# rafifmalikdzaki/Multitask-Bonetumor-yolo

Hardware: AMD Instinct MI355X
Metric: images/sec at 640x640 multitask fwd (det+seg+cls) + decode/NMS/masks (higher is better)
Workload: dtype bf16; 1 GPU; configs[1]: batch-16/GPU 640x640 multitask inference (ConvNeXt-T + C2f-BiFPN + Detect/Segment/cls) + decode + per-image NMS(top-100) + mask assembly; random-init weights; batch_per_gpu=16, img=640, parallelism=dp1 (batch sharded, no data-path collective)

## Files before the change

include/mtbt_hip.h:

```cpp
#ifndef MTBT_HIP_H
#define MTBT_HIP_H

#include <stdint.h>

#ifdef __cplusplus
extern "C" {
#endif

#define MTBT_OK 0
#define MTBT_EINVAL (-1)
#define MTBT_EALIGN (-2)
#define MTBT_ELAUNCH (-3)
#define MTBT_EWORKSPACE (-4)

#define MTBT_F32 0
#define MTBT_BF16 1
#define MTBT_F16 2

#define MTBT_ACT_NONE 0
#define MTBT_ACT_SILU 1
#define MTBT_ACT_ELU 2
#define MTBT_ACT_GELU 3
#define MTBT_ACT_DSILU 5
#define MTBT_ACT_DELU 6
#define MTBT_ACT_DGELU 7
#define MTBT_ACT_GELU_POLY 4
#define MTBT_ACT_DGELU_POLY 8

#define MTBT_OUT_NHWC 0
#define MTBT_OUT_CONVT2X2 1

#define MTBT_ABI_VERSION 5
int mtbt_abi_version(void);
int mtbt_sizeof_args(int which);
const char* mtbt_target_arch(void);

typedef struct mtbt_conv_args {
  const void* x;
  const void* w;
  void* y;
  const float* scale;
  const float* shift;
  const void* res;
  int64_t x_batch_stride, y_batch_stride, res_batch_stride;
  int32_t x_pixel_stride, y_pixel_stride, res_pixel_stride;
  int32_t N, H, W, C;
  int32_t K;
  int32_t R, S;
  int32_t stride, pad;
  int32_t Ho, Wo;
  int32_t dtype;
  int32_t out_dtype;
  int32_t act;
  int32_t out_mode;
  int32_t tile_hint;
  void* y2;
  int32_t policy;
  int32_t debug;
  float* colsum;
  const float* colsum_shift;
  int32_t colsum_sq;
  int32_t colsum_accumulate;
  void* colsum_ws;
  int64_t colsum_ws_bytes;
} mtbt_conv_args;

int mtbt_conv2d_nhwc(const mtbt_conv_args* a, void* stream);
int64_t mtbt_conv_colsum_workspace_bytes(int64_t pixels , int K, int with_squares);
int mtbt_conv_colsum_layout(const mtbt_conv_args* a, int64_t* rows, int32_t* pitch);
int mtbt_conv_kernel_choice(const mtbt_conv_args* a, int32_t* choice);

int mtbt_conv2d_nhwc_batch(const mtbt_conv_args* calls, int n, void* stream);
int mtbt_conv_batch_kernel_choice(const mtbt_conv_args* calls, int n, int32_t* choice);

int mtbt_stem_conv4x4_ln(const float* x, const float* w, const float* bias, const float* ln_w,
                         const float* ln_b, float ln_eps, void* y, int N, int H, int W, int Cout,
                         int out_dtype, void* stream);

int mtbt_dwconv_nhwc(const void* x, const void* w, const float* bias, const float* ln_w,
                     const float* ln_b, float ln_eps, const float* scale, const float* shift, int act,
                     void* y, int N, int H, int W, int C, int ksize, int dtype, void* stream);
int mtbt_dwconv3x3_mult_nhwc(const void* x, const void* w, const float* scale, const float* shift, int act, void* y,
                             int N, int H, int W, int C, int M, int dtype, void* stream);
int mtbt_dwconv_kernel_choice(int N, int H, int W, int C, int ksize, int ln, int act, int dtype, int32_t* choice);
int mtbt_dwconv3x3_mult_kernel_choice(int N, int H, int W, int C, int M, int act, int dtype, int32_t* choice);

int mtbt_layernorm_nhwc(const void* x, const float* w, const float* b, float eps, void* y,
                        int64_t pixels, int C, int dtype, void* stream);

typedef struct mtbt_fuse_args {
  const void* x[3];
  float wgt[3];
  int32_t resample[3];
  int32_t n_in;
  void* y;
  int32_t N, H, W, C;
  int32_t dtype;
  int32_t add_weight_bug;
  const float* wgt_dev;
} mtbt_fuse_args;

int mtbt_bifpn_fuse(const mtbt_fuse_args* a, void* stream);

typedef struct mtbt_node_args {
  mtbt_fuse_args fuse;
  const void* w;
  const float* shift;
  void* y;
  int32_t y_pixel_stride;
  int32_t K;
  int32_t act;
} mtbt_node_args;
int mtbt_bifpn_node_nhwc(const mtbt_node_args* a, void* stream);

typedef struct mtbt_pw_chain_args {
  const void* x;
  const void* w1;
  const float* scale1;
  const float* shift1;
  const void* w2;
  const float* scale2;
  const float* shift2;
  void* y;
  int64_t pixels;
  int32_t y_pixel_stride;
  int32_t C;
  int32_t M;
  int32_t K;
  int32_t dtype;
  int32_t out_dtype;
  int32_t act1;
  int32_t act2;
} mtbt_pw_chain_args;
int mtbt_pw_chain_nhwc(const mtbt_pw_chain_args* a, void* stream);
int mtbt_pw_chain_supported(const mtbt_pw_chain_args* a);
int mtbt_sizeof_pw_chain_args(void);

int64_t mtbt_bn_train_workspace_bytes(int64_t pixels, int C);
int mtbt_bn_train_nhwc(const void* x, void* y, const float* gamma, const float* beta, float* running_mean,
                       float* running_var, float momentum, float eps, int act, int64_t pixels, int C, int dtype,
                       void* workspace, int64_t workspace_bytes, void* stream);

int mtbt_gap_fc(const void* x, const float* w, const float* b, float* y, int N, int HW, int C,
                int nout, int dtype, void* stream);

typedef struct mtbt_decode_args {
  const float* map[3];
  int32_t h[3], w[3];
  int32_t map_pixel_stride[3];
  float stride[3];
  int32_t n_levels, N, nc, reg_max;
  int32_t xywh;
  float* boxes;
  float* scores;
  float* best_score;
  int32_t* best_label;
  float* preds_cat;
  int32_t cat_stride;
} mtbt_decode_args;

int mtbt_decode_boxes(const mtbt_decode_args* a, void* stream);

int64_t mtbt_nms_workspace_bytes(int N, int A);
int mtbt_nms_batched(const float* boxes, const float* best_score, const int32_t* best_label, int N, int A,
                     float conf_th, float iou_th, float clamp_max, int top_k, int64_t* keep_idx,
                     int32_t* keep_anchor, float* out_boxes, float* out_scores, int64_t* out_labels,
                     int32_t* counts, int32_t* n_cand, void* workspace, int64_t workspace_bytes,
                     void* stream);

typedef struct mtbt_mask_args {
  const float* protos;
  const float* coeff;
  int64_t coeff_batch_stride, coeff_k_stride, coeff_c_stride;
  const int32_t* gather_idx;
  const int32_t* counts;
  float bias;
  int32_t N, K, nm, hp, wp, Hout, Wout;
  float* logits;
  uint8_t* masks;
} mtbt_mask_args;

int mtbt_mask_assemble(const mtbt_mask_args* a, void* stream);

typedef struct mtbt_frame {
  int32_t height, width;
  float step;
  float scale;
  int32_t pitch;
  int32_t reserved;
  int64_t offset;
} mtbt_frame;

typedef struct mtbt_frame_mask_args {
  const float* protos;
  const float* coeff;
  int64_t coeff_batch_stride, coeff_k_stride, coeff_c_stride;
  const int32_t* gather_idx;
  const int32_t* counts;
  const float* boxes;
  float* boxes_frame;
  uint8_t* out;
  int64_t out_bytes;
  int32_t N, K, nm, hp, wp;
  int32_t crop;
} mtbt_frame_mask_args;

int mtbt_masks_to_frames(const mtbt_frame_mask_args* a, const mtbt_frame* frames, int n_frames, void* stream);
int mtbt_sizeof_frame_args(int which);

#define MTBT_FUSE_MAX_SOURCES 8
#define MTBT_FUSE_MAX_CANDIDATES 4096
typedef struct mtbt_box_fuse_args {
  const float* boxes[MTBT_FUSE_MAX_SOURCES];
  const float* scores[MTBT_FUSE_MAX_SOURCES];
  const int64_t* labels[MTBT_FUSE_MAX_SOURCES];
  const int32_t* counts[MTBT_FUSE_MAX_SOURCES];
  const int32_t* anchors[MTBT_FUSE_MAX_SOURCES];
  int32_t orient[MTBT_FUSE_MAX_SOURCES];
  float weight[MTBT_FUSE_MAX_SOURCES];
  int32_t n_sources, N, K, top_k;
  float img_size, iou_thr, skip_thr;
  int32_t reserved;
  float* out_boxes;
  float* out_scores;
  int64_t* out_labels;
  int32_t* out_counts;
  int32_t* n_clusters;
  int32_t* n_members;
  int32_t* lead_source;
  int32_t* lead_slot;
  int32_t* lead_anchor;
  void* workspace;
  int64_t workspace_bytes;
} mtbt_box_fuse_args;

int64_t mtbt_fuse_workspace_bytes(int n_sources, int N, int K);
int mtbt_fuse_detections(const mtbt_box_fuse_args* a, void* stream);
int mtbt_sizeof_box_fuse_args(void);
int mtbt_fuse_detections_members(const mtbt_box_fuse_args* a, int32_t* member_slot, void* stream);

typedef struct mtbt_vote_mask_args {
  const float* protos[MTBT_FUSE_MAX_SOURCES];
  const float* mc[MTBT_FUSE_MAX_SOURCES];
  int64_t mc_batch_stride[MTBT_FUSE_MAX_SOURCES], mc_k_stride[MTBT_FUSE_MAX_SOURCES], mc_c_stride[MTBT_FUSE_MAX_SOURCES];
  const int32_t* anchors[MTBT_FUSE_MAX_SOURCES];
  const float* scores[MTBT_FUSE_MAX_SOURCES];
  float weight[MTBT_FUSE_MAX_SOURCES];
  int32_t orient[MTBT_FUSE_MAX_SOURCES];
  const int32_t* member_slot;
  const int32_t* counts;
  const float* boxes;
  float* boxes_frame;
  float* W;
  float* Ss;
  uint8_t* out;
  int64_t out_bytes;
  int32_t n_sources, N, K, top_k, nm, hp, wp, crop;
} mtbt_vote_mask_args;

int mtbt_vote_masks(const mtbt_vote_mask_args* a, const mtbt_frame* frames, int n_frames, void* stream);
int mtbt_sizeof_vote_mask_args(void);

#define MTBT_TILE_MAX_PER_IMAGE 64
#define MTBT_MERGE_IOU 0
#define MTBT_MERGE_IOS 1
typedef struct mtbt_tile {
  int32_t image;
  int32_t pox, poy;
  int32_t wx0, wy0, wx1, wy1;
  int32_t height, width;
  int32_t reserved;
  float step, scale;
  float fox, foy;
} mtbt_tile;

typedef struct mtbt_tile_merge_args {
  const float* boxes;
  const float* scores;
  const int64_t* labels;
  const int32_t* counts;
  const int32_t* anchors;
  const mtbt_tile* tiles;
  const mtbt_tile* tiles_dev;
  const int32_t* first;
  int32_t N, n_tiles, K, top_k;
  int32_t metric, class_agnostic;
  float thr, skip_thr;
  float* out_boxes;
  float* out_scores;
  int64_t* out_labels;
// ... 442 lines not shown
```

multitask_bonetumor_yolo_amd/_lib.py:

```python
import ctypes as C
import os

_HERE = os.path.dirname(os.path.abspath(__file__))
LIB_PATH = os.path.join(_HERE, "csrc", "libmtbt_hip.so")

ABI_VERSION = 5
F32, BF16, F16 = 0, 1, 2
ACT_NONE, ACT_SILU, ACT_ELU, ACT_GELU, ACT_GELU_POLY, ACT_DSILU, ACT_DELU, ACT_DGELU, ACT_DGELU_POLY = 0, 1, 2, 3, 4, 5, 6, 7, 8
OUT_NHWC, OUT_CONVT2X2 = 0, 1
RES_ID, RES_UP_BILINEAR, RES_DOWN_MEAN, RES_UP_NEAREST, RES_MAXPOOL = 0, 1, 2, 3, 4
CONFUSION_MAX_NC = 64

ERRORS = {-1: "MTBT_EINVAL (bad argument / unsupported shape)", -2: "MTBT_EALIGN (misaligned pointer or stride)",
          -3: "MTBT_ELAUNCH (kernel launch failed)", -4: "MTBT_EWORKSPACE (workspace too small)"}


class ConvArgs(C.Structure):
    _fields_ = [
        ("x", C.c_void_p), ("w", C.c_void_p), ("y", C.c_void_p), ("scale", C.c_void_p), ("shift", C.c_void_p),
        ("res", C.c_void_p),
        ("x_batch_stride", C.c_int64), ("y_batch_stride", C.c_int64), ("res_batch_stride", C.c_int64),
        ("x_pixel_stride", C.c_int32), ("y_pixel_stride", C.c_int32), ("res_pixel_stride", C.c_int32),
        ("N", C.c_int32), ("H", C.c_int32), ("W", C.c_int32), ("C", C.c_int32), ("K", C.c_int32),
        ("R", C.c_int32), ("S", C.c_int32), ("stride", C.c_int32), ("pad", C.c_int32),
        ("Ho", C.c_int32), ("Wo", C.c_int32), ("dtype", C.c_int32), ("out_dtype", C.c_int32),
        ("act", C.c_int32), ("out_mode", C.c_int32), ("tile_hint", C.c_int32), ("y2", C.c_void_p),
        ("policy", C.c_int32), ("debug", C.c_int32),
        ("colsum", C.c_void_p), ("colsum_shift", C.c_void_p), ("colsum_sq", C.c_int32), ("colsum_accumulate", C.c_int32),
        ("colsum_ws", C.c_void_p), ("colsum_ws_bytes", C.c_int64),
    ]


class FuseArgs(C.Structure):
    _fields_ = [
        ("x", C.c_void_p * 3), ("wgt", C.c_float * 3), ("resample", C.c_int32 * 3), ("n_in", C.c_int32),
        ("y", C.c_void_p), ("N", C.c_int32), ("H", C.c_int32), ("W", C.c_int32), ("C", C.c_int32),
        ("dtype", C.c_int32), ("add_weight_bug", C.c_int32), ("wgt_dev", C.c_void_p),
    ]


class NodeArgs(C.Structure):
    _fields_ = [("fuse", FuseArgs), ("w", C.c_void_p), ("shift", C.c_void_p), ("y", C.c_void_p), ("y_pixel_stride", C.c_int32), ("K", C.c_int32),
                ("act", C.c_int32)]


class PwChainArgs(C.Structure):
    _fields_ = [("x", C.c_void_p), ("w1", C.c_void_p), ("scale1", C.c_void_p), ("shift1", C.c_void_p), ("w2", C.c_void_p), ("scale2", C.c_void_p),
                ("shift2", C.c_void_p), ("y", C.c_void_p), ("pixels", C.c_int64), ("y_pixel_stride", C.c_int32), ("C", C.c_int32), ("M", C.c_int32),
                ("K", C.c_int32), ("dtype", C.c_int32), ("out_dtype", C.c_int32), ("act1", C.c_int32), ("act2", C.c_int32)]


class UpconvArgs(C.Structure):
    _fields_ = [("x", C.c_void_p), ("w", C.c_void_p), ("y", C.c_void_p), ("shift", C.c_void_p),
                ("x_batch_stride", C.c_int64), ("y_batch_stride", C.c_int64), ("x_pixel_stride", C.c_int32), ("y_pixel_stride", C.c_int32),
                ("N", C.c_int32), ("H", C.c_int32), ("W", C.c_int32), ("C", C.c_int32), ("K", C.c_int32), ("dtype", C.c_int32), ("act", C.c_int32)]


class DecodeArgs(C.Structure):
    _fields_ = [
        ("map", C.c_void_p * 3), ("h", C.c_int32 * 3), ("w", C.c_int32 * 3), ("map_pixel_stride", C.c_int32 * 3),
        ("stride", C.c_float * 3), ("n_levels", C.c_int32), ("N", C.c_int32), ("nc", C.c_int32),
        ("reg_max", C.c_int32), ("xywh", C.c_int32),
        ("boxes", C.c_void_p), ("scores", C.c_void_p), ("best_score", C.c_void_p), ("best_label", C.c_void_p),
        ("preds_cat", C.c_void_p), ("cat_stride", C.c_int32),
    ]


class MaskArgs(C.Structure):
    _fields_ = [
        ("protos", C.c_void_p), ("coeff", C.c_void_p),
        ("coeff_batch_stride", C.c_int64), ("coeff_k_stride", C.c_int64), ("coeff_c_stride", C.c_int64),
        ("gather_idx", C.c_void_p), ("counts", C.c_void_p), ("bias", C.c_float),
        ("N", C.c_int32), ("K", C.c_int32), ("nm", C.c_int32), ("hp", C.c_int32), ("wp", C.c_int32),
        ("Hout", C.c_int32), ("Wout", C.c_int32), ("logits", C.c_void_p), ("masks", C.c_void_p),
    ]


class LossArgs(C.Structure):
    _fields_ = [
        ("map", C.c_void_p * 3), ("h", C.c_int32 * 3), ("w", C.c_int32 * 3), ("map_pixel_stride", C.c_int32 * 3),
        ("n_levels", C.c_int32), ("N", C.c_int32), ("nc", C.c_int32), ("reg_max", C.c_int32), ("img_size", C.c_float),
        ("gt_xyxy", C.c_void_p), ("gt_cls", C.c_void_p), ("gt_off", C.c_void_p),
        ("iou_thresh", C.c_float), ("label_smoothing", C.c_float), ("training", C.c_int32),
        ("seg_logits", C.c_void_p), ("seg_targets", C.c_void_p), ("seg_bias", C.c_void_p), ("seg_n", C.c_int64),
        ("img_logits", C.c_void_p), ("img_gt", C.c_void_p), ("n_img_classes", C.c_int32),
        ("w_seg", C.c_float), ("w_box", C.c_float), ("w_dfl", C.c_float), ("w_cls", C.c_float), ("w_img", C.c_float),
        ("workspace", C.c_void_p), ("workspace_bytes", C.c_int64), ("out", C.c_void_p),
    ]


class BoxEvalArgs(C.Structure):
    _fields_ = [("boxes", C.c_void_p), ("scores", C.c_void_p), ("labels", C.c_void_p), ("counts", C.c_void_p), ("gt", C.c_void_p),
                ("rank", C.c_void_p), ("match", C.c_void_p), ("ignore", C.c_void_p), ("gt_area", C.c_void_p), ("status", C.c_void_p),
                ("iou_thresholds", C.c_double * 32), ("B", C.c_int32), ("K", C.c_int32), ("M", C.c_int32), ("T", C.c_int32),
                ("max_det", C.c_int32), ("gt_format", C.c_int32), ("img_size", C.c_float)]


class PrepDesc(C.Structure):
    _fields_ = [("src", C.c_void_p), ("dst", C.c_void_p), ("scale0", C.c_void_p), ("scale1", C.c_void_p),
                ("sstride", C.c_int64 * 4), ("dim", C.c_int32 * 4), ("flip", C.c_int32 * 4),
                ("scale0_dim", C.c_int32), ("scale1_dim", C.c_int32), ("dst_dtype", C.c_int32), ("src_dim3", C.c_int32)]


class RawImage(C.Structure):
    _fields_ = [("bgr", C.c_void_p), ("mask", C.c_void_p), ("height", C.c_int32), ("width", C.c_int32),
                ("row_stride", C.c_int64), ("mask_row_stride", C.c_int64)]


class Frame(C.Structure):
    _fields_ = [("height", C.c_int32), ("width", C.c_int32), ("step", C.c_float), ("scale", C.c_float), ("pitch", C.c_int32),
                ("reserved", C.c_int32), ("offset", C.c_int64)]


class FrameMaskArgs(C.Structure):
    _fields_ = [("protos", C.c_void_p), ("coeff", C.c_void_p),
                ("coeff_batch_stride", C.c_int64), ("coeff_k_stride", C.c_int64), ("coeff_c_stride", C.c_int64),
                ("gather_idx", C.c_void_p), ("counts", C.c_void_p), ("boxes", C.c_void_p), ("boxes_frame", C.c_void_p),
                ("out", C.c_void_p), ("out_bytes", C.c_int64),
                ("N", C.c_int32), ("K", C.c_int32), ("nm", C.c_int32), ("hp", C.c_int32), ("wp", C.c_int32), ("crop", C.c_int32)]


class PackMasksArgs(C.Structure):
    _fields_ = [("src", C.c_void_p), ("plane_of", C.c_void_p), ("boxes", C.c_void_p), ("out", C.c_void_p),
                ("plane_stride", C.c_int64), ("row_stride", C.c_int64),
                ("n_src", C.c_int32), ("n_out", C.c_int32), ("H", C.c_int32), ("W", C.c_int32), ("pitch", C.c_int32), ("dtype", C.c_int32)]


class MaskImage(C.Structure):
    _fields_ = [("det", C.c_void_p), ("gt_base", C.c_void_p), ("H", C.c_int32), ("W", C.c_int32), ("pitch", C.c_int32),
                ("g0", C.c_int32), ("gt_planes", C.c_int32), ("reserved", C.c_int32)]


class MaskPairArgs(C.Structure):
    _fields_ = [("counts", C.c_void_p), ("gt_image", C.c_void_p), ("inter", C.c_void_p), ("det_area", C.c_void_p), ("gt_area", C.c_void_p),
                ("B", C.c_int32), ("K", C.c_int32), ("M", C.c_int32), ("reserved", C.c_int32)]


class MaskEvalArgs(C.Structure):
    _fields_ = [("inter", C.c_void_p), ("det_area", C.c_void_p), ("gt_px", C.c_void_p), ("scores", C.c_void_p), ("labels", C.c_void_p),
                ("counts", C.c_void_p), ("gt_image", C.c_void_p), ("gt_label", C.c_void_p),
                ("rank", C.c_void_p), ("match", C.c_void_p), ("ignore", C.c_void_p), ("gt_area", C.c_void_p), ("status", C.c_void_p),
                ("iou_thresholds", C.c_double * 32), ("B", C.c_int32), ("K", C.c_int32), ("M", C.c_int32), ("T", C.c_int32),
                ("max_det", C.c_int32), ("reserved", C.c_int32)]


class MaskLossArgs(C.Structure):
    _fields_ = [("map", C.c_void_p * 3), ("h", C.c_int32 * 3), ("w", C.c_int32 * 3), ("map_pixel_stride", C.c_int32 * 3),
                ("n_levels", C.c_int32), ("N", C.c_int32), ("reg_max", C.c_int32), ("img_size", C.c_float), ("iou_thresh", C.c_float),
                ("n_gt", C.c_int32), ("gt_xyxy", C.c_void_p), ("gt_off", C.c_void_p), ("mc", C.c_void_p),
                ("mc_batch_stride", C.c_int64), ("mc_anchor_stride", C.c_int64), ("mc_channel_stride", C.c_int64),
                ("protos", C.c_void_p), ("gt_masks", C.c_void_p), ("hp", C.c_int32), ("wp", C.c_int32), ("nm", C.c_int32), ("weight", C.c_float),
                ("d_mc", C.c_void_p), ("d_protos", C.c_void_p), ("accumulate_dmc", C.c_int32), ("dprotos_dtype", C.c_int32),
                ("accumulate_dprotos", C.c_int32), ("reserved", C.c_int32), ("workspace", C.c_void_p), ("workspace_bytes", C.c_int64),
                ("out", C.c_void_p)]


class TalLossArgs(C.Structure):
    _fields_ = [("map", C.c_void_p * 3), ("h", C.c_int32 * 3), ("w", C.c_int32 * 3), ("map_pixel_stride", C.c_int32 * 3),
                ("n_levels", C.c_int32), ("N", C.c_int32), ("nc", C.c_int32), ("reg_max", C.c_int32), ("img_size", C.c_float),
                ("n_gt", C.c_int32), ("gt_xyxy", C.c_void_p), ("gt_cls", C.c_void_p), ("gt_off", C.c_void_p),
                ("topk", C.c_int32), ("alpha", C.c_float), ("beta", C.c_float), ("w_box", C.c_float), ("w_dfl", C.c_float), ("w_cls", C.c_float),
                ("accumulate", C.c_int32), ("reserved", C.c_int32), ("d_map", C.c_void_p * 3), ("d_map_pixel_stride", C.c_int32 * 3),
                ("reserved2", C.c_int32), ("assigned", C.c_void_p), ("target_score", C.c_void_p),
                ("workspace", C.c_void_p), ("workspace_bytes", C.c_int64), ("out", C.c_void_p)]


class BoxFuseArgs(C.Structure):
    _fields_ = [("boxes", C.c_void_p * 8), ("scores", C.c_void_p * 8), ("labels", C.c_void_p * 8), ("counts", C.c_void_p * 8),
                ("anchors", C.c_void_p * 8), ("orient", C.c_int32 * 8), ("weight", C.c_float * 8),
                ("n_sources", C.c_int32), ("N", C.c_int32), ("K", C.c_int32), ("top_k", C.c_int32),
                ("img_size", C.c_float), ("iou_thr", C.c_float), ("skip_thr", C.c_float), ("reserved", C.c_int32),
                ("out_boxes", C.c_void_p), ("out_scores", C.c_void_p), ("out_labels", C.c_void_p), ("out_counts", C.c_void_p),
                ("n_clusters", C.c_void_p), ("n_members", C.c_void_p), ("lead_source", C.c_void_p), ("lead_slot", C.c_void_p),
                ("lead_anchor", C.c_void_p), ("workspace", C.c_void_p), ("workspace_bytes", C.c_int64)]


class VoteMaskArgs(C.Structure):
    _fields_ = [("protos", C.c_void_p * 8), ("mc", C.c_void_p * 8),
                ("mc_batch_stride", C.c_int64 * 8), ("mc_k_stride", C.c_int64 * 8), ("mc_c_stride", C.c_int64 * 8),
                ("anchors", C.c_void_p * 8), ("scores", C.c_void_p * 8), ("weight", C.c_float * 8), ("orient", C.c_int32 * 8),
                ("member_slot", C.c_void_p), ("counts", C.c_void_p), ("boxes", C.c_void_p), ("boxes_frame", C.c_void_p),
                ("W", C.c_void_p), ("Ss", C.c_void_p), ("out", C.c_void_p), ("out_bytes", C.c_int64),
                ("n_sources", C.c_int32), ("N", C.c_int32), ("K", C.c_int32), ("top_k", C.c_int32),
                ("nm", C.c_int32), ("hp", C.c_int32), ("wp", C.c_int32), ("crop", C.c_int32)]


class Tile(C.Structure):
    _fields_ = [("image", C.c_int32), ("pox", C.c_int32), ("poy", C.c_int32),
                ("wx0", C.c_int32), ("wy0", C.c_int32), ("wx1", C.c_int32), ("wy1", C.c_int32),
                ("height", C.c_int32), ("width", C.c_int32), ("reserved", C.c_int32),
                ("step", C.c_float), ("scale", C.c_float), ("fox", C.c_float), ("foy", C.c_float)]


class TileMergeArgs(C.Structure):
    _fields_ = [("boxes", C.c_void_p), ("scores", C.c_void_p), ("labels", C.c_void_p), ("counts", C.c_void_p), ("anchors", C.c_void_p),
                ("tiles", C.POINTER(Tile)), ("tiles_dev", C.c_void_p), ("first", C.POINTER(C.c_int32)),
                ("N", C.c_int32), ("n_tiles", C.c_int32), ("K", C.c_int32), ("top_k", C.c_int32),
                ("metric", C.c_int32), ("class_agnostic", C.c_int32), ("thr", C.c_float), ("skip_thr", C.c_float),
                ("out_boxes", C.c_void_p), ("out_scores", C.c_void_p), ("out_labels", C.c_void_p), ("out_counts", C.c_void_p),
                ("n_members", C.c_void_p), ("lead_tile", C.c_void_p), ("lead_slot", C.c_void_p), ("lead_anchor", C.c_void_p),
                ("member_slot", C.c_void_p), ("n_left", C.c_void_p)]


class TileMaskArgs(C.Structure):
    _fields_ = [("protos", C.c_void_p), ("mc", C.c_void_p),
                ("mc_batch_stride", C.c_int64), ("mc_k_stride", C.c_int64), ("mc_c_stride", C.c_int64),
                ("anchors", C.c_void_p), ("scores", C.c_void_p), ("member_slot", C.c_void_p), ("counts", C.c_void_p), ("boxes", C.c_void_p),
                ("tiles", C.POINTER(Tile)), ("tiles_dev", C.c_void_p), ("first", C.POINTER(C.c_int32)),
                ("W", C.c_void_p), ("Ss", C.c_void_p), ("out", C.c_void_p), ("out_bytes", C.c_int64),
                ("N", C.c_int32), ("n_tiles", C.c_int32), ("K", C.c_int32), ("top_k", C.c_int32), ("Tmax", C.c_int32),
                ("nm", C.c_int32), ("hp", C.c_int32), ("wp", C.c_int32), ("crop", C.c_int32), ("reserved", C.c_int32)]


class SurfaceArgs(C.Structure):
    _fields_ = [("a", C.c_void_p), ("b", C.c_void_p), ("workspace", C.c_void_p), ("workspace_bytes", C.c_int64),
                ("n_edge", C.c_void_p), ("max_d2", C.c_void_p), ("n_within", C.c_void_p), ("sum_d", C.c_void_p), ("rank_d2", C.c_void_p),
                ("q", C.c_double * 4), ("n", C.c_int32), ("H", C.c_int32), ("W", C.c_int32), ("pitch", C.c_int32),
                ("tol2", C.c_uint32), ("Q", C.c_int32)]


class ComponentsArgs(C.Structure):
    _fields_ = [("packed", C.c_void_p), ("other", C.c_void_p), ("workspace", C.c_void_p), ("workspace_bytes", C.c_int64),
                ("labels", C.c_void_p), ("n_components", C.c_void_p), ("area", C.c_void_p), ("box", C.c_void_p), ("first", C.c_void_p),
                ("inter", C.c_void_p), ("n", C.c_int32), ("H", C.c_int32), ("W", C.c_int32), ("pitch", C.c_int32),
                ("connectivity", C.c_int32), ("max_components", C.c_int32)]


class SelectComponentsArgs(C.Structure):
    _fields_ = [("packed", C.c_void_p), ("workspace", C.c_void_p), ("workspace_bytes", C.c_int64), ("out", C.c_void_p),
                ("n_kept", C.c_void_p), ("n", C.c_int32), ("H", C.c_int32), ("W", C.c_int32), ("pitch", C.c_int32),
                ("min_area", C.c_uint32), ("keep_largest", C.c_int32)]


class FillPolygonsArgs(C.Structure):
    _fields_ = [("vertices", C.c_void_p), ("poly_offsets", C.c_void_p), ("plane_offsets", C.c_void_p), ("clip", C.c_void_p),
                ("out", C.c_void_p), ("area", C.c_void_p), ("box", C.c_void_p),
                ("n", C.c_int32), ("n_polys", C.c_int32), ("n_vertices", C.c_int32), ("H", C.c_int32), ("W", C.c_int32), ("pitch", C.c_int32)]


class ClaheImage(C.Structure):
    _fields_ = [("src", C.c_void_p), ("dst", C.c_void_p), ("height", C.c_int32), ("width", C.c_int32), ("channels", C.c_int32), ("clip", C.c_int32),
                ("src_row_stride", C.c_int64), ("dst_row_stride", C.c_int64)]


SYMBOLS = {
    "mtbt_abi_version": (C.c_int, []),
    "mtbt_sizeof_args": (C.c_int, [C.c_int]),
    "mtbt_target_arch": (C.c_char_p, []),
    "mtbt_conv2d_nhwc": (C.c_int, [C.POINTER(ConvArgs), C.c_void_p]),
    "mtbt_convt2x2_conv3x3_nhwc": (C.c_int, [C.POINTER(UpconvArgs), C.c_void_p]),
    "mtbt_stem_conv4x4_ln": (C.c_int, [C.c_void_p] * 5 + [C.c_float, C.c_void_p] + [C.c_int] * 5 + [C.c_void_p]),
    "mtbt_dwconv_nhwc": (C.c_int, [C.c_void_p] * 5 + [C.c_float, C.c_void_p, C.c_void_p, C.c_int, C.c_void_p]
                         + [C.c_int] * 6 + [C.c_void_p]),
    "mtbt_layernorm_nhwc": (C.c_int, [C.c_void_p] * 3 + [C.c_float, C.c_void_p, C.c_int64, C.c_int, C.c_int, C.c_void_p]),
    "mtbt_bifpn_fuse": (C.c_int, [C.POINTER(FuseArgs), C.c_void_p]),
    "mtbt_bifpn_node_nhwc": (C.c_int, [C.POINTER(NodeArgs), C.c_void_p]),
    "mtbt_pw_chain_nhwc": (C.c_int, [C.POINTER(PwChainArgs), C.c_void_p]),
    "mtbt_pw_chain_supported": (C.c_int, [C.POINTER(PwChainArgs)]),
    "mtbt_sizeof_pw_chain_args": (C.c_int, []),
    "mtbt_bn_train_workspace_bytes": (C.c_int64, [C.c_int64, C.c_int]),
    "mtbt_bn_train_nhwc": (C.c_int, [C.c_void_p] * 6 + [C.c_float, C.c_float, C.c_int, C.c_int64, C.c_int, C.c_int, C.c_void_p,
                                      C.c_int64, C.c_void_p]),
    "mtbt_gap_fc": (C.c_int, [C.c_void_p] * 4 + [C.c_int] * 5 + [C.c_void_p]),
    "mtbt_decode_boxes": (C.c_int, [C.POINTER(DecodeArgs), C.c_void_p]),
    "mtbt_nms_workspace_bytes": (C.c_int64, [C.c_int, C.c_int]),
    "mtbt_nms_batched": (C.c_int, [C.c_void_p] * 3 + [C.c_int, C.c_int, C.c_float, C.c_float, C.c_float, C.c_int]
                         + [C.c_void_p] * 8 + [C.c_int64, C.c_void_p]),
    "mtbt_mask_assemble": (C.c_int, [C.POINTER(MaskArgs), C.c_void_p]),
    "mtbt_loss_workspace_bytes": (C.c_int64, [C.c_int, C.c_int, C.c_int64]),
    "mtbt_multitask_loss": (C.c_int, [C.POINTER(LossArgs), C.c_void_p]),
    "mtbt_multitask_loss_grad": (C.c_int, [C.POINTER(LossArgs), C.POINTER(C.c_void_p), C.POINTER(C.c_int32), C.c_void_p, C.c_void_p, C.c_void_p]),
    "mtbt_convnext_mlp_fused": (C.c_int, [C.c_void_p] * 7 + [C.c_int64, C.c_int, C.c_void_p]),
    "mtbt_convnext_mlp_fused_dt": (C.c_int, [C.c_void_p] * 7 + [C.c_int64, C.c_int, C.c_int, C.c_void_p]),
    "mtbt_convnext_mlp_fused_train": (C.c_int, [C.c_void_p] * 8 + [C.c_int64, C.c_int, C.c_void_p]),
    "mtbt_bbox_iou_pairwise": (C.c_int, [C.c_void_p, C.c_int, C.c_void_p, C.c_int, C.c_float, C.c_void_p, C.c_void_p]),
    "mtbt_letterbox_batch": (C.c_int, [C.POINTER(RawImage), C.c_int, C.c_int, C.c_void_p, C.c_void_p, C.POINTER(C.c_double), C.c_void_p]),
    "mtbt_augment_batch": (C.c_int, [C.POINTER(RawImage), C.c_int, C.c_int, C.POINTER(C.c_int32), C.c_int, C.c_void_p, C.c_void_p, C.c_void_p, C.c_void_p]),
    "mtbt_mosaic_batch": (C.c_int, [C.POINTER(RawImage), C.c_int, C.c_int, C.POINTER(C.c_int32), C.c_int, C.POINTER(C.c_int32), C.c_void_p, C.c_void_p, C.c_void_p, C.c_void_p]),
    "mtbt_seg_confusion_workspace_bytes": (C.c_int64, [C.c_int]),
    "mtbt_seg_confusion": (C.c_int, [C.c_void_p, C.c_void_p, C.c_int, C.c_int64, C.c_void_p, C.c_void_p, C.c_void_p, C.c_int64, C.c_void_p]),
    "mtbt_conv_wgrad_workspace_bytes": (C.c_int64, [C.c_int] * 7),
    "mtbt_conv_wgrad": (C.c_int, [C.c_void_p] * 3 + [C.c_int] * 9 + [C.c_int64, C.c_int32, C.c_int64, C.c_int32, C.c_int, C.c_int, C.c_void_p,
                                  C.c_int64, C.c_void_p]),
    "mtbt_conv_wgrad_xact": (C.c_int, [C.c_void_p] * 3 + [C.c_int] * 9 + [C.c_int64, C.c_int32, C.c_int64, C.c_int32, C.c_int, C.c_int, C.c_int, C.c_void_p,
                                       C.c_int64, C.c_void_p]),
    "mtbt_conv_wgrad_bias": (C.c_int, [C.c_void_p] * 4 + [C.c_int] * 9 + [C.c_int64, C.c_int32, C.c_int64, C.c_int32, C.c_int, C.c_int, C.c_void_p,
                                       C.c_int64, C.c_void_p]),
    "mtbt_act_backward": (C.c_int, [C.c_void_p] * 3 + [C.c_int64, C.c_int, C.c_int, C.c_void_p]),
    "mtbt_channel_sum_workspace_bytes": (C.c_int64, [C.c_int64, C.c_int]),
    "mtbt_channel_sum": (C.c_int, [C.c_void_p, C.c_void_p, C.c_int64, C.c_int, C.c_int32, C.c_int32, C.c_int, C.c_void_p, C.c_int, C.c_void_p,
                                   C.c_int64, C.c_void_p]),
    "mtbt_channel_affine2": (C.c_int, [C.c_void_p] * 6 + [C.c_int64, C.c_int, C.c_int, C.c_void_p]),
    "mtbt_layernorm_backward_nhwc": (C.c_int, [C.c_void_p] * 3 + [C.c_float, C.c_void_p, C.c_void_p, C.c_int64, C.c_int, C.c_int, C.c_int, C.c_void_p]),
    "mtbt_layernorm_backward_params_workspace_bytes": (C.c_int64, [C.c_int64, C.c_int]),
    "mtbt_layernorm_backward_params_nhwc": (C.c_int, [C.c_void_p] * 3 + [C.c_float, C.c_void_p, C.c_int64, C.c_int, C.c_int, C.c_int, C.c_void_p, C.c_void_p,
                                                      C.c_int, C.c_void_p, C.c_int64, C.c_void_p]),
    "mtbt_dwconv_wgrad_workspace_bytes": (C.c_int64, [C.c_int] * 5),
    "mtbt_dwconv_wgrad": (C.c_int, [C.c_void_p] * 3 + [C.c_int] * 7 + [C.c_void_p, C.c_int64, C.c_void_p]),
    "mtbt_dwconv_wgrad_bias": (C.c_int, [C.c_void_p] * 4 + [C.c_int] * 7 + [C.c_void_p, C.c_int64, C.c_void_p]),
    "mtbt_adamw_step": (C.c_int, [C.c_void_p] * 4 + [C.c_int64] + [C.c_float] * 5 + [C.c_int64, C.c_void_p, C.c_void_p]),
    "mtbt_sgd_step": (C.c_int, [C.c_void_p] * 3 + [C.c_int64] + [C.c_float] * 4 + [C.c_int, C.c_int64, C.c_void_p, C.c_void_p]),
    "mtbt_adamw_step_ema": (C.c_int, [C.c_void_p] * 5 + [C.c_int64] + [C.c_float] * 5 + [C.c_int64, C.c_void_p, C.c_double, C.c_void_p]),
    "mtbt_sgd_step_ema": (C.c_int, [C.c_void_p] * 4 + [C.c_int64] + [C.c_float] * 4 + [C.c_int, C.c_int64, C.c_void_p, C.c_double, C.c_void_p]),
    "mtbt_ema_update": (C.c_int, [C.c_void_p, C.c_void_p, C.c_int64, C.c_double, C.c_void_p]),
    "mtbt_sumsq_workspace_bytes": (C.c_int64, []),
    "mtbt_sumsq": (C.c_int, [C.c_void_p, C.c_int64, C.c_void_p, C.c_int, C.c_void_p, C.c_int64, C.c_void_p]),
    "mtbt_clip_coef": (C.c_int, [C.c_void_p, C.c_float, C.c_void_p, C.c_void_p, C.c_void_p]),
    "mtbt_stem_conv4x4_ln_train": (C.c_int, [C.c_void_p] * 5 + [C.c_float, C.c_void_p, C.c_void_p] + [C.c_int] * 5 + [C.c_void_p]),
    "mtbt_dwconv_nhwc_train": (C.c_int, [C.c_void_p] * 5 + [C.c_float, C.c_void_p, C.c_void_p, C.c_int, C.c_void_p, C.c_void_p, C.c_void_p]
                               + [C.c_int] * 6 + [C.c_void_p]),
    "mtbt_bn_forward_nhwc": (C.c_int, [C.c_void_p, C.c_void_p, C.c_int32] + [C.c_void_p] * 4 + [C.c_float, C.c_float, C.c_int, C.c_int64, C.c_int, C.c_int,
                                       C.c_int, C.c_void_p, C.c_void_p, C.c_int64, C.c_void_p]),
    "mtbt_bn_forward_sums_nhwc": (C.c_int, [C.c_void_p, C.c_void_p, C.c_int32] + [C.c_void_p] * 4 + [C.c_float, C.c_float, C.c_int, C.c_int64, C.c_int, C.c_int,
                                            C.c_void_p, C.c_void_p, C.c_void_p, C.c_void_p]),
    "mtbt_conv_colsum_workspace_bytes": (C.c_int64, [C.c_int64, C.c_int, C.c_int]),
    "mtbt_conv_colsum_layout": (C.c_int, [C.c_void_p, C.c_void_p, C.c_void_p]),
    "mtbt_conv_kernel_choice": (C.c_int, [C.c_void_p, C.c_void_p]),
    "mtbt_conv2d_nhwc_batch": (C.c_int, [C.c_void_p, C.c_int, C.c_void_p]),
    "mtbt_conv_batch_kernel_choice": (C.c_int, [C.c_void_p, C.c_int, C.c_void_p]),
    "mtbt_dwconv3x3_mult_nhwc": (C.c_int, [C.c_void_p] * 4 + [C.c_int, C.c_void_p] + [C.c_int] * 6 + [C.c_void_p]),
    "mtbt_dwconv_kernel_choice": (C.c_int, [C.c_int] * 8 + [C.c_void_p]),
    "mtbt_dwconv3x3_mult_kernel_choice": (C.c_int, [C.c_int] * 7 + [C.c_void_p]),
    "mtbt_bn_forward_partials_nhwc": (C.c_int, [C.c_void_p, C.c_void_p, C.c_int32] + [C.c_void_p] * 4 + [C.c_float, C.c_float, C.c_int, C.c_int64, C.c_int, C.c_int,
                                                C.c_void_p, C.c_int64, C.c_int32, C.c_void_p, C.c_void_p, C.c_void_p]),
    "mtbt_bn_backward_workspace_bytes": (C.c_int64, [C.c_int64, C.c_int]),
    "mtbt_bn_backward_nhwc": (C.c_int, [C.c_void_p, C.c_int32] + [C.c_void_p] * 4 + [C.c_float, C.c_int, C.c_int] + [C.c_void_p] * 3
                              + [C.c_int, C.c_int64, C.c_int, C.c_int, C.c_void_p, C.c_int64, C.c_void_p]),
    "mtbt_weight_prep_blocks": (C.c_int, [C.c_int64]),
    "mtbt_weight_prep": (C.c_int, [C.c_void_p, C.c_void_p, C.c_int, C.c_int, C.c_void_p]),
    "mtbt_bifpn_norm_weights": (C.c_int, [C.c_void_p, C.c_int, C.c_float, C.c_void_p, C.c_void_p]),
    "mtbt_bifpn_norm_weights_backward": (C.c_int, [C.c_void_p, C.c_int, C.c_float, C.c_void_p, C.c_void_p, C.c_int, C.c_void_p]),
    "mtbt_wadd_norm_weights": (C.c_int, [C.c_void_p, C.c_int, C.c_float, C.c_void_p, C.c_void_p]),
    "mtbt_wadd_norm_weights_backward": (C.c_int, [C.c_void_p, C.c_int, C.c_float, C.c_void_p, C.c_int, C.c_void_p, C.c_int, C.c_void_p]),
    "mtbt_resample_backward": (C.c_int, [C.c_void_p, C.c_void_p, C.c_int, C.c_void_p, C.c_int] + [C.c_int] * 5 + [C.c_void_p]),
    "mtbt_bifpn_fuse_backward_workspace_bytes": (C.c_int64, []),
    "mtbt_bifpn_fuse_backward": (C.c_int, [C.c_void_p, C.c_void_p, C.c_int, C.c_void_p, C.c_void_p, C.c_int, C.c_void_p, C.c_int] + [C.c_int] * 5
                                 + [C.c_void_p, C.c_int64, C.c_void_p]),
    "mtbt_projector_backward_workspace_bytes": (C.c_int64, [C.c_int] * 4),
    "mtbt_projector_backward": (C.c_int, [C.c_void_p] * 4 + [C.c_int, C.c_int, C.c_void_p, C.c_void_p, C.c_int] + [C.c_int] * 6
                                + [C.c_void_p, C.c_int64, C.c_void_p]),
    "mtbt_gap_fc_backward": (C.c_int, [C.c_void_p] * 4 + [C.c_int, C.c_void_p, C.c_void_p, C.c_int, C.c_void_p] + [C.c_int] * 5 + [C.c_void_p]),
    "mtbt_copy_strided": (C.c_int, [C.c_void_p, C.c_int, C.c_int64, C.c_int32, C.c_void_p, C.c_int, C.c_int64, C.c_int32, C.c_int, C.c_int64,
                                    C.c_int, C.c_int, C.c_void_p]),
    "mtbt_scale_grad": (C.c_int, [C.c_int] + [C.c_void_p] * 8 + [C.c_int, C.c_int, C.c_int, C.c_void_p]),
    "mtbt_add_nhwc": (C.c_int, [C.c_void_p, C.c_int64, C.c_int32, C.c_void_p, C.c_int64, C.c_int32, C.c_int, C.c_int64, C.c_int, C.c_int, C.c_void_p]),
    "mtbt_stem_wgrad_workspace_bytes": (C.c_int64, [C.c_int]),
    "mtbt_stem_wgrad": (C.c_int, [C.c_void_p] * 3 + [C.c_int] * 6 + [C.c_void_p, C.c_int64, C.c_void_p]),
    "mtbt_cast": (C.c_int, [C.c_void_p, C.c_void_p, C.c_int64, C.c_int, C.c_int, C.c_void_p]),
    "mtbt_box_eval": (C.c_int, [C.POINTER(BoxEvalArgs), C.c_void_p]),
    "mtbt_det_confusion": (C.c_int, [C.POINTER(LossArgs), C.c_void_p, C.c_void_p, C.c_void_p]),
    "mtbt_cls_confusion": (C.c_int, [C.c_void_p, C.c_void_p, C.c_int, C.c_int, C.c_void_p, C.c_void_p, C.c_void_p]),
    "mtbt_masks_to_frames": (C.c_int, [C.POINTER(FrameMaskArgs), C.POINTER(Frame), C.c_int, C.c_void_p]),
    "mtbt_sizeof_frame_args": (C.c_int, [C.c_int]),
    "mtbt_pack_masks": (C.c_int, [C.POINTER(PackMasksArgs), C.c_void_p]),
    "mtbt_mask_pair_counts": (C.c_int, [C.POINTER(MaskPairArgs), C.POINTER(MaskImage), C.c_int, C.c_void_p]),
    "mtbt_mask_eval": (C.c_int, [C.POINTER(MaskEvalArgs), C.c_void_p]),
    "mtbt_sizeof_mask_eval_args": (C.c_int, [C.c_int]),
    "mtbt_mask_loss_workspace_bytes": (C.c_int64, [C.c_int] * 5),
    "mtbt_instance_mask_loss": (C.c_int, [C.POINTER(MaskLossArgs), C.c_void_p]),
    "mtbt_instance_mask_loss_assigned": (C.c_int, [C.POINTER(MaskLossArgs), C.c_void_p, C.c_void_p]),
    "mtbt_sizeof_mask_loss_args": (C.c_int, []),
    "mtbt_tal_loss_workspace_bytes": (C.c_int64, [C.c_int] * 3),
    "mtbt_tal_det_loss": (C.c_int, [C.POINTER(TalLossArgs), C.c_void_p]),
    "mtbt_sizeof_tal_loss_args": (C.c_int, []),
    "mtbt_fuse_workspace_bytes": (C.c_int64, [C.c_int, C.c_int, C.c_int]),
    "mtbt_fuse_detections": (C.c_int, [C.POINTER(BoxFuseArgs), C.c_void_p]),
    "mtbt_sizeof_box_fuse_args": (C.c_int, []),
    "mtbt_fuse_detections_members": (C.c_int, [C.POINTER(BoxFuseArgs), C.c_void_p, C.c_void_p]),
    "mtbt_vote_masks": (C.c_int, [C.POINTER(VoteMaskArgs), C.POINTER(Frame), C.c_int, C.c_void_p]),
    "mtbt_sizeof_vote_mask_args": (C.c_int, []),
    "mtbt_merge_tiles": (C.c_int, [C.POINTER(TileMergeArgs), C.c_void_p]),
    "mtbt_vote_tile_masks": (C.c_int, [C.POINTER(TileMaskArgs), C.POINTER(Frame), C.c_int, C.c_void_p]),
    "mtbt_sizeof_tile_args": (C.c_int, [C.c_int]),
    "mtbt_surface_distances_workspace_bytes": (C.c_int64, [C.c_int, C.c_int, C.c_int]),
    "mtbt_surface_distances": (C.c_int, [C.POINTER(SurfaceArgs), C.c_void_p]),
    "mtbt_sizeof_surface_args": (C.c_int, [C.c_int]),
    "mtbt_components_workspace_bytes": (C.c_int64, [C.c_int, C.c_int, C.c_int]),
    "mtbt_label_components": (C.c_int, [C.POINTER(ComponentsArgs), C.c_void_p]),
    "mtbt_select_components": (C.c_int, [C.POINTER(SelectComponentsArgs), C.c_void_p]),
    "mtbt_sizeof_components_args": (C.c_int, [C.c_int]),
    "mtbt_fill_polygons": (C.c_int, [C.POINTER(FillPolygonsArgs), C.c_void_p]),
    "mtbt_sizeof_fill_polygons_args": (C.c_int, [C.c_int]),
    "mtbt_clahe_workspace_bytes": (C.c_int64, [C.POINTER(ClaheImage), C.c_int, C.c_int, C.c_int]),
    "mtbt_clahe_batch": (C.c_int, [C.POINTER(ClaheImage), C.c_int, C.c_int, C.c_int, C.c_void_p, C.c_int64, C.c_void_p]),
    "mtbt_sizeof_clahe_args": (C.c_int, [C.c_int]),
}

ARG_STRUCTS = (ConvArgs, FuseArgs, DecodeArgs, MaskArgs, LossArgs, PrepDesc, RawImage, UpconvArgs, NodeArgs, BoxEvalArgs)
FRAME_STRUCTS = (Frame, FrameMaskArgs)
MASK_EVAL_STRUCTS = (PackMasksArgs, MaskImage, MaskPairArgs, MaskEvalArgs)
TILE_STRUCTS = (Tile, TileMergeArgs, TileMaskArgs)
SURFACE_STRUCTS = (SurfaceArgs,)
COMPONENTS_STRUCTS = (ComponentsArgs, SelectComponentsArgs)
POLYGON_STRUCTS = (FillPolygonsArgs,)
CLAHE_STRUCTS = (ClaheImage,)
_lib = None


def load():
    global _lib
    if _lib is None:
        if not os.path.exists(LIB_PATH):
            raise RuntimeError(f"{LIB_PATH} is missing: run `python -m multitask_bonetumor_yolo_amd.build` "
                               "(there is no CPU fallback)")
        lib = C.CDLL(LIB_PATH)
        for name, (res, args) in SYMBOLS.items():
            fn = getattr(lib, name)
            fn.restype, fn.argtypes = res, args
        if lib.mtbt_abi_version() != ABI_VERSION:
            raise RuntimeError(f"libmtbt_hip.so reports ABI version {lib.mtbt_abi_version()}, this binding is version {ABI_VERSION}: rebuild "
                               "(`python -m multitask_bonetumor_yolo_amd.build`)")
        for which, st in enumerate(ARG_STRUCTS):
            if lib.mtbt_sizeof_args(which) != C.sizeof(st):
                raise RuntimeError(f"libmtbt_hip.so was built with sizeof({st.__name__}) = {lib.mtbt_sizeof_args(which)}, this binding lays it out in "
                                   f"{C.sizeof(st)} bytes: stale library, rebuild")
        for sizeof, structs in ((lib.mtbt_sizeof_frame_args, FRAME_STRUCTS), (lib.mtbt_sizeof_mask_eval_args, MASK_EVAL_STRUCTS),
                                (lib.mtbt_sizeof_tile_args, TILE_STRUCTS), (lib.mtbt_sizeof_surface_args, SURFACE_STRUCTS),
                                (lib.mtbt_sizeof_components_args, COMPONENTS_STRUCTS), (lib.mtbt_sizeof_fill_polygons_args, POLYGON_STRUCTS),
                                (lib.mtbt_sizeof_clahe_args, CLAHE_STRUCTS)):
            for which, st in enumerate(structs):
                if sizeof(which) != C.sizeof(st):
                    raise RuntimeError(f"libmtbt_hip.so was built with sizeof({st.__name__}) = {sizeof(which)}, this binding lays it "
                                       f"out in {C.sizeof(st)} bytes: stale library, rebuild")
        for sizeof, st in ((lib.mtbt_sizeof_mask_loss_args, MaskLossArgs), (lib.mtbt_sizeof_tal_loss_args, TalLossArgs),
                           (lib.mtbt_sizeof_pw_chain_args, PwChainArgs), (lib.mtbt_sizeof_box_fuse_args, BoxFuseArgs),
                           (lib.mtbt_sizeof_vote_mask_args, VoteMaskArgs)):
            if sizeof() != C.sizeof(st):
                raise RuntimeError(f"libmtbt_hip.so was built with sizeof({st.__name__}) = {sizeof()}, this binding lays it "
                                   f"out in {C.sizeof(st)} bytes: stale library, rebuild")
        _lib = lib
    return _lib


def check(code: int, what: str):
    if code != 0:
        raise RuntimeError(f"{what}: {ERRORS.get(code, code)}")
```

multitask_bonetumor_yolo_amd/build.py:

```python
import os
import subprocess
import sys
from concurrent.futures import ThreadPoolExecutor

HERE = os.path.dirname(os.path.abspath(__file__))
CSRC = os.path.join(HERE, "csrc")
INCLUDE = os.path.join(os.path.dirname(HERE), "include")
LIB = os.path.join(CSRC, "libmtbt_hip.so")
SOURCES = ["conv_igemm.hip", "conv_igemm_bf16.hip", "conv_igemm_bf16_n.hip", "conv_direct_bf16.hip", "conv_igemm_f32.hip", "conv_igemm_f32_n.hip", "conv_direct_f32.hip", "conv_igemm_f16.hip", "conv_igemm_f16_n.hip", "conv_direct_f16.hip", "conv_batch_bf16.hip", "conv_batch_f16.hip", "conv_batch_f32.hip", "dwconv.hip", "dwconv_bf16.hip", "dwconv_f16.hip", "dwconv_f32.hip", "pointwise.hip", "postprocess.hip", "mask_mfma.hip", "mask_frame.hip", "bn_train.hip", "mlp_fused.hip", "upconv_fused.hip", "node_gemm.hip", "pw_stream.hip", "pw_chain.hip", "loss.hip", "mask_loss.hip", "det_loss_tal.hip", "preprocess.hip", "metrics.hip", "optim.hip", "wgrad.hip", "pointwise_bwd.hip", "train_ops.hip", "resample_bwd.hip", "box_eval.hip", "mask_eval.hip", "box_fuse.hip", "mask_vote.hip", "tile_merge.hip", "mask_tiles.hip", "surface_dist.hip", "components.hip", "polygon_fill.hip", "clahe.hip"]
HIPCC = os.environ.get("HIPCC", "/opt/rocm/bin/hipcc")
FLAGS = ["--offload-arch=gfx950", "-O3", "-std=c++17", "-fPIC", "-I" + INCLUDE, "-I" + CSRC,
         "-fno-gpu-rdc", "-Wno-unused-value"]
if os.environ.get("MTBT_CONV_ABLATION"):
    FLAGS.append("-DMTBT_CONV_ABLATION")


EXTRA_FLAGS = {"postprocess.hip": ["-ffp-contract=off"], "loss.hip": ["-ffp-contract=off"], "mask_loss.hip": ["-ffp-contract=off"], "det_loss_tal.hip": ["-ffp-contract=off"], "preprocess.hip": ["-ffp-contract=off"], "optim.hip": ["-ffp-contract=off"],
               "box_eval.hip": ["-ffp-contract=off"], "mask_frame.hip": ["-ffp-contract=off"], "box_fuse.hip": ["-ffp-contract=off"], "mask_vote.hip": ["-ffp-contract=off"],
               "tile_merge.hip": ["-ffp-contract=off"], "mask_tiles.hip": ["-ffp-contract=off"], "surface_dist.hip": ["-ffp-contract=off"]}


def _newer(target, deps):
    if not os.path.exists(target):
        return True
    t = os.path.getmtime(target)
    return any(os.path.getmtime(d) > t for d in deps)


def build(force: bool = False, verbose: bool = False) -> str:
    headers = [os.path.join(INCLUDE, "mtbt_hip.h")] + [os.path.join(CSRC, f) for f in os.listdir(CSRC) if f.endswith((".h", ".inc"))]
    jobs = []
    for s in SOURCES:
        src = os.path.join(CSRC, s)
        obj = os.path.join(CSRC, s.replace(".hip", ".o"))
        if force or _newer(obj, [src] + headers):
            jobs.append([HIPCC] + FLAGS + EXTRA_FLAGS.get(s, []) + ["-c", src, "-o", obj])

    def run(cmd):
        if verbose:
            print(" ".join(cmd), flush=True)
        r = subprocess.run(cmd, capture_output=True, text=True)
        if r.returncode != 0:
            raise RuntimeError("hipcc failed:\n" + " ".join(cmd) + "\n" + r.stdout + r.stderr)

    if jobs:
        with ThreadPoolExecutor(max_workers=min(8, len(jobs))) as ex:
            list(ex.map(run, jobs))
    objs = [os.path.join(CSRC, s.replace(".hip", ".o")) for s in SOURCES]
    if force or jobs or _newer(LIB, objs):
        run([HIPCC, "--offload-arch=gfx950", "-shared", "-fPIC", "-o", LIB] + objs)
    return LIB


if __name__ == "__main__":
    print(build(force="--force" in sys.argv, verbose=True))
```

multitask_bonetumor_yolo_amd/csrc/conv3x3_direct.inc:

```
#ifndef MTBT_RR_RESPF
#define MTBT_RR_RESPF 2
#endif
#pragma once
#include "common.h"
#include "conv_dma.h"
#include "conv_epilogue.h"
#include "conv_params.h"
#include "conv_tiles.h"

namespace {

template <typename T, int TC>
__global__ __launch_bounds__(256, 2) void conv3x3_direct_kernel(const ConvP p) {
  constexpr int ES = (int)sizeof(T), EPC = 16 / ES, BKB = 128, BKE = BKB / ES;
  constexpr int HWID = 18, NHP = HWID * HWID;
  constexpr int FC = TC / 16, FP = 4;
  constexpr int XDMA = (NHP * 8 + 255) / 256;
  constexpr int XBYTES = XDMA * 256 * 16;
  constexpr int WDMA = TC * 8 / 256;
  constexpr int WBYTES = TC * BKB;
  constexpr unsigned OOB = 0x80000000u;
  static_assert(TC % 32 == 0 && WDMA * 256 == TC * 8, "weight tile = whole wave-instructions");

  extern __shared__ __attribute__((aligned(16))) char smem[];
  float* aff = reinterpret_cast<float*>(smem + XBYTES + 2 * WBYTES);
  static_assert(4 * 16 * (TC * 4 + 16) <= XBYTES + 2 * WBYTES, "epilogue slabs below the affine copy");
  const int tid = threadIdx.x, lane = tid & 63;
  const int wave = __builtin_amdgcn_readfirstlane(tid >> 6);
  const int lr = lane & 15, lq = lane >> 4;

  const int slot = blockIdx.x >> 3, xcd = blockIdx.x & 7;
  const int ctile = slot % p.ctiles;
  const int ptile = xcd * p.ptiles_per_xcd + slot / p.ctiles;
  const int tiles_x = p.W >> 4, tpi = tiles_x * (p.H >> 4);
  if (ptile >= p.N * tpi) return;
  const int n = ptile / tpi, trem = ptile - n * tpi;
  const int ty0 = (trem / tiles_x) << 4, tx0 = (trem % tiles_x) << 4;
  const int cbase = ctile * TC;
  const int Kdim = 9 * p.C;
  stage_affine<TC>(p, aff, cbase, tid);

  const srd_t xsrd = make_srd(reinterpret_cast<const T*>(p.x) + (long)n * p.xbs);
  const srd_t wsrd = make_srd(reinterpret_cast<const T*>(p.w) + (long)cbase * Kdim);
  const unsigned lds0 = (unsigned)(size_t)(__attribute__((address_space(3))) char*)smem;

  unsigned xvoff[XDMA];
#pragma unroll
  for (int i = 0; i < XDMA; ++i) {
    const int c = i * 256 + tid;
    const int hp = c >> 3, sl = c & 7;
    const int hy = hp / HWID, hx = hp - hy * HWID;
    const int iy = ty0 - 1 + hy, ix = tx0 - 1 + hx;
    const bool ok = hp < NHP && (unsigned)iy < (unsigned)p.H && (unsigned)ix < (unsigned)p.W;
    xvoff[i] = ok ? (unsigned)((((long)iy * p.W + ix) * p.ldx + (sl ^ (hp & 7)) * EPC) * ES) : OOB;
  }
  unsigned wvoff[WDMA];
#pragma unroll
  for (int i = 0; i < WDMA; ++i) {
    const int c = i * 256 + tid;
    const int row = c >> 3, sl = c & 7;
    const int srow = epi_row_channel(row);
    wvoff[i] = (cbase + srow < p.K) ? (unsigned)(((long)srow * Kdim + (sl ^ ((row >> 1) & 7)) * EPC) * ES) : OOB;
  }

  int baddr[6][3][2];
#pragma unroll
  for (int rr = 0; rr < 6; ++rr)
#pragma unroll
    for (int s = 0; s < 3; ++s) {
      const int hp = (4 * wave + rr) * HWID + lr + s;
#pragma unroll
      for (int ks = 0; ks < 2; ++ks) baddr[rr][s][ks] = hp * BKB + (((ks * 4 + lq) ^ (hp & 7)) << 4);
    }
  int abase[2];
#pragma unroll
  for (int ks = 0; ks < 2; ++ks) abase[ks] = XBYTES + lr * BKB + (((ks * 4 + lq) ^ ((lr >> 1) & 7)) << 4);

  f32x4 acc[FC][FP];
#pragma unroll
  for (int i = 0; i < FC; ++i)
#pragma unroll
    for (int j = 0; j < FP; ++j) acc[i][j] = f32x4{0.f, 0.f, 0.f, 0.f};

  const int nchunks = p.C / BKE;
  for (int cc = 0; cc < nchunks; ++cc) {
    lds_barrier();
    const int csoff = cc * BKB;
#pragma unroll
    for (int i = 0; i < XDMA; ++i) lds_dma16(xsrd, xvoff[i], csoff, lds0 + (i * 256 + wave * 64) * 16);
#pragma unroll
    for (int i = 0; i < WDMA; ++i) lds_dma16(wsrd, wvoff[i], csoff, lds0 + XBYTES + (i * 256 + wave * 64) * 16);
#pragma unroll
    for (int tap = 0; tap < 9; ++tap) {
      wait_vm<0>();
      lds_barrier();
      if (tap < 8) {
        const int wsoff = ((tap + 1) * p.C) * ES + csoff;
#pragma unroll
        for (int i = 0; i < WDMA; ++i)
          lds_dma16(wsrd, wvoff[i], wsoff, lds0 + XBYTES + ((tap + 1) & 1) * WBYTES + (i * 256 + wave * 64) * 16);
      }
      const int r = tap / 3, s = tap - 3 * r;
      const char* wb = smem + (tap & 1) * WBYTES;
#pragma unroll
      for (int ks = 0; ks < 2; ++ks) {
        uint4 a[FC], b[FP];
#pragma unroll
        for (int f = 0; f < FC; ++f) a[f] = *reinterpret_cast<const uint4*>(wb + abase[ks] + f * 16 * BKB);
#pragma unroll
        for (int j = 0; j < FP; ++j) b[j] = *reinterpret_cast<const uint4*>(smem + baddr[j + r][s][ks]);
#pragma unroll
        for (int i = 0; i < FC; ++i)
#pragma unroll
          for (int j = 0; j < FP; ++j) {
            if constexpr (sizeof(T) == 2) {
              acc[i][j] = mfma_16x16x32<T>(a[i], b[j], acc[i][j]);
            } else {
              acc[i][j] = __builtin_amdgcn_mfma_f32_16x16x4f32(__uint_as_float(a[i].x), __uint_as_float(b[j].x), acc[i][j], 0, 0, 0);
              acc[i][j] = __builtin_amdgcn_mfma_f32_16x16x4f32(__uint_as_float(a[i].y), __uint_as_float(b[j].y), acc[i][j], 0, 0, 0);
              acc[i][j] = __builtin_amdgcn_mfma_f32_16x16x4f32(__uint_as_float(a[i].z), __uint_as_float(b[j].z), acc[i][j], 0, 0, 0);
              acc[i][j] = __builtin_amdgcn_mfma_f32_16x16x4f32(__uint_as_float(a[i].w), __uint_as_float(b[j].w), acc[i][j], 0, 0, 0);
            }
          }
      }
    }
  }
  __syncthreads();

  const EpiSeq seq{(long)(ty0 + 4 * wave) * p.W + tx0, p.W, 0x7fffffffffffffffL, (long)n * p.ybs, (long)n * p.rbs};
  conv_epilogue<T, TC, FC, FP, false, MTBT_RR_RESPF, false, true>(p, acc, smem + wave * (16 * (TC * 4 + 16)), aff, cbase, 0, lane,
                               [&](int j, int row, int ch, long& yoff, long& roff) -> bool {
    const long pixoff = (long)(ty0 + 4 * wave + j) * p.W + tx0 + row;
    yoff = (long)n * p.ybs + pixoff * p.ldy + ch;
    roff = (long)n * p.rbs + pixoff * p.ldr + ch;
    return true;
  }, seq, true, (long)ptile * DIRECT_CS_ROWS + wave);
}

template <typename T, int TC>
int launch_direct3x3(ConvP q, hipStream_t stream) {
  constexpr int XBYTES = ((324 * 8 + 255) / 256) * 256 * 16;
  constexpr int lds_main = XBYTES + 2 * TC * 128;
  constexpr int lds_epi = 4 * 16 * (TC * 4 + 16);
  constexpr int lds = (lds_main > lds_epi ? lds_main : lds_epi) + 2 * TC * 4;
  return conv_launch_tiles(conv3x3_direct_kernel<T, TC>, q, TC, (long)q.N * (q.H >> 4) * (q.W >> 4), 1, lds, stream);
}

template <typename T, int TC>
__global__ __launch_bounds__(256, 2) void conv3x3_rr_kernel(const ConvP p) {
  const unsigned bid = blockIdx.x;
#include "conv3x3_rr_body.inc"
}

#ifdef MTBT_CONV_BATCH_UNIT
template <typename T, int TC>
__global__ __launch_bounds__(256, 2) void conv3x3_rr_batch_kernel(const ConvBatchP b) {
  const ConvP p = conv_member(b, (int)blockIdx.y);
  const unsigned bid = blockIdx.x;
#include "conv3x3_rr_body.inc"
}
#endif

template <int TC, typename Kernel, typename Params>
int launch_direct3x3_rr(Kernel kernel, Params q, int n, hipStream_t stream) {
  constexpr int XBYTES = ((324 * 4 + 255) / 256) * 256 * 16;
  constexpr int lds = XBYTES + 2 * 3 * TC * 64 + 2 * TC * 4;
  const ConvP& p = conv_of(q);
  return conv_launch_tiles(kernel, q, TC, (long)p.N * (p.H >> 4) * (p.W >> 4), n, lds, stream);
}

template <typename T>
int dispatch_direct3x3(const ConvP& p, int TC, bool row_reuse, hipStream_t s) {
  if (row_reuse && TC == 128) return launch_direct3x3_rr<128>(conv3x3_rr_kernel<T, 128>, p, 1, s);
  if (row_reuse && TC == 64) return launch_direct3x3_rr<64>(conv3x3_rr_kernel<T, 64>, p, 1, s);
  if (TC == 128) return launch_direct3x3<T, 128>(p, s);
  if (TC == 64) return launch_direct3x3<T, 64>(p, s);
  return MTBT_EINVAL;
}

}
```

multitask_bonetumor_yolo_amd/csrc/conv3x3_rr_body.inc:

```
  constexpr int ES = (int)sizeof(T), EPC = 16 / ES, BKB = 64, BKE = BKB / ES;
  constexpr int HWID = 18, NHP = HWID * HWID;
  constexpr int FC = TC / 32, FP = 8, WCH = TC / 2;
  constexpr int XDMA = (NHP * 4 + 255) / 256;
  constexpr int XBYTES = XDMA * 256 * 16;
  constexpr int WTAP = TC * BKB, WGRP = 3 * WTAP;
  constexpr int WDMA = WGRP / 16 / 256;
  constexpr unsigned OOB = 0x80000000u;
  static_assert(TC % 64 == 0 && WDMA * 256 * 16 == WGRP, "weight column = whole wave-instructions");
  static_assert(FC % 2 == 0, "fragment pairs (PERM epilogue)");

  extern __shared__ __attribute__((aligned(16))) char smem[];
  float* aff = reinterpret_cast<float*>(smem + XBYTES + 2 * WGRP);
  static_assert(2 * 4 * 16 * (WCH * 4 + 16) <= XBYTES + 2 * WGRP, "epilogue slabs (two regions per wave) below the affine copy");
  const int tid = threadIdx.x, lane = tid & 63;
  const int wave = __builtin_amdgcn_readfirstlane(tid >> 6);
  const int wc = wave & 1, wr = wave >> 1;
  const int lr = lane & 15, lq = lane >> 4;

  const int slot = bid >> 3, xcd = bid & 7;
  const int ctile = slot % p.ctiles;
  const int ptile = xcd * p.ptiles_per_xcd + slot / p.ctiles;
  const int tiles_x = p.W >> 4, tpi = tiles_x * (p.H >> 4);
  if (ptile >= p.N * tpi) return;
  const int n = ptile / tpi, trem = ptile - n * tpi;
  const int ty0 = (trem / tiles_x) << 4, tx0 = (trem % tiles_x) << 4;
  const int cbase = ctile * TC;
  const int Kdim = 9 * p.C;
  stage_affine<TC>(p, aff, cbase, tid);

  const srd_t xsrd = make_srd(reinterpret_cast<const T*>(p.x) + (long)n * p.xbs);
  const srd_t wsrd = make_srd(reinterpret_cast<const T*>(p.w) + (long)cbase * Kdim);
  const unsigned lds0 = (unsigned)(size_t)(__attribute__((address_space(3))) char*)smem;

  unsigned xvoff[XDMA];
#pragma unroll
  for (int i = 0; i < XDMA; ++i) {
    const int c = i * 256 + tid;
    const int hp = c >> 2, sl = c & 3;
    const int hy = hp / HWID, hx = hp - hy * HWID;
    const int iy = ty0 - 1 + hy, ix = tx0 - 1 + hx;
    const bool ok = hp < NHP && (unsigned)iy < (unsigned)p.H && (unsigned)ix < (unsigned)p.W;
    xvoff[i] = ok ? (unsigned)((((long)iy * p.W + ix) * p.ldx + (sl ^ ((hp >> 2) & 3)) * EPC) * ES) : OOB;
  }
  unsigned wvoff[WDMA];
#pragma unroll
  for (int i = 0; i < WDMA; ++i) {
    const int c = i * 256 + tid;
    const int r = c / (TC * 4), rem = c - r * (TC * 4);
    const int row = rem >> 2, sl = rem & 3;
    const int srow = (row / WCH) * WCH + epi_row_channel(row % WCH);
    wvoff[i] = (cbase + srow < p.K) ? (unsigned)(((long)srow * Kdim + (long)r * 3 * p.C + (sl ^ ((row >> 2) & 3)) * EPC) * ES) : OOB;
  }
  const int hp0 = (8 * wr) * HWID + lr;
  const int arow = wc * WCH + lr;
  const int aoff = XBYTES + arow * BKB + ((lq ^ ((arow >> 2) & 3)) << 4);

  f32x4 acc[FC][FP];
#pragma unroll
  for (int i = 0; i < FC; ++i)
#pragma unroll
    for (int j = 0; j < FP; ++j) acc[i][j] = f32x4{0.f, 0.f, 0.f, 0.f};

  const int nslabs = p.C / BKE, nsteps = 3 * nslabs;
  auto stage_w = [&](int g) {
    const int cc = g / 3, s = g - 3 * cc;
    const int wsoff = (s * p.C) * ES + cc * BKB;
#pragma unroll
    for (int i = 0; i < WDMA; ++i) lds_dma16(wsrd, wvoff[i], wsoff, lds0 + XBYTES + (g & 1) * WGRP + (i * 256 + wave * 64) * 16);
  };
  auto stage_x = [&](int cc) {
#pragma unroll
    for (int i = 0; i < XDMA; ++i) lds_dma16(xsrd, xvoff[i], cc * BKB, lds0 + (i * 256 + wave * 64) * 16);
  };
  stage_x(0);
  stage_w(0);
#pragma unroll 1
  for (int g0 = 0; g0 < nsteps; g0 += 6) {
#pragma unroll
    for (int u = 0; u < 6; ++u) {
      const int g = g0 + u;
      if (g >= nsteps) continue;
      const int s = u % 3;
      wait_vm<0>();
      lds_barrier();
      if (g + 1 < nsteps && !MTBT_ABL(p, 1)) stage_w(g + 1);
      uint4 b[FP + 2];
#pragma unroll
      for (int rr = 0; rr < FP + 2; ++rr) {
        const int hp = hp0 + rr * HWID + s;
        b[rr] = MTBT_ABL(p, 8) ? uint4{1u, 2u, 3u, (unsigned)rr} : *reinterpret_cast<const uint4*>(smem + hp * BKB + ((lq ^ ((hp >> 2) & 3)) << 4));
      }
      if (s == 2 && g + 1 < nsteps && !MTBT_ABL(p, 1)) {
        lds_barrier();
        stage_x(g / 3 + 1);
      }
      const char* wb = smem + aoff + (u & 1) * WGRP;
#pragma unroll
      for (int r = 0; r < 3; ++r) {
        uint4 a[FC];
#pragma unroll
        for (int f = 0; f < FC; ++f) a[f] = MTBT_ABL(p, 8) ? uint4{1u, 2u, 3u, (unsigned)f} : *reinterpret_cast<const uint4*>(wb + r * WTAP + f * 16 * BKB);
        if (MTBT_ABL(p, 4)) {
#pragma unroll
          for (int i = 0; i < FC; ++i) acc[i][0].x += __uint_as_float(a[i].x ^ b[i + r].y ^ b[i + 4 + r].z);
          continue;
        }
#pragma unroll
        for (int i = 0; i < FC; ++i)
#pragma unroll
          for (int j = 0; j < FP; ++j) {
            if constexpr (sizeof(T) == 2) {
              acc[i][j] = mfma_16x16x32<T>(a[i], b[j + r], acc[i][j]);
            } else {
              acc[i][j] = __builtin_amdgcn_mfma_f32_16x16x4f32(__uint_as_float(a[i].x), __uint_as_float(b[j + r].x), acc[i][j], 0, 0, 0);
              acc[i][j] = __builtin_amdgcn_mfma_f32_16x16x4f32(__uint_as_float(a[i].y), __uint_as_float(b[j + r].y), acc[i][j], 0, 0, 0);
              acc[i][j] = __builtin_amdgcn_mfma_f32_16x16x4f32(__uint_as_float(a[i].z), __uint_as_float(b[j + r].z), acc[i][j], 0, 0, 0);
              acc[i][j] = __builtin_amdgcn_mfma_f32_16x16x4f32(__uint_as_float(a[i].w), __uint_as_float(b[j + r].w), acc[i][j], 0, 0, 0);
            }
          }
      }
    }
  }
  __syncthreads();

  const EpiSeq seq{(long)(ty0 + 8 * wr) * p.W + tx0, p.W, 0x7fffffffffffffffL, (long)n * p.ybs, (long)n * p.rbs};
  conv_epilogue<T, TC, FC, FP, false, MTBT_RR_RESPF, (sizeof(T) == 2), true>(p, acc, smem + wave * (2 * 16 * (WCH * 4 + 16)), aff, cbase, wc * WCH, lane,
                               [&](int j, int row, int ch, long& yoff, long& roff) -> bool {
    const long pixoff = (long)(ty0 + 8 * wr + j) * p.W + tx0 + row;
    yoff = (long)n * p.ybs + pixoff * p.ldy + ch;
    roff = (long)n * p.rbs + pixoff * p.ldr + ch;
    return true;
  }, seq, true, (long)ptile * DIRECT_RR_CS_ROWS + wr);
```

multitask_bonetumor_yolo_amd/csrc/conv_epilogue.h:

```cpp
#pragma once
#include "common.h"
#include "conv_params.h"

namespace {

template <int TC>
__device__ __forceinline__ void stage_affine(const ConvP& p, float* aff, int cbase, int tid) {
  for (int c = tid; c < TC; c += 256) {
    const bool ok = cbase + c < p.K;
    aff[c] = (ok && p.scale) ? p.scale[cbase + c] : 1.f;
    aff[TC + c] = (ok && p.shift) ? p.shift[cbase + c] : 0.f;
  }
}

template <typename OUT> __device__ __forceinline__ float stored_value(float v);
template <> __device__ __forceinline__ float stored_value<float>(float v) { return v; }
template <> __device__ __forceinline__ float stored_value<bf16_t>(float v) { return __uint_as_float((unsigned)f2bf(v) << 16); }
template <> __device__ __forceinline__ float stored_value<f16_t>(float v) { return h2f(f2h(v)); }

__device__ __forceinline__ int epi_row_channel(int r) {
  const int F = r >> 4, q = (r >> 2) & 3, e = r & 3;
  return 32 * (F >> 1) + 8 * q + 4 * (F & 1) + e;
}
template <bool PERM> __device__ __forceinline__ int epi_cpos(int i, int lq) { return PERM ? 32 * (i >> 1) + 8 * lq + 4 * (i & 1) : i * 16 + lq * 4; }
// ... 145 lines not shown
    ro[it] = q.rbias + px[it] * p.ldr + ch;
    so[it] = row * PITCH + c8 * 32;
  }
  const long ystep = (long)q.jstep * p.ldy, rstep = (long)q.jstep * p.ldr;
  const bool has_res = p.res != nullptr;
  const int cs_ch = cbase + chl0 + (lane % C8) * 8;
  float cs[8], cq[8], csh[8];
#pragma unroll
  for (int e = 0; e < 8; ++e) { cs[e] = 0.f; cq[e] = 0.f; csh[e] = (SUMS && p.cs_shift && cs_ch + e < p.K) ? p.cs_shift[cs_ch + e] : 0.f; }
  HT* const yp = reinterpret_cast<HT*>(p.y);
  HT* const y2p = reinterpret_cast<HT*>(p.y2);
  const T* const rp = reinterpret_cast<const T*>(p.res);
  uint4 rpf[RESPF == 1 ? FP : 1][RESPF ? ITER : 1];
  uint4 rnx[RESPF == 2 ? ITER : 1];
  auto fetch_res = [&](int j, uint4 (&dst)[RESPF ? ITER : 1]) {
#pragma unroll
    for (int it = 0; it < ITER; ++it) {
      dst[RESPF ? it : 0] = uint4{0u, 0u, 0u, 0u};
      if (ok[it] && px[it] + (long)j * q.jstep < q.npix) dst[RESPF ? it : 0] = *reinterpret_cast<const uint4*>(rp + ro[it] + j * rstep);
    }
  };
  if constexpr (RESPF == 2) {
    if (MODE == 2 || has_res) fetch_res(0, rpf[0]);
  }
  if constexpr (RESPF == 1) {
    if (MODE == 2 || has_res) {
#pragma unroll
      for (int j = 0; j < FP; ++j)
#pragma unroll
        for (int it = 0; it < ITER; ++it) {
          rpf[j][it] = uint4{0u, 0u, 0u, 0u};
          if (ok[it] && px[it] + (long)j * q.jstep < q.npix) rpf[j][it] = *reinterpret_cast<const uint4*>(rp + ro[it] + j * rstep);
        }
    }
  }
  constexpr int SLB = 16 * PITCH;
  auto write_slab = [&](int j, char* sb) {
#pragma unroll
    for (int i = 0; i < FC; ++i) {
      float4 s4, h4;
      if (HOIST) { s4 = sc[HOIST ? i : 0]; h4 = sh[HOIST ? i : 0]; }
      else {
        const int cl = chl0 + epi_cpos<PERM>(i, lq);
        s4 = *reinterpret_cast<const float4*>(aff + cl);
        h4 = *reinterpret_cast<const float4*>(aff + TC + cl);
      }
      float4 v;
      v.x = fmaf(acc[i][j][0], s4.x, h4.x); v.y = fmaf(acc[i][j][1], s4.y, h4.y);
      v.z = fmaf(acc[i][j][2], s4.z, h4.z); v.w = fmaf(acc[i][j][3], s4.w, h4.w);
      if (MODE == 0) { v.x = act_apply(v.x, ACT); v.y = act_apply(v.y, ACT); v.z = act_apply(v.z, ACT); v.w = act_apply(v.w, ACT); }
      *reinterpret_cast<float4*>(sb + lr * PITCH + epi_cpos<PERM>(i, lq) * 4) = v;
    }
  };
  char* const slab0 = slab;
  if constexpr (DB) write_slab(0, slab0);
#pragma clang loop unroll(full)
  for (int j = 0; j < FP; ++j) {
    slab = slab0 + (DB ? (j & 1) * SLB : 0);
    if constexpr (DB) {
      if (j + 1 < FP) {
        write_slab(j + 1, slab0 + ((j + 1) & 1) * SLB);
        asm volatile("s_waitcnt lgkmcnt(%0)" ::"n"(FC) : "memory");
      } else {
        asm volatile("s_waitcnt lgkmcnt(0)" ::: "memory");
      }
    } else {
      write_slab(j, slab);
      asm volatile("s_waitcnt lgkmcnt(0)" ::: "memory");
    }
    if constexpr (RESPF == 2) {
      if ((MODE == 2 || has_res) && j + 1 < FP) fetch_res(j + 1, rnx);
    }
#pragma unroll
    for (int it = 0; it < ITER; ++it) {
      if (!ok[it] || px[it] + (long)j * q.jstep >= q.npix) continue;
      const float4 lo = *reinterpret_cast<const float4*>(slab + so[it]);
      const float4 hi = *reinterpret_cast<const float4*>(slab + so[it] + 16);
      float v[8] = {lo.x, lo.y, lo.z, lo.w, hi.x, hi.y, hi.z, hi.w};
      const long yoff = yo[it] + j * ystep, roff = ro[it] + j * rstep;
      if (MODE == 1) {
        st8<HT>(y2p + yoff, v);
#pragma unroll
        for (int e = 0; e < 8; ++e) v[e] = act_apply(v[e], ACT);
      }
      if (MODE == 2) {
        float r[8];
        if constexpr (RESPF != 0) ld8<T>(reinterpret_cast<const T*>(&rpf[RESPF == 1 ? j : 0][RESPF ? it : 0]), r); else ld8<T>(rp + roff, r);
#pragma unroll
        for (int e = 0; e < 8; ++e) v[e] *= act_grad(r[e], ACT);
      } else if (has_res) {
        float r[8];
        if constexpr (RESPF != 0) ld8<T>(reinterpret_cast<const T*>(&rpf[RESPF == 1 ? j : 0][RESPF ? it : 0]), r); else ld8<T>(rp + roff, r);
#pragma unroll
        for (int e = 0; e < 8; ++e) v[e] += r[e];
      }
      st8<HT>(yp + yoff, v);
      if (SUMS) {
#pragma unroll
        for (int e = 0; e < 8; ++e) { const float d = stored_value<HT>(v[e]) - csh[e]; cs[e] += d; cq[e] += d * d; }
      }
    }
    if constexpr (RESPF == 2) {
#pragma unroll
      for (int it = 0; it < ITER; ++it) rpf[0][it] = rnx[it];
    }
    if constexpr (DB) asm volatile("" ::: "memory"); else asm volatile("s_waitcnt lgkmcnt(0)" ::: "memory");
  }
  if constexpr (SUMS && (C8 & (C8 - 1)) == 0) colsum_flush<C8>(p, cs, cq, srow, cs_ch, cs_ch < p.K, lane);
}

template <typename T, int TC, int FC, int FP, int ACT>
__device__ __forceinline__ void conv_epilogue_direct(const ConvP& p, f32x4 (&acc)[FC][FP], const float* aff, int cbase, int chl0, int lane, const EpiSeq q) {
  static_assert(FC % 2 == 0 && sizeof(T) == 2, "fragment pairs, 16-bit storage");
  typedef typename half_of<T>::type HT;
  const int lr = lane & 15, lq = lane >> 4;
  HT* const yp = reinterpret_cast<HT*>(p.y);
  const T* const rp = reinterpret_cast<const T*>(p.res);
  const bool has_res = p.res != nullptr;
  const long px0 = q.pix0 + lr;
#pragma unroll
  for (int m = 0; m < FC / 2; ++m) {
    const int cl = chl0 + m * 32 + lq * 8;
    const int ch = cbase + cl;
    if (ch >= p.K) continue;
    const float4 s0 = *reinterpret_cast<const float4*>(aff + cl), s1 = *reinterpret_cast<const float4*>(aff + cl + 4);
    const float4 h0 = *reinterpret_cast<const float4*>(aff + TC + cl), h1 = *reinterpret_cast<const float4*>(aff + TC + cl + 4);
    u32x4 rv[FP];
    if (has_res) {
#pragma unroll
      for (int j = 0; j < FP; ++j) {
        const long px = px0 + (long)j * q.jstep;
        rv[j] = u32x4{0u, 0u, 0u, 0u};
        if (px < q.npix) rv[j] = *reinterpret_cast<const u32x4*>(rp + q.rbias + px * p.ldr + ch);
      }
    }
#pragma unroll
    for (int j = 0; j < FP; ++j) {
      const long px = px0 + (long)j * q.jstep;
      if (px >= q.npix) continue;
      float v[8];
      v[0] = act_apply(fmaf(acc[2 * m][j][0], s0.x, h0.x), ACT); v[1] = act_apply(fmaf(acc[2 * m][j][1], s0.y, h0.y), ACT);
      v[2] = act_apply(fmaf(acc[2 * m][j][2], s0.z, h0.z), ACT); v[3] = act_apply(fmaf(acc[2 * m][j][3], s0.w, h0.w), ACT);
      v[4] = act_apply(fmaf(acc[2 * m + 1][j][0], s1.x, h1.x), ACT); v[5] = act_apply(fmaf(acc[2 * m + 1][j][1], s1.y, h1.y), ACT);
      v[6] = act_apply(fmaf(acc[2 * m + 1][j][2], s1.z, h1.z), ACT); v[7] = act_apply(fmaf(acc[2 * m + 1][j][3], s1.w, h1.w), ACT);
      if (has_res) {
        float r[8];
        ld8<T>(reinterpret_cast<const T*>(&rv[j]), r);
#pragma unroll
        for (int e = 0; e < 8; ++e) v[e] += r[e];
      }
      st8<HT>(yp + q.ybias + px * p.ldy + ch, v);
    }
  }
}


template <typename T, int TC, int FC, int FP, bool TRAIN = true, int RESPF = (TRAIN ? 1 : 0), bool DB = false, bool PERM = false, typename AddrFn>
__device__ __forceinline__ void conv_epilogue(const ConvP& p, f32x4 (&acc)[FC][FP], char* slab, const float* aff, int cbase,
                                              int chl0 , int lane, AddrFn addr, const EpiSeq seq, bool use_seq,
                                              long srow = -1 ) {
#define MTBT_FAST(ACTV, MODEV)                                                                                                     \
  do {                                                                                                                            \
    if constexpr (PERM && (MODEV) == 0) conv_epilogue_direct<T, TC, FC, FP, ACTV>(p, acc, aff, cbase, chl0, lane, seq);           \
    else conv_epilogue_fast<T, TC, FC, FP, ACTV, MODEV, false, RESPF, DB, PERM>(p, acc, slab, aff, cbase, chl0, lane, seq);        \
  } while (0)
  const bool fast = sizeof(T) == 2 && use_seq && p.vec_ok && !(p.K & 7) && !p.out_f32 && p.out_mode == MTBT_OUT_NHWC;
  constexpr bool CS_OK = (((FC * 16) / 8) & ((FC * 16) / 8 - 1)) == 0;
  if constexpr (sizeof(T) == 2) {
  if (CS_OK && fast && p.cs_part && srow >= 0 && !(TRAIN && p.y2)) {
    if (p.act == MTBT_ACT_NONE) { conv_epilogue_fast<T, TC, FC, FP, MTBT_ACT_NONE, 0, true, RESPF, DB, PERM>(p, acc, slab, aff, cbase, chl0, lane, seq, srow); return; }
    if (TRAIN && p.act == MTBT_ACT_DGELU_POLY) { conv_epilogue_fast<T, TC, FC, FP, MTBT_ACT_DGELU_POLY, 2, true, RESPF, DB, PERM>(p, acc, slab, aff, cbase, chl0, lane, seq, srow); return; }
  } else if (fast && !(TRAIN && p.y2)) {
    switch (p.act) {
      case MTBT_ACT_NONE: MTBT_FAST(MTBT_ACT_NONE, 0); return;
      case MTBT_ACT_SILU: MTBT_FAST(MTBT_ACT_SILU, 0); return;
      case MTBT_ACT_ELU: MTBT_FAST(MTBT_ACT_ELU, 0); return;
      case MTBT_ACT_GELU: MTBT_FAST(MTBT_ACT_GELU, 0); return;
      case MTBT_ACT_GELU_POLY: MTBT_FAST(MTBT_ACT_GELU_POLY, 0); return;
      case MTBT_ACT_DSILU: if (TRAIN) { MTBT_FAST(MTBT_ACT_DSILU, 2); return; } break;
      case MTBT_ACT_DELU: if (TRAIN) { MTBT_FAST(MTBT_ACT_DELU, 2); return; } break;
      case MTBT_ACT_DGELU_POLY: if (TRAIN) { MTBT_FAST(MTBT_ACT_DGELU_POLY, 2); return; } break;
      default: break;
    }
  } else if (TRAIN && fast && !(p.cs_part && srow >= 0)) {
    switch (p.act) {
      case MTBT_ACT_NONE: MTBT_FAST(MTBT_ACT_NONE, 1); return;
      case MTBT_ACT_GELU: MTBT_FAST(MTBT_ACT_GELU, 1); return;
      case MTBT_ACT_GELU_POLY: MTBT_FAST(MTBT_ACT_GELU_POLY, 1); return;
      default: break;
    }
  }
  }
#undef MTBT_FAST
  conv_epilogue_body<T, TC, FC, FP, TRAIN, -1, false, PERM>(p, acc, slab, aff, cbase, chl0, lane, addr, srow);
}

}
```

multitask_bonetumor_yolo_amd/csrc/conv_igemm.hip:

```cpp
#include "common.h"
#include "conv_params.h"
#include "conv_tiles.h"
#include "rowreduce.h"

struct ConvUnit {
  int (*gemm[2])(const ConvP& p, int TC, int TP, hipStream_t s);
  int (*direct3x3)(const ConvP& p, int TC, bool row_reuse, hipStream_t s);
  int (*batch)(const ConvBatchP& b, int n, const ConvChoice& c, hipStream_t s);
};
#define MTBT_DECL(dt)                                                                      \
  int mtbt_conv_dispatch_##dt##_wide(const ConvP& p, int TC, int TP, hipStream_t s);       \
  int mtbt_conv_dispatch_##dt##_narrow(const ConvP& p, int TC, int TP, hipStream_t s);     \
  int mtbt_conv3x3_direct_##dt(const ConvP& p, int TC, bool row_reuse, hipStream_t s);     \
  int mtbt_conv_batch_dispatch_##dt(const ConvBatchP& b, int n, const ConvChoice& c, hipStream_t s); \
  static const ConvUnit conv_unit_##dt = {{mtbt_conv_dispatch_##dt##_narrow, mtbt_conv_dispatch_##dt##_wide}, mtbt_conv3x3_direct_##dt, mtbt_conv_batch_dispatch_##dt};
MTBT_DECL(bf16)
MTBT_DECL(f32)
MTBT_DECL(f16)
#undef MTBT_DECL
static const ConvUnit& conv_unit(int dtype) { return dtype == MTBT_F32 ? conv_unit_f32 : (dtype == MTBT_F16 ? conv_unit_f16 : conv_unit_bf16); }
bool mtbt_pw_stream_applies(const ConvP& p, int dtype, bool any_width);
int mtbt_pw_stream(const ConvP& p, int dtype, hipStream_t s);
bool mtbt_pw_stream_batch_applies(const ConvP& p, int dtype);
int mtbt_pw_stream_batch(const ConvBatchP& b, int n, int dtype, hipStream_t s);
// ... 91 lines not shown
  p.M = a->N * a->Ho * a->Wo;
  p.y_linear = (a->out_mode == MTBT_OUT_NHWC) && (a->y_batch_stride == (int64_t)a->Ho * a->Wo * a->y_pixel_stride) &&
               (!a->res || a->res_batch_stride == (int64_t)a->Ho * a->Wo * a->res_pixel_stride);
  p.ctiles = 0;
  p.ptiles_per_xcd = 0;
  p.debug = a->debug;
  p.cs_part = nullptr; p.cs_shift = a->colsum_shift; p.cs_sq = a->colsum_sq ? 1 : 0; p.cs_pitch = a->K * (a->colsum_sq ? 2 : 1);
  if (a->colsum && !a->colsum_ws) return MTBT_EINVAL;
  if (a->colsum_ws) {
    if (a->out_mode != MTBT_OUT_NHWC || !aligned16(a->colsum_ws)) return MTBT_EINVAL;
    p.cs_part = reinterpret_cast<float*>(a->colsum_ws);
  }
  if ((double)a->R * a->S > 31) return MTBT_EINVAL;
  if (((long)(128 / (a->Ho * a->Wo) + 2) * a->x_batch_stride + 2L * ((long)a->pad * a->W + a->pad) * a->x_pixel_stride) * es >= 0x7fff0000L) return MTBT_EINVAL;
  if ((long)128 * a->R * a->S * a->C * es >= 0x7fff0000L || (long)a->R * a->S * a->C * es >= 0x7fff0000L) return MTBT_EINVAL;
  const int oes = p.out_f32 ? 4 : 2;
  const int kq = a->out_mode == MTBT_OUT_CONVT2X2 ? a->K / 4 : a->K;
  const int ovec = 16 / oes;
  bool vec = (kq % 8 == 0 || a->out_mode == MTBT_OUT_NHWC) && (a->y_pixel_stride % ovec == 0) &&
             (a->y_batch_stride % ovec == 0) && aligned16(a->y);
  if (a->out_mode == MTBT_OUT_CONVT2X2) vec = vec && (kq % 8 == 0);
  if (a->res) vec = vec && (a->res_pixel_stride % epc == 0) && (a->res_batch_stride % epc == 0) && aligned16(a->res);
  p.vec_ok = vec ? 1 : 0;
  return MTBT_OK;
}

static int conv_choose(const mtbt_conv_args* a, const ConvP& p, int nmem, ConvChoice* c) {
  const int es = a->dtype == MTBT_F32 ? 4 : 2;
  const int pol = (a->policy & 0x100) ? (a->policy & 0xff) : 7;
  const bool want_cs = p.cs_part != nullptr;
  if (!a->tile_hint && (pol & 64) == 0 && (long)a->K * a->C * es < 0x7fff0000L &&
      (nmem ? mtbt_pw_stream_batch_applies(p, a->dtype) : mtbt_pw_stream_applies(p, a->dtype, (pol & 128) != 0))) {
    *c = ConvChoice{CONV_PW_STREAM, a->K, 128, false, false, 0, 0};
    return MTBT_OK;
  }
  if ((pol & 4) && !((a->tile_hint >> 26) & 1) && !a->y2 && a->act < MTBT_ACT_DSILU && a->R == 3 && a->S == 3 && a->stride == 1 && a->pad == 1 && a->H % 16 == 0 &&
      a->W % 16 == 0 && a->out_mode == MTBT_OUT_NHWC && a->C % (128 / es) == 0 && a->K > 32 &&
      (long)a->H * a->W * a->x_pixel_stride * es < 0x7fff0000L && (long)128 * 9 * a->C * es < 0x7fff0000L) {
    const bool rr = (pol & 8) || ((a->tile_hint >> 25) & 1) || !(pol & 16);
    const long rows = (long)a->N * (a->H >> 4) * (a->W >> 4) * (rr ? DIRECT_RR_CS_ROWS : DIRECT_CS_ROWS);
    *c = ConvChoice{CONV_DIRECT3X3, (a->K >= 96 && !(pol & 32)) ? 128 : 64, DIRECT_TP, false, rr, rows, p.cs_pitch};
    return MTBT_OK;
  }
  int TC = (a->tile_hint >> 16) & 0x1ff, TP = a->tile_hint & 0xffff;
  int narrow = (a->tile_hint >> 27) & 1;
  if (!a->tile_hint || !TC || !TP) pick_tile(pol, a->K, nmem ? (long)p.M * nmem : (long)p.M, a->R * a->S, a->C, es, &TC, &TP, &narrow, want_cs, a->act);
  if (want_cs && TC == 96) return MTBT_EINVAL;
  const int waves_p = conv_tile_waves_p(TC, TP);
  *c = ConvChoice{CONV_IGEMM, TC, TP, a->C % (128 / es) == 0 && !narrow, false, (((long)p.M + TP - 1) / TP) * (waves_p ? waves_p : 4), p.cs_pitch};
  return MTBT_OK;
}

static int conv_launch(const mtbt_conv_args* a, const ConvP& p, const ConvChoice& c, hipStream_t s) {
  if (c.kind == CONV_PW_STREAM) return mtbt_pw_stream(p, a->dtype, s);
  if (p.cs_part && a->colsum_ws_bytes < c.cs_rows * c.cs_pitch * (int64_t)sizeof(float)) return MTBT_EWORKSPACE;
  const ConvUnit& u = conv_unit(a->dtype);
  const int rc = c.kind == CONV_DIRECT3X3 ? u.direct3x3(p, c.TC, c.row_reuse, s) : u.gemm[c.wide](p, c.TC, c.TP, s);
  if (rc != MTBT_OK || !a->colsum) return rc;
  return colsum_finish(a, p, c.cs_rows, s);
}

static int conv_plan(const mtbt_conv_args* a, int nmem, ConvP* p, ConvChoice* c) {
  if (const int rc = conv_validate(a, p)) return rc;
  return conv_choose(a, *p, nmem, c);
}

static void conv_report(const ConvChoice& c, int32_t* choice) {
  choice[0] = c.kind; choice[1] = c.TC; choice[2] = c.TP;
  choice[3] = c.kind == CONV_IGEMM ? c.wide : (c.kind == CONV_DIRECT3X3 ? !c.row_reuse : 0);
}

extern "C" int mtbt_conv2d_nhwc(const mtbt_conv_args* a, void* stream) {
  ConvP p;
  ConvChoice c;
  if (const int rc = conv_plan(a, 0, &p, &c)) return rc;
  return conv_launch(a, p, c, reinterpret_cast<hipStream_t>(stream));
}

extern "C" int mtbt_conv_colsum_layout(const mtbt_conv_args* a, int64_t* rows, int32_t* pitch) {
  if (!rows || !pitch || !a || !a->colsum_ws) return MTBT_EINVAL;
  ConvP p;
  ConvChoice c;
  if (const int rc = conv_plan(a, 0, &p, &c)) return rc;
  *rows = c.cs_rows; *pitch = c.cs_pitch;
  return MTBT_OK;
}

extern "C" int mtbt_conv_kernel_choice(const mtbt_conv_args* a, int32_t* choice) {
  if (!a || !choice) return MTBT_EINVAL;
  ConvP p;
  ConvChoice c;
  if (const int rc = conv_plan(a, 0, &p, &c)) return rc;
  conv_report(c, choice);
  return MTBT_OK;
}

static bool batch_same_shape(const mtbt_conv_args& a, const mtbt_conv_args& b) {
  return a.N == b.N && a.H == b.H && a.W == b.W && a.C == b.C && a.K == b.K && a.R == b.R && a.S == b.S && a.stride == b.stride && a.pad == b.pad &&
         a.Ho == b.Ho && a.Wo == b.Wo && a.dtype == b.dtype && a.out_dtype == b.out_dtype && a.act == b.act && a.out_mode == b.out_mode &&
         a.tile_hint == b.tile_hint && a.policy == b.policy && a.debug == b.debug && !a.scale == !b.scale && !a.shift == !b.shift && !a.res == !b.res;
}

static bool batch_outputs_overlap(const mtbt_conv_args& a, const mtbt_conv_args& b) {
  const long oes = a.out_dtype == MTBT_F32 ? 4 : 2;
  const long ext_a = ((long)(a.N - 1) * a.y_batch_stride + ((long)a.Ho * a.Wo - 1) * a.y_pixel_stride + a.K) * oes;
  const long ext_b = ((long)(b.N - 1) * b.y_batch_stride + ((long)b.Ho * b.Wo - 1) * b.y_pixel_stride + b.K) * oes;
  const char* ya = reinterpret_cast<const char*>(a.y);
  const char* yb = reinterpret_cast<const char*>(b.y);
  if (ya + ext_a <= yb || yb + ext_b <= ya) return false;
  const long ld = a.y_pixel_stride;
  if (ld != b.y_pixel_stride || a.y_batch_stride != b.y_batch_stride || ld <= 0 || a.y_batch_stride % ld != 0) return true;
  const long db = yb - ya;
  if (db % oes != 0) return true;
  const long r = ((db / oes) % ld + ld) % ld;
  return !(r >= a.K && r + a.K <= ld);
}


static int conv_batch_impl(const mtbt_conv_args* calls, int n, void* stream, int32_t* choice) {
  if (!calls || n < 1 || n > MTBT_CONV_BATCH_MAX) return MTBT_EINVAL;
  ConvBatchP b;
  ConvChoice c0;
  for (int i = 0; i < n; ++i) {
    const mtbt_conv_args& a = calls[i];
    if (a.y2 || a.colsum || a.colsum_ws || a.out_mode != MTBT_OUT_NHWC) return MTBT_EINVAL;
    if (i && !batch_same_shape(calls[0], a)) return MTBT_EINVAL;
    ConvP p;
    ConvChoice c;
    if (const int rc = conv_plan(&a, n, &p, &c)) return rc;
    if (i == 0) { b.p = p; c0 = c; }
    else if (c.kind != c0.kind || c.TC != c0.TC || c.TP != c0.TP || c.wide != c0.wide || c.row_reuse != c0.row_reuse) return MTBT_EINVAL;
    ConvMember& m = b.m[i];
    m.x = p.x; m.w = p.w; m.y = p.y; m.scale = p.scale; m.shift = p.shift; m.res = p.res;
    m.xbs = p.xbs; m.ybs = p.ybs; m.rbs = p.rbs; m.ldx = p.ldx; m.ldy = p.ldy; m.ldr = p.ldr;
    m.vec_ok = p.vec_ok; m.y_linear = p.y_linear; m.pad_ = 0;
    for (int j = 0; j < i; ++j)
      if (batch_outputs_overlap(calls[j], a)) return MTBT_EINVAL;
  }
  for (int i = n; i < MTBT_CONV_BATCH_MAX; ++i) b.m[i] = b.m[0];
  if (c0.kind == CONV_IGEMM && !(c0.wide && conv_tile_batched(c0.TC, c0.TP))) return MTBT_EINVAL;
  if (c0.kind == CONV_DIRECT3X3 && !(c0.TC == 64 && c0.row_reuse)) return MTBT_EINVAL;
  if (choice) { conv_report(c0, choice); return MTBT_OK; }
  hipStream_t s = reinterpret_cast<hipStream_t>(stream);
  if (c0.kind == CONV_PW_STREAM) return mtbt_pw_stream_batch(b, n, calls[0].dtype, s);
  return conv_unit(calls[0].dtype).batch(b, n, c0, s);
}

extern "C" int mtbt_conv2d_nhwc_batch(const mtbt_conv_args* calls, int n, void* stream) { return conv_batch_impl(calls, n, stream, nullptr); }

extern "C" int mtbt_conv_batch_kernel_choice(const mtbt_conv_args* calls, int n, int32_t* choice) {
  if (!choice) return MTBT_EINVAL;
  return conv_batch_impl(calls, n, nullptr, choice);
}
```

multitask_bonetumor_yolo_amd/csrc/conv_igemm.inc:

```
#pragma once
#include "common.h"
#include "conv_params.h"
#include "conv_tiles.h"
#include "conv_dma.h"
#include "conv_epilogue.h"

namespace {


template <int CPR> __device__ __forceinline__ int swz(int row) {
  if constexpr (CPR == 4) return (-(row >> 2)) & 3;
  else return (row >> 1) & 7;
}

template <typename T, int TC, int TP, int WAVES_C, int WAVES_P, int BKB, int NBUF>
__global__ __launch_bounds__(256, 2) void conv_igemm_kernel(const ConvP p) {
  const unsigned bid = blockIdx.x;
#include "conv_igemm_body.inc"
}

#ifdef MTBT_CONV_BATCH_UNIT
template <typename T, int TC, int TP, int WAVES_C, int WAVES_P, int BKB, int NBUF>
__global__ __launch_bounds__(256, 2) void conv_igemm_batch_kernel(const ConvBatchP b) {
  const ConvP p = conv_member(b, (int)blockIdx.y);
  const unsigned bid = blockIdx.x;
#include "conv_igemm_body.inc"
}
#endif

template <int TC, int TP, int WAVES_C, int BKB, int NBUF, typename Kernel, typename Params>
int launch_tile(Kernel kernel, Params q, int n, hipStream_t stream) {
  constexpr int CPR = BKB / 16;
  constexpr int TCS = ((TC * CPR + 255) / 256) * 256 / CPR;
  constexpr int lds_main = NBUF * (TCS + TP) * BKB;
  constexpr int lds_epi = 2 * 4 * 16 * ((TC / WAVES_C) * 4 + 16);
  constexpr int lds = (lds_main > lds_epi ? lds_main : lds_epi) + 2 * TC * 4;
  static_assert(lds <= 160 * 1024, "this (tile, depth) does not fit the CU's 160 KiB of LDS");
  return conv_launch_tiles(kernel, q, TC, ((long)conv_of(q).M + TP - 1) / TP, n, lds, stream);
}

template <typename T, int BKB, int NBUF>
int dispatch_tile(const ConvP& p, int TC, int TP, hipStream_t s) {
#define MTBT_X(tc, tp, wc, wp, batched) \
  if (TC == tc && TP == tp) return launch_tile<tc, tp, wc, BKB, NBUF>(conv_igemm_kernel<T, tc, tp, wc, wp, BKB, NBUF>, p, 1, s);
  MTBT_CONV_TILES(MTBT_X)
#undef MTBT_X
  return MTBT_EINVAL;
}

#ifdef MTBT_CONV_BATCH_UNIT
template <typename T>
int dispatch_tile_batch(const ConvBatchP& b, int n, int TC, int TP, hipStream_t s) {
#define MTBT_X(tc, tp, wc, wp, batched) \
  if constexpr (batched) { if (TC == tc && TP == tp) return launch_tile<tc, tp, wc, 128, 2>(conv_igemm_batch_kernel<T, tc, tp, wc, wp, 128, 2>, b, n, s); }
  MTBT_CONV_TILES(MTBT_X)
#undef MTBT_X
  return MTBT_EINVAL;
}
#endif

}
```

multitask_bonetumor_yolo_amd/csrc/conv_igemm_body.inc:

```
  constexpr int EPC = 16 / (int)sizeof(T);
  constexpr int CPR = BKB / 16;
  constexpr int BKE = BKB / (int)sizeof(T);
  constexpr int WC = TC / WAVES_C, WP = TP / WAVES_P;
  constexpr int FC = WC / 16, FP = WP / 16;
  constexpr int TCS = ((TC * CPR + 255) / 256) * 256 / CPR;
  constexpr int WCH = TCS * CPR / 256, XCH = TP * CPR / 256;
  static_assert(WCH * 256 == TCS * CPR && XCH * 256 == TP * CPR, "whole wave-instructions");
  constexpr int KSUB = BKB / 64;
  constexpr int BUF = (TCS + TP) * BKB;
  constexpr int G = WCH + XCH;
  constexpr int D = NBUF - 1;
  static_assert(WAVES_C * WAVES_P == 4, "4 waves");
  static_assert(WC % 16 == 0 && WP % 16 == 0, "wave tile");

  extern __shared__ __attribute__((aligned(16))) char smem[];
  constexpr int EPI = 2 * 4 * 16 * ((TC / WAVES_C) * 4 + 16);
  constexpr int AFF_OFF = (NBUF * BUF > EPI) ? NBUF * BUF : EPI;
  float* aff = reinterpret_cast<float*>(smem + AFF_OFF);

  const int tid = threadIdx.x;
  const int slot = bid >> 3, xcd = bid & 7;
  const int ctile = slot % p.ctiles;
  const int ptile = xcd * p.ptiles_per_xcd + slot / p.ctiles;
  if ((long)ptile * TP >= p.M) return;
  const int cbase = ctile * TC;
  const int pbase = ptile * TP;
  const int HoWo = p.Ho * p.Wo;
  const int Kdim = p.R * p.S * p.C;
  stage_affine<TC>(p, aff, cbase, tid);

  constexpr unsigned OOB = 0x80000000u;
  const int wave_u = __builtin_amdgcn_readfirstlane(tid >> 6);
  const int n_first = pbase / HoWo;
  const long padoff = ((long)p.pad * p.W + p.pad) * p.ldx;
  const srd_t xsrd = make_srd(reinterpret_cast<const T*>(p.x) + ((long)n_first * p.xbs - padoff));
  const srd_t wsrd = make_srd(reinterpret_cast<const T*>(p.w) + (long)cbase * Kdim);
  const unsigned lds0 = (unsigned)(size_t)(__attribute__((address_space(3))) char*)smem;
  unsigned xvoff[XCH], xmask[XCH];
  const bool flat = p.R * p.S == 1 && p.stride == 1 && p.pad == 0 && p.xbs == (long)HoWo * p.ldx;
#pragma unroll
  for (int i = 0; i < XCH; ++i) {
    const int c = tid + i * 256;
    const int row = c / CPR, q = (c % CPR) ^ swz<CPR>(row);
    const int pix = pbase + row;
    const bool ok = pix < p.M;
    if (flat) {
      xmask[i] = ok ? 1u : 0u;
      xvoff[i] = ok ? (unsigned)(((long)(pix - n_first * HoWo) * p.ldx + q * EPC) * (long)sizeof(T)) : OOB;
      continue;
    }
    const int pp = ok ? pix : pbase;
    const int n = pp / HoWo;
    const int rem = pp - n * HoWo;
    const int oy = rem / p.Wo, ox = rem - oy * p.Wo;
    const int iy0 = oy * p.stride - p.pad, ix0 = ox * p.stride - p.pad;
    xvoff[i] = (unsigned)(((long)(n - n_first) * p.xbs + ((long)iy0 * p.W + ix0) * p.ldx + padoff + q * EPC) * (long)sizeof(T));
    unsigned m = 0;
    for (int r = 0; r < p.R; ++r)
      for (int s2 = 0; s2 < p.S; ++s2)
        if ((unsigned)(iy0 + r) < (unsigned)p.H && (unsigned)(ix0 + s2) < (unsigned)p.W) m |= 1u << (r * p.S + s2);
    xmask[i] = ok ? m : 0u;
    if (p.R * p.S == 1 && !(m & 1u && ok)) xvoff[i] = OOB;
  }
  constexpr bool PERM = (FC % 2 == 0);
  unsigned wvoff[WCH];
#pragma unroll
  for (int i = 0; i < WCH; ++i) {
    const int c = tid + i * 256;
    const int row = c / CPR, q = (c % CPR) ^ swz<CPR>(row);
    const int srow = PERM ? (row / WC) * WC + epi_row_channel(row % WC) : row;
    const bool ok = (row < TC) && (cbase + srow < p.K);
    wvoff[i] = ok ? (unsigned)(((long)srow * Kdim + q * EPC) * (long)sizeof(T)) : OOB;
  }

  const int wave = tid >> 6, lane = tid & 63;
  const int wc = wave / WAVES_P, wp = wave % WAVES_P;
  const int lr = lane & 15, lq = lane >> 4;
  int abase[KSUB], bbase[KSUB];
#pragma unroll
  for (int ks = 0; ks < KSUB; ++ks) {
    const int arow = wc * WC + lr, brow = wp * WP + lr;
    abase[ks] = arow * BKB + (((ks * 4 + lq) ^ swz<CPR>(arow)) << 4);
    bbase[ks] = TCS * BKB + brow * BKB + (((ks * 4 + lq) ^ swz<CPR>(brow)) << 4);
  }

  f32x4 acc[FC][FP];
#pragma unroll
  for (int i = 0; i < FC; ++i)
#pragma unroll
    for (int j = 0; j < FP; ++j) acc[i][j] = f32x4{0.f, 0.f, 0.f, 0.f};

  int kr = 0, ks_ = 0, kc = 0;
  int kw = 0;
  const int nsteps = Kdim / BKE;

  const bool single_tap = (p.R * p.S == 1);
  auto stage_tile = [&](int bufidx) {
    const int tap = kr * p.S + ks_;
    const int xsoff = (int)((((long)kr * p.W + ks_) * p.ldx + kc) * (long)sizeof(T));
    const int wsoff = kw * (int)sizeof(T);
    const unsigned base = lds0 + bufidx * BUF + wave_u * 1024;
#pragma unroll
    for (int i = 0; i < XCH; ++i) {
      const unsigned vo = (single_tap || ((xmask[i] >> tap) & 1u)) ? xvoff[i] : OOB;
      lds_dma16(xsrd, vo, xsoff, base + TCS * BKB + i * 4096);
    }
#pragma unroll
    for (int i = 0; i < WCH; ++i) lds_dma16(wsrd, wvoff[i], wsoff, base + i * 4096);
    kw += BKE;
    kc += BKE;
    if (kc == p.C) { kc = 0; if (++ks_ == p.S) { ks_ = 0; ++kr; } }
  };

#pragma unroll
  for (int d = 0; d < D; ++d)
    if (d < nsteps) stage_tile(d);

  for (int t0 = 0; t0 < nsteps; t0 += NBUF) {
#pragma unroll
    for (int u = 0; u < NBUF; ++u) {
      const int t = t0 + u;
      if (t >= nsteps) break;
      wait_stages<G, D - 1>(nsteps - 1 - t);
      lds_barrier();
      if (t + D < nsteps && !MTBT_ABL(p, 1)) stage_tile((u + D) % NBUF);
      if (MTBT_ABL(p, 2)) continue;
      const char* cur = smem + u * BUF;
#pragma unroll
      for (int ks = 0; ks < KSUB; ++ks) {
        uint4 a[FC], b[FP];
#pragma unroll
        for (int f = 0; f < FC; ++f) a[f] = MTBT_ABL(p, 8) ? uint4{1u, 2u, 3u, (unsigned)f} : *reinterpret_cast<const uint4*>(cur + abase[ks] + f * 16 * BKB);
#pragma unroll
        for (int f = 0; f < FP; ++f) b[f] = MTBT_ABL(p, 8) ? uint4{1u, 2u, 3u, (unsigned)f} : *reinterpret_cast<const uint4*>(cur + bbase[ks] + f * 16 * BKB);
        if (MTBT_ABL(p, 4)) {
#pragma unroll
          for (int f = 0; f < FC; ++f) { const unsigned z = a[f].x ^ a[f].y ^ a[f].z ^ a[f].w; asm volatile("" ::"v"(z)); }
#pragma unroll
          for (int f = 0; f < FP; ++f) { const unsigned z = b[f].x ^ b[f].y ^ b[f].z ^ b[f].w; asm volatile("" ::"v"(z)); }
          continue;
        }
#pragma unroll
        for (int i = 0; i < FC; ++i)
#pragma unroll
          for (int j = 0; j < FP; ++j) {
            if constexpr (sizeof(T) == 2) {
              acc[i][j] = mfma_16x16x32<T>(a[i], b[j], acc[i][j]);
            } else {
              acc[i][j] = __builtin_amdgcn_mfma_f32_16x16x4f32(__uint_as_float(a[i].x), __uint_as_float(b[j].x), acc[i][j], 0, 0, 0);
              acc[i][j] = __builtin_amdgcn_mfma_f32_16x16x4f32(__uint_as_float(a[i].y), __uint_as_float(b[j].y), acc[i][j], 0, 0, 0);
              acc[i][j] = __builtin_amdgcn_mfma_f32_16x16x4f32(__uint_as_float(a[i].z), __uint_as_float(b[j].z), acc[i][j], 0, 0, 0);
              acc[i][j] = __builtin_amdgcn_mfma_f32_16x16x4f32(__uint_as_float(a[i].w), __uint_as_float(b[j].w), acc[i][j], 0, 0, 0);
            }
          }
      }
    }
  }
  __syncthreads();
  if (MTBT_ABL(p, 16)) return;

  const int Cq = p.K >> 2;
  const EpiSeq seq{(long)pbase + wp * WP, 16, (long)p.M, 0, 0};
  conv_epilogue<T, TC, FC, FP, true, 1, (sizeof(T) == 2), PERM>(p, acc, smem + wave * (2 * 16 * (WC * 4 + 16)), aff, cbase, wc * WC, lane,
                               [&](int j, int row, int ch, long& yoff, long& roff) -> bool {
    const int pix = pbase + wp * WP + j * 16 + row;
    if (pix >= p.M) return false;
    if (p.y_linear) {
      yoff = (long)pix * p.ldy + ch;
      roff = (long)pix * p.ldr + ch;
    } else if (p.out_mode == MTBT_OUT_CONVT2X2) {
      const int n = pix / HoWo, rem = pix - n * HoWo;
      const int oy = rem / p.Wo, ox = rem - oy * p.Wo;
      const int quad = ch / Cq, chout = ch - quad * Cq;
      const long opix = (long)(2 * oy + (quad >> 1)) * (2 * p.Wo) + (2 * ox + (quad & 1));
      yoff = (long)n * p.ybs + opix * p.ldy + chout;
      roff = (long)n * p.rbs + opix * p.ldr + chout;
    } else {
      const int n = pix / HoWo, rem = pix - n * HoWo;
      yoff = (long)n * p.ybs + (long)rem * p.ldy + ch;
      roff = (long)n * p.rbs + (long)rem * p.ldr + ch;
    }
    return true;
  }, seq, p.y_linear != 0, (long)ptile * WAVES_P + wp);
```

multitask_bonetumor_yolo_amd/csrc/conv_params.h:

```cpp
#pragma once

struct ConvP {
  const void* x;
  const void* w;
  void* y;
  const float* scale;
  const float* shift;
  const void* res;
  void* y2;
  long xbs, ybs, rbs;
  int ldx, ldy, ldr;
  int N, H, W, C, K, R, S, stride, pad, Ho, Wo;
  int act, out_mode, out_f32, vec_ok;
  int y_linear;
  int M;
  int ctiles;
  int ptiles_per_xcd;
  float* cs_part;
  const float* cs_shift;
  int cs_sq, cs_pitch;
  int debug;
};

#ifdef MTBT_CONV_ABLATION
#define MTBT_ABL(p, bit) ((p).debug & (bit))
#else
#define MTBT_ABL(p, bit) 0
#endif

#define MTBT_CONV_BATCH_MAX 8
struct ConvMember {
  const void* x;
  const void* w;
  void* y;
  const float* scale;
  const float* shift;
  const void* res;
  long xbs, ybs, rbs;
  int ldx, ldy, ldr;
  int vec_ok, y_linear, pad_;
};

struct ConvBatchP {
  ConvP p;
  ConvMember m[MTBT_CONV_BATCH_MAX];
};

#if defined(__HIPCC__)
inline ConvP& conv_of(ConvP& p) { return p; }
inline ConvP& conv_of(ConvBatchP& b) { return b.p; }
template <typename Kernel, typename Params>
int conv_launch_tiles(Kernel kernel, Params& q, int TC, long ptiles, int n, int lds, hipStream_t stream) {
  ConvP& p = conv_of(q);
  p.ctiles = (p.K + TC - 1) / TC;
  p.ptiles_per_xcd = (int)((ptiles + 7) / 8);
  const long blocks = (long)p.ptiles_per_xcd * 8 * p.ctiles;
  if (blocks <= 0 || blocks > 0x7fffffffL || n < 1 || n > MTBT_CONV_BATCH_MAX) return MTBT_EINVAL;
  if (int rc = mtbt_allow_lds(kernel, lds)) return rc;
  hipLaunchKernelGGL(kernel, dim3((unsigned)blocks, (unsigned)n), dim3(256), lds, stream, q);
  MTBT_LAUNCH_CHECK();
  return MTBT_OK;
}

__device__ __forceinline__ ConvP conv_member(const ConvBatchP& b, int i) {
  ConvP p = b.p;
  const ConvMember& m = b.m[i];
  p.x = m.x; p.w = m.w; p.y = m.y; p.scale = m.scale; p.shift = m.shift; p.res = m.res;
  p.xbs = m.xbs; p.ybs = m.ybs; p.rbs = m.rbs;
  p.ldx = m.ldx; p.ldy = m.ldy; p.ldr = m.ldr;
  p.vec_ok = m.vec_ok; p.y_linear = m.y_linear;
  return p;
}
#endif
```

multitask_bonetumor_yolo_amd/engine.py:

```python
import ctypes as C
import os
from contextlib import contextmanager
from dataclasses import dataclass
from typing import Callable, List, Optional

import torch

from . import _lib as L

TORCH_DTYPE = {L.F32: torch.float32, L.BF16: torch.bfloat16, L.F16: torch.float16}
ESIZE = {L.F32: 4, L.BF16: 2, L.F16: 2}


def code_of(dtype: torch.dtype) -> int:
    if dtype == torch.float32:
        return L.F32
    if dtype == torch.bfloat16:
        return L.BF16
    if dtype == torch.float16:
        return L.F16
    raise ValueError(f"unsupported compute dtype {dtype}: float32 (parity), bfloat16 (throughput) or float16 (inference, BASELINE configs[4])")


@dataclass
# ... 386 lines not shown
        return arr

    def _conv_args(self, x, w, y, R, S, stride, pad, scale, shift, act, res, out_mode, tile_hint, policy):
        K = w.shape[0]
        assert w.shape[1] == R * S * x.C, (w.shape, R, S, x.C)
        Ho = (x.H + 2 * pad - R) // stride + 1
        Wo = (x.W + 2 * pad - S) // stride + 1
        a = L.ConvArgs()
        a.x, a.w, a.y = x.ptr, w.data_ptr(), y.ptr
        a.scale = scale.data_ptr() if scale is not None else None
        a.shift = shift.data_ptr() if shift is not None else None
        a.res = res.ptr if res is not None else None
        a.x_batch_stride, a.x_pixel_stride = x.batch_stride, x.ld
        a.y_batch_stride = y.batch_stride
        a.y_pixel_stride = y.ld
        a.res_batch_stride = res.batch_stride if res is not None else 0
        a.res_pixel_stride = res.ld if res is not None else 0
        a.N, a.H, a.W, a.C, a.K, a.R, a.S = x.N, x.H, x.W, x.C, K, R, S
        a.stride, a.pad, a.Ho, a.Wo = stride, pad, Ho, Wo
        a.dtype, a.out_dtype, a.act, a.out_mode, a.tile_hint = x.code, y.code, act, out_mode, tile_hint
        a.policy, a.debug = self.call_policy(policy), self.conv_debug
        flops = 2.0 * x.N * Ho * Wo * K * R * S * x.C
        byts = (x.N * x.H * x.W * x.C + K * R * S * x.C) * ESIZE[x.code] + x.N * Ho * Wo * K * ESIZE[y.code]
        return a, flops, byts

    def stem(self, x_nchw: torch.Tensor, w, b, lnw, lnb, eps, y: Act, name="stem"):
        N, _, H, W = x_nchw.shape
        args = (x_nchw.data_ptr(), w.data_ptr(), b.data_ptr(), lnw.data_ptr(), lnb.data_ptr(), C.c_float(eps), y.ptr,
                N, H, W, y.C, y.code)
        self.launches.append(Launch(self.lib.mtbt_stem_conv4x4_ln, args, name, (x_nchw, w, b, lnw, lnb, y.buf),
                                    2.0 * N * (H // 4) * (W // 4) * y.C * 48,
                                    N * 3 * H * W * 4 + N * (H // 4) * (W // 4) * y.C * ESIZE[y.code]))
        self._io([], [y])

    def dwconv(self, x: Act, w, y: Act, ksize, *, bias=None, lnw=None, lnb=None, eps=0.0, scale=None, shift=None,
               act=L.ACT_NONE, name="dwconv"):
        assert x.dense and y.dense
        p = lambda t: t.data_ptr() if t is not None else None
        if y.C != x.C:
            M = y.C // x.C
            assert ksize == 3 and y.C == M * x.C and bias is None and lnw is None and scale is not None and shift is not None
            args = (x.ptr, w.data_ptr(), p(scale), p(shift), act, y.ptr, x.N, x.H, x.W, x.C, M, x.code)
            n = x.N * x.H * x.W
            self.launches.append(Launch(self.lib.mtbt_dwconv3x3_mult_nhwc, args, name, (x.buf, w, scale, shift, y.buf),
                                        2.0 * n * y.C * 9, 1.0 * n * (x.C + y.C) * ESIZE[x.code]))
            self._io([x, w], [y])
            return
        args = (x.ptr, w.data_ptr(), p(bias), p(lnw), p(lnb), C.c_float(eps), p(scale), p(shift), act, y.ptr,
                x.N, x.H, x.W, x.C, ksize, x.code)
        n = x.N * x.H * x.W * x.C
        self.launches.append(Launch(self.lib.mtbt_dwconv_nhwc, args, name, (x.buf, w, bias, lnw, lnb, scale, shift, y.buf),
                                    2.0 * n * ksize * ksize, 2.0 * n * ESIZE[x.code]))
        self._io([x, w], [y])

    def layernorm(self, x: Act, w, b, eps, y: Act, name="layernorm"):
        assert x.dense and y.dense
        pixels = x.N * x.H * x.W
        args = (x.ptr, w.data_ptr(), b.data_ptr(), C.c_float(eps), y.ptr, pixels, x.C, x.code)
        self.launches.append(Launch(self.lib.mtbt_layernorm_nhwc, args, name, (x.buf, w, b, y.buf), 0.0,
                                    2.0 * pixels * x.C * ESIZE[x.code]))
        self._io([x], [y])

    def fuse(self, inputs, weights, modes, y: Act, bug=False, name="bifpn_fuse", wgt_dev: Optional[torch.Tensor] = None, wgt_first=0):
        a = L.FuseArgs()
        for i, (t, wv, m) in enumerate(zip(inputs, weights, modes)):
            assert t.dense
            a.x[i], a.wgt[i], a.resample[i] = t.ptr, float(wv), m
        a.n_in, a.y = len(inputs), y.ptr
        a.N, a.H, a.W, a.C, a.dtype, a.add_weight_bug = y.N, y.H, y.W, y.C, y.code, int(bug)
        if wgt_dev is not None:
            a.wgt_dev = wgt_dev.data_ptr() + 4 * wgt_first
        n = y.N * y.H * y.W * y.C
        self.launches.append(Launch(self.lib.mtbt_bifpn_fuse, (C.byref(a),), name, (a, y.buf, wgt_dev) + tuple(t.buf for t in inputs),
                                    0.0, n * ESIZE[y.code] * (1 + len(inputs))))
        self._io(list(inputs) + [wgt_dev], [y])
        return a

    def gap_fc(self, x: Act, w, b, y: torch.Tensor, name="gap_fc"):
        assert x.dense
        args = (x.ptr, w.data_ptr(), b.data_ptr() if b is not None else None, y.data_ptr(), x.N, x.H * x.W, x.C,
                w.shape[0], x.code)
        self.launches.append(Launch(self.lib.mtbt_gap_fc, args, name, (x.buf, w, b, y), 0.0,
                                    x.N * x.H * x.W * x.C * ESIZE[x.code]))
        self._io([x], [y])

    def bn_train(self, x: Act, y: Act, bn, act, name="bn_train"):
        assert x.dense and y.dense and x.C == y.C and x.code == y.code
        if bn.momentum is None:
            raise NotImplementedError("BatchNorm2d(momentum=None) (cumulative average) is not supported")
        pixels = x.N * x.H * x.W
        nbytes = self.lib.mtbt_bn_train_workspace_bytes(pixels, x.C)
        ws = torch.empty((nbytes // 4,), dtype=torch.float32, device=self.device)
        rm = bn.running_mean.data_ptr() if bn.running_mean is not None else None
        rv = bn.running_var.data_ptr() if bn.running_var is not None else None
        g, b = self.const(bn.weight, torch.float32), self.const(bn.bias, torch.float32)
        args = (x.ptr, y.ptr, g.data_ptr(), b.data_ptr(), rm, rv, C.c_float(bn.momentum), C.c_float(bn.eps), act, pixels, x.C,
                x.code, ws.data_ptr(), nbytes)
        self.launches.append(Launch(self.lib.mtbt_bn_train_nhwc, args, name, (x.buf, y.buf, g, b, ws, bn), 0.0,
                                    3.0 * pixels * x.C * ESIZE[x.code]))
        self._io([x], [y])

    def cast(self, x: Act, y: Act, name="cast"):
        assert x.dense and y.dense
        n = x.N * x.H * x.W * x.C
        self.launches.append(Launch(self.lib.mtbt_cast, (x.ptr, y.ptr, n, x.code, y.code), name, (x.buf, y.buf), 0.0,
                                    n * (ESIZE[x.code] + ESIZE[y.code])))
        self._io([x], [y])

    def mlp_fused(self, t: Act, res: Act, w1, b1, w2p, b2, y: Act, name="mlp"):
        assert t.dense and res.dense and y.dense and t.code in (L.BF16, L.F16) and t.C in (96, 192, 384)
        M, D = t.N * t.H * t.W, t.C
        args = (t.ptr, res.ptr, w1.data_ptr(), b1.data_ptr(), w2p.data_ptr(), b2.data_ptr(), y.ptr, M, D, t.code)
        self.launches.append(Launch(self.lib.mtbt_convnext_mlp_fused_dt, args, name, (t.buf, res.buf, w1, b1, w2p, b2, y.buf),
                                    2.0 * M * D * 4 * D * 2, 3.0 * M * D * 2 + 2.0 * 4 * D * D * 2))
        self._io([t, res], [y])

    def node(self, inputs, weights, modes, w: torch.Tensor, shift: torch.Tensor, y: Act, act=L.ACT_ELU, name="bifpn_node"):
        K, Cin = w.shape
        assert y.C == K and y.bs == y.H * y.W * y.ld and all(t.dense and t.C == Cin for t in inputs)
        a = L.NodeArgs()
        for i, (t, wv, m) in enumerate(zip(inputs, weights, modes)):
            a.fuse.x[i], a.fuse.wgt[i], a.fuse.resample[i] = t.ptr, float(wv), m
        a.fuse.n_in = len(inputs)
        a.fuse.N, a.fuse.H, a.fuse.W, a.fuse.C, a.fuse.dtype, a.fuse.add_weight_bug = y.N, y.H, y.W, Cin, y.code, 0
        a.w, a.shift, a.y, a.y_pixel_stride, a.K, a.act = w.data_ptr(), shift.data_ptr(), y.ptr, y.ld, K, act
        n = y.N * y.H * y.W
        self.launches.append(Launch(self.lib.mtbt_bifpn_node_nhwc, (C.byref(a),), name, (a, w, shift, y.buf) + tuple(t.buf for t in inputs),
                                    2.0 * n * K * Cin, n * (K + Cin * len(inputs)) * ESIZE[y.code]))
        self._io(list(inputs) + [w, shift], [y])
        return a

    def pw_chain_args(self, x: Act, w1: torch.Tensor, shift1, act1, w2: torch.Tensor, shift2, act2, y: Act, any_size=False):
        if not (x.dense and y.bs == y.H * y.W * y.ld and (x.N, x.H, x.W) == (y.N, y.H, y.W)) or x.code not in (L.BF16, L.F16):
            return None
        a = L.PwChainArgs()
        a.x, a.w1, a.w2, a.y = x.ptr, w1.data_ptr(), w2.data_ptr(), y.ptr
        a.shift1 = shift1.data_ptr() if shift1 is not None else None
        a.shift2 = shift2.data_ptr() if shift2 is not None else None
        a.pixels, a.y_pixel_stride = x.N * x.H * x.W, y.ld
        a.C, a.M, a.K = x.C, w1.shape[0], w2.shape[0]
        a.dtype, a.out_dtype, a.act1, a.act2 = x.code, y.code, act1, act2
        if w1.shape[1] != x.C or w2.shape[1] != w1.shape[0] or y.C != w2.shape[0]:
            return None
        return a if self.lib.mtbt_pw_chain_supported(C.byref(a)) in ((1, 2) if any_size else (1,)) else None

    def pw_chain(self, a, x: Act, w1, shift1, w2, shift2, y: Act, name="pw_chain"):
        n = x.N * x.H * x.W
        Cin, M, K = x.C, w1.shape[0], w2.shape[0]
        self.launches.append(Launch(self.lib.mtbt_pw_chain_nhwc, (C.byref(a),), name, (a, x.buf, w1, shift1, w2, shift2, y.buf),
                                    2.0 * n * (M * Cin + K * M), (n * Cin + M * Cin + K * M) * ESIZE[x.code] + n * K * ESIZE[y.code]))
        self._io([x, w1, shift1, w2, shift2], [y])
        return a

    def upconv(self, x: Act, w: torch.Tensor, shift9: torch.Tensor, y: Act, act=L.ACT_SILU, name="upconv"):
        K = w.shape[0] // 4
        assert w.shape[1] == 4 * x.C and tuple(shift9.shape) == (9, K) and y.C == K and y.H == 2 * x.H and y.W == 2 * x.W and x.code == y.code
        a = L.UpconvArgs()
        a.x, a.w, a.y, a.shift = x.ptr, w.data_ptr(), y.ptr, shift9.data_ptr()
        a.x_batch_stride, a.y_batch_stride, a.x_pixel_stride, a.y_pixel_stride = x.batch_stride, y.batch_stride, x.ld, y.ld
        a.N, a.H, a.W, a.C, a.K, a.dtype, a.act = x.N, x.H, x.W, x.C, K, x.code, act
        flops = 2.0 * x.N * x.H * x.W * 4 * K * 4 * x.C
        byts = (x.N * x.H * x.W * x.C + 16 * K * x.C + 4 * x.N * x.H * x.W * K) * ESIZE[x.code]
        self.launches.append(Launch(self.lib.mtbt_convt2x2_conv3x3_nhwc, (C.byref(a),), name, (a, x.buf, w, shift9, y.buf), flops, byts))
        self._io([x, w, shift9], [y])
        return a

    def raw(self, fn, args, name, keep=(), reads=(), writes=()):
        self.launches.append(Launch(fn, args, name, keep))
        self._io(list(reads), list(writes))

    def _io(self, reads, writes):
        l = self.launches[-1]
        l.reads = tuple(_region(a) for a in reads if a is not None)
        l.writes = tuple(_region(a) for a in writes if a is not None)
```

multitask_bonetumor_yolo_amd/graphed.py:

```python
import torch

from . import postprocess as pp


AUTOTUNE_KNOBS = (("PW_CHAIN", ("1",)), ("NODE_FUSED", ("1",)), ("SEG_GATE", ("1", "2")), ("LANE_WIDE_US", ("200",)), ("LANES", ("3",)), ("ADAPTOR_EARLY", ("1",)),
                  ("HEADS_EARLY", ("1",)))


class GraphedInference:
    def __init__(self, model, x: torch.Tensor, img_size: int, conf_th=pp.CONF_TH, iou_th=pp.NMS_IOU, top_k=pp.TOP_K, masks=True,
                 warmup: int = 2, autotune: bool = False, log=None):
        if autotune:
            import time
            opts = dict(model.__dict__.get("plan_options", {}))

            def timed(o):
                model.plan_options = o
                g = GraphedInference(model, x, img_size, conf_th, iou_th, top_k, masks, warmup=1)
                for _ in range(3):
                    g.replay()
                torch.cuda.synchronize(x.device)
                t0 = time.perf_counter()
                for _ in range(12):
                    g.replay()
                torch.cuda.synchronize(x.device)
                dt = (time.perf_counter() - t0) / 12
                del g
                model.__dict__.get("_plans", {}).clear()
                return dt
            timed(dict(opts))
            best = timed(dict(opts))
            if log:
                log(f"autotune: defaults {best * 1e3:.3f} ms")
            for name, values in AUTOTUNE_KNOBS:
                for v in values:
                    cand = dict(opts, **{name: v})
                    t = timed(cand)
                    if log:
                        log(f"autotune: {name}={v} {t * 1e3:.3f} ms" + (" *" if t < best * 0.995 else ""))
                    if t < best * 0.995:
                        best, opts = t, cand
            model.plan_options = opts
            model.__dict__.get("_plans", {}).clear()
            if log:
                log(f"autotune: kept {opts} ({best * 1e3:.3f} ms)")
        if not x.is_cuda or x.dtype != torch.float32 or not x.is_contiguous():
            raise ValueError("GraphedInference needs a contiguous fp32 CUDA/HIP batch [B,3,S,S] (it is read in place)")
        self.model, self.x = model, x
        self._compiled = None
        self.args = (img_size, conf_th, iou_th, top_k, masks)
        from .engine import reserved_stream
        self.stream = reserved_stream(x.device, "graph_capture")
        self.side = reserved_stream(x.device, "graph_side")
        self.graph = torch.cuda.CUDAGraph()
        self.stream.wait_stream(torch.cuda.current_stream(x.device))
        with torch.cuda.stream(self.stream), torch.no_grad():
            for _ in range(warmup):
                self._step()
            torch.cuda.synchronize(x.device)
            with torch.cuda.graph(self.graph, stream=self.stream, capture_error_mode="thread_local"):
                self.fwd, self.out = self._step()
            with model._heads_mode(False):
                self._compiled = model.compile(x)
            self._sig = self._compiled.sig
        torch.cuda.current_stream(x.device).wait_stream(self.stream)

    def _step(self):
        img_size, conf_th, iou_th, top_k, masks = self.args
        return self.model.infer_and_detect(self.x, img_size, conf_th, iou_th, top_k, masks, side_stream=self.side,
                                           own_outputs=False)

    def replay(self):
        self.graph.replay()
        if self.model._weights_sig(self.model._bn_modes(heads_eval=True)) != self._sig:
            raise RuntimeError("GraphedInference: the model's weights / BatchNorm statistics changed since the capture (the graph replays "
                               "kernels over the OLD folded weights): build a new GraphedInference")
        return self.out
```

multitask_bonetumor_yolo_amd/model.py:

```python
import ctypes as C
import math
import os
from contextlib import contextmanager
from typing import List

import torch
import torch.nn as nn

from . import _lib as L
from .engine import Act, Plan, code_of, TORCH_DTYPE, reserved_stream

BN_MOMENTUM, BN_EPS = 0.9997, 4e-5
LN_EPS = 1e-6
DEPTHS, DIMS = (3, 3, 9, 3), (96, 192, 384, 768)


class _Params(nn.Module):

    def forward(self, *a, **k):
        raise RuntimeError(f"{type(self).__name__} is a parameter container of the HIP launch plan; "
                           "call the top-level ConvNeXtBiFPNYOLO.forward")


class ConvBlock(_Params):
# ... 69 lines not shown
        self.norm = nn.LayerNorm(d, eps=LN_EPS)
        self.mlp = _Mlp(d)
        self.gamma = nn.Parameter(1e-6 * torch.ones(d))


class _CNStage(_Params):
    def __init__(self, cin, cout, depth, downsample):
        super().__init__()
        self.downsample = (nn.Sequential(nn.LayerNorm(cin, eps=LN_EPS), nn.Conv2d(cin, cout, 2, 2))
                           if downsample else nn.Identity())
        self.blocks = nn.Sequential(*[_CNBlock(cout) for _ in range(depth)])


class _CNFeatures(_Params):
    def __init__(self):
        super().__init__()
        self.stem_0 = nn.Conv2d(3, DIMS[0], 4, 4)
        self.stem_1 = nn.LayerNorm(DIMS[0], eps=LN_EPS)
        prev = DIMS[0]
        for i, (d, n) in enumerate(zip(DIMS, DEPTHS)):
            setattr(self, f"stages_{i}", _CNStage(prev, d, n, i > 0))
            prev = d


class ConvNeXtTiny(_Params):

    def __init__(self, pretrained: bool = True):
        super().__init__()
        if pretrained:
            raise RuntimeError("pretrained_backbone=True would download timm weights (main_model.py:21-26); there is "
                               "no network: build with pretrained_backbone=False and load_state_dict() a checkpoint")
        self.body = _CNFeatures().eval()
        self.c2f_p3 = C2f(192, 256)
        self.c2f_p4 = C2f(384, 384)
        self.c2f_p5 = C2f(768, 512)
        self.out_channels = list(DIMS[1:])


class _UConv(_Params):
    def __init__(self, c1, c2, k=1, g=1):
        super().__init__()
        self.conv = nn.Conv2d(c1, c2, k, 1, k // 2, groups=g, bias=False)
        self.bn = nn.BatchNorm2d(c2)
        self.act = nn.SiLU()


class _DFL(_Params):
    def __init__(self, c1=16):
        super().__init__()
        self.conv = nn.Conv2d(c1, 1, 1, bias=False).requires_grad_(False)
        self.conv.weight.data[:] = torch.arange(c1, dtype=torch.float).view(1, c1, 1, 1)
        self.c1 = c1


class _Proto(_Params):
    def __init__(self, c1, c_=256, c2=32):
        super().__init__()
        self.cv1 = _UConv(c1, c_, 3)
        self.upsample = nn.ConvTranspose2d(c_, c_, 2, 2, 0, bias=True)
        self.cv2 = _UConv(c_, c_, 3)
        self.cv3 = _UConv(c_, c2)


class Detect(_Params):
    def __init__(self, nc=80, ch=()):
        super().__init__()
        self.nc, self.nl, self.reg_max = nc, len(ch), 16
        self.no = nc + self.reg_max * 4
        self.stride = torch.zeros(self.nl)
        c2 = max(16, ch[0] // 4, self.reg_max * 4)
        c3 = max(ch[0], min(nc, 100))
        self.cv2 = nn.ModuleList(
            nn.Sequential(_UConv(x, c2, 3), _UConv(c2, c2, 3), nn.Conv2d(c2, 4 * self.reg_max, 1)) for x in ch)
        self.cv3 = nn.ModuleList(
            nn.Sequential(nn.Sequential(_UConv(x, x, 3, g=x), _UConv(x, c3, 1)),
                          nn.Sequential(_UConv(c3, c3, 3, g=c3), _UConv(c3, c3, 1)),
                          nn.Conv2d(c3, nc, 1)) for x in ch)
        self.dfl = _DFL(self.reg_max)


class Segment(Detect):
    def __init__(self, nc=80, nm=32, npr=256, ch=()):
        super().__init__(nc, ch)
        self.nm, self.npr = nm, npr
        self.proto = _Proto(ch[0], npr, nm)
        c4 = max(ch[0] // 4, nm)
        self.cv4 = nn.ModuleList(
            nn.Sequential(_UConv(x, c4, 3), _UConv(c4, c4, 3), nn.Conv2d(c4, nm, 1)) for x in ch)


def _bn_fold(bn: nn.BatchNorm2d, conv_bias=None):
    scale = bn.weight.detach().float() / torch.sqrt(bn.running_var.float() + bn.eps)
    shift = bn.bias.detach().float() - bn.running_mean.float() * scale
    if conv_bias is not None:
        shift = shift + conv_bias.detach().float() * scale
    return scale, shift


def _permute_hidden(w2: torch.Tensor) -> torch.Tensor:
    kk = torch.arange(32)
    g, j = kk // 8, kk % 8
    within = torch.where(j < 4, 4 * g + j, 16 + 4 * g + (j - 4))
    idx = (torch.arange(w2.shape[1] // 32)[:, None] * 32 + within[None, :]).reshape(-1)
    return w2[:, idx.to(w2.device)].contiguous()


def _krsc(w: torch.Tensor) -> torch.Tensor:
    return w.detach().permute(0, 2, 3, 1).reshape(w.shape[0], -1)


def compose_upconv(wt: torch.Tensor, bt: torch.Tensor, w3: torch.Tensor, scale: torch.Tensor, shift: torch.Tensor):
    wt, bt, w3 = wt.detach().double(), bt.detach().double(), w3.detach().double() * scale.detach().double()[:, None, None, None]
    K, Ci = w3.shape[0], wt.shape[0]
    w = torch.zeros(2, 2, K, 2, 2, Ci, dtype=torch.float64, device=w3.device)
    for a in range(2):
        for b in range(2):
            for dy in (-1, 0, 1):
                for dx in (-1, 0, 1):
                    rho, sy = (a + dy) // 2 - (a - 1), (a + dy) % 2
                    sig, sx = (b + dx) // 2 - (b - 1), (b + dx) % 2
                    w[a, b, :, rho, sig, :] += w3[:, :, dy + 1, dx + 1] @ wt[:, :, sy, sx].t()
    tapb = torch.einsum("kcyx,c->kyx", w3, bt)
    valid = {0: (1, 2), 1: (0, 1, 2), 2: (0, 1)}
    shift9 = torch.stack([shift.detach().double() + tapb[:, list(valid[rc])][:, :, list(valid[cc])].sum(dim=(1, 2)) for rc in range(3) for cc in range(3)])
    return w.reshape(4 * K, 4 * Ci).float(), shift9.float()


def fold_dwblock(mod: DepthwiseConvBlock):
    dw = mod.depthwise.weight.detach().float().reshape(1, -1)
    pw = mod.pointwise.weight.detach().float().reshape(mod.pointwise.out_channels, -1) * dw
    scale, shift = _bn_fold(mod.bn)
    return pw * scale[:, None], shift


def pack_convblocks(mods):
    ws, shs = [], []
    for m in mods:
        scale, shift = _bn_fold(m.bn, m.conv.bias)
        ws.append(_krsc(m.conv.weight).float() * scale[:, None])
        shs.append(shift)
    return torch.cat(ws, 0), torch.cat(shs, 0)


def pack_dwblocks(mods):
    ws, scs, shs = [], [], []
    for m in mods:
        scale, shift = _bn_fold(m.bn)
        ws.append(m.conv.weight.detach().reshape(m.conv.out_channels, 9).t())
        scs.append(scale)
        shs.append(shift)
    return torch.cat(ws, 1).contiguous(), torch.cat(scs, 0), torch.cat(shs, 0)


PLAN_OPTION_DEFAULTS = {"NODE_FUSED": "0", "ADAPTOR_EARLY": "0", "HEADS_EARLY": "0", "SEG_GATE": "0", "HEADS_MERGED": "0", "PW_CHAIN": "0", "LANES": None, "LANE_WIDE_US": None}


def plan_option(model, name: str):
    v = model.__dict__.get("plan_options", {}).get(name)
    if v is None:
        v = os.environ.get("MTBT_" + name, PLAN_OPTION_DEFAULTS[name])
    return v


class _Lowering:

    def __init__(self, model, shape, device, code: int):
        self.m = model
        self.code = code
        self.dt = TORCH_DTYPE[code]
        self.device = device
        self.p = Plan(device)
        self.x = torch.empty(tuple(shape), dtype=torch.float32, device=device)
        self.train_bns = []

    def W(self, t):
        return self.p.const(t.float(), self.dt)

    def F(self, t):
        return self.p.const(t.float(), torch.float32)

    def _bn_batch_stats(self, raw: Act, bn, act, y, name):
        if y is not None and not y.dense:
            raise NotImplementedError(f"{name}: batch-statistic BatchNorm into a channel slice (C2f concat buffer) is not lowered; "
                                      "only the Detect/Segment heads run in train mode inside forward(mode='train')")
        self.train_bns.append(bn)
        if y is None or y.code == raw.code:
            out = y if y is not None else raw
            self.p.bn_train(raw, out, bn, act, name=name + ".bn(batch)")
            if out is not raw:
                self.p.release(raw)
            return out
        self.p.bn_train(raw, raw, bn, act, name=name + ".bn(batch)")
        self.p.cast(raw, y, name=name + ".cast")
        self.p.release(raw)
        return y

    def convblock(self, x: Act, mod, y: Act = None, name=""):
        conv, bn = mod.conv, mod.bn
        k = conv.kernel_size[0]
        if bn.training:
            raw = self.p.new(x.N, x.H, x.W, conv.out_channels, self.code)
            self.p.conv(x, self.W(_krsc(conv.weight)), raw, R=k, S=k, stride=1, pad=k // 2,
                        shift=self.F(conv.bias) if conv.bias is not None else None, name=name)
            return self._bn_batch_stats(raw, bn, L.ACT_SILU, y, name)
        scale, shift = _bn_fold(bn, conv.bias)
        if y is None:
            y = self.p.new(x.N, x.H, x.W, conv.out_channels, self.code)
        self.p.conv(x, self.W(_krsc(conv.weight).float() * scale[:, None]), y, R=k, S=k, stride=1, pad=k // 2,
                    shift=self.F(shift), act=L.ACT_SILU, name=name)
        return y

    def conv_plain(self, x: Act, conv: nn.Conv2d, y: Act, name=""):
        k = conv.kernel_size[0]
        self.p.conv(x, self.W(_krsc(conv.weight)), y, R=k, S=k, stride=conv.stride[0], pad=conv.padding[0],
                    shift=self.F(conv.bias) if conv.bias is not None else None, name=name)
        return y

    def dwblock(self, x: Act, mod: _UConv, name=""):
        w = self.W(mod.conv.weight.detach().reshape(x.C, 9).t())
        y = self.p.new(x.N, x.H, x.W, x.C, self.code)
        if mod.bn.training:
            one, zero = self.F(torch.ones(x.C)), self.F(torch.zeros(x.C))
            self.p.dwconv(x, w, y, 3, scale=one, shift=zero, act=L.ACT_NONE, name=name)
            return self._bn_batch_stats(y, mod.bn, L.ACT_SILU, None, name)
        scale, shift = _bn_fold(mod.bn)
        self.p.dwconv(x, w, y, 3, scale=self.F(scale), shift=self.F(shift), act=L.ACT_SILU, name=name)
        return y

    def pw_pair(self, x: Act, first, second, y: Act, name) -> bool:
        n0 = len(self.p.consts)
        (w1, s1, a1), (w2, s2, a2) = first, second
        w1, w2 = self.W(w1), self.W(w2)
        s1, s2 = (self.F(s1) if s1 is not None else None), (self.F(s2) if s2 is not None else None)
        a = self.p.pw_chain_args(x, w1, s1, a1, w2, s2, a2, y, any_size=plan_option(self.m, "PW_CHAIN") == "2")
        if a is None:
            del self.p.consts[n0:]
            return False
        self.p.pw_chain(a, x, w1, s1, w2, s2, y, name=name)
        return True

    def pw_chain_on(self, *bns) -> bool:
        return plan_option(self.m, "PW_CHAIN") in ("1", "2") and self.code in (L.BF16, L.F16) and not any(bn.training for bn in bns)

    def c2f(self, x: Act, mod: C2f, name="", cv1=None):
        c, n = mod.c, len(mod.m)
        cat = self.p.new(x.N, x.H, x.W, (2 + n) * c, self.code)
        if cv1 is not None:
            cv1(cat.slice(0, 2 * c))
        else:
            self.convblock(x, mod.cv1, cat.slice(0, 2 * c), name + ".cv1")
        prev = cat.slice(c, c)
        for i, b in enumerate(mod.m):
            if b.add:
                raise NotImplementedError("Bottleneck shortcut is never enabled by the reference model")
            t = self.convblock(prev, b.cv1, None, f"{name}.m.{i}.cv1")
            dst = cat.slice((2 + i) * c, c)
            self.convblock(t, b.cv2, dst, f"{name}.m.{i}.cv2")
            self.p.release(t)
            prev = dst
        y = self.convblock(cat, mod.cv2, None, name + ".cv2")
        self.p.release(cat)
        return y

    def dw_pointwise(self, x: Act, mod: DepthwiseConvBlock, name=""):
        if mod.bn.training:
            raise NotImplementedError(f"{name}: BiFPN DepthwiseConvBlock with batch-statistic BatchNorm (model.train()) is not lowered yet")
        w, shift = fold_dwblock(mod)
        y = self.p.new(x.N, x.H, x.W, w.shape[0], self.code)
        self.p.conv(x, self.W(w), y, shift=self.F(shift), act=L.ACT_ELU, name=name)
        return y

    @staticmethod
    def fused_dims():
        env = os.environ.get("MTBT_FUSED_DIMS")
        return tuple(int(v) for v in env.replace(":", ",").split(",")) if env else (96, 192, 384)

    def backbone(self):
        bb = self.m.backbone
        early = plan_option(self.m, "ADAPTOR_EARLY") == "1"
        mods = {1: (bb.c2f_p3, "backbone.c2f_p3"), 2: (bb.c2f_p4, "backbone.c2f_p4"), 3: (bb.c2f_p5, "backbone.c2f_p5")}
        outs = {}

        def hook(si, a):
            if early:
                with self.p.branch(side=si < 3):
                    outs[si] = self.c2f(a, *mods[si])
        feats = self.features(bb.body, hook)
        if not early:
            for si in (1, 2, 3):
                outs[si] = self.c2f(feats[si - 1], *mods[si])
        for f in feats:
            self.p.release(f)
        return outs[1], outs[2], outs[3]

    def features(self, body, on_feature=None):
        N, _, H, W = self.x.shape
        a = self.p.new(N, H // 4, W // 4, DIMS[0], self.code)
        self.p.stem(self.x, self.F(body.stem_0.weight.detach().reshape(DIMS[0], 48)), self.F(body.stem_0.bias),
                    self.F(body.stem_1.weight), self.F(body.stem_1.bias), body.stem_1.eps, a, name="backbone.body.stem")
        feats = []
        for si in range(4):
            st = getattr(body, f"stages_{si}")
            nm = f"backbone.body.stages_{si}"
            if si > 0:
                ln, cv = st.downsample[0], st.downsample[1]
                t = self.p.new(a.N, a.H, a.W, a.C, self.code)
                self.p.layernorm(a, self.F(ln.weight), self.F(ln.bias), ln.eps, t, name=nm + ".downsample.0")
# ... 10 lines not shown
            h = None if fused else self.p.new(a.N, a.H, a.W, 4 * d, self.code)
            pp_ = [self.p.new(a.N, a.H, a.W, d, self.code) for _ in range(2)] if len(st.blocks) > 1 else []
            consts = []
            for blk in st.blocks:
                g = blk.gamma.detach().float()
                consts.append((self.W(blk.conv_dw.weight.detach().reshape(d, 49).t()), self.F(blk.conv_dw.bias), self.F(blk.norm.weight),
                               self.F(blk.norm.bias), self.W(blk.mlp.fc1.weight), self.F(blk.mlp.fc1.bias),
                               self.W(blk.mlp.fc2.weight.detach().float() * g[:, None]), self.F(g * blk.mlp.fc2.bias.detach().float())))
            w2p = [self.p.const(_permute_hidden(c_[6]), self.dt) for c_ in consts] if fused else None
            gelu = L.ACT_GELU_POLY if self.code in (L.BF16, L.F16) else L.ACT_GELU
            cur = a
            for bi, blk in enumerate(st.blocks):
                bn_ = f"{nm}.blocks.{bi}"
                dww, dwb, lnw, lnb, w1, b1, w2, b2 = consts[bi]
                self.p.dwconv(cur, dww, t, 7, bias=dwb, lnw=lnw, lnb=lnb, eps=blk.norm.eps, name=bn_ + ".conv_dw+norm")
                dst = out if bi == len(st.blocks) - 1 else pp_[bi % 2]
                if fused:
                    self.p.mlp_fused(t, cur, w1, b1, w2p[bi], b2, dst, name=bn_ + ".mlp(fused)")
                else:
                    self.p.conv(t, w1, h, shift=b1, act=gelu, name=bn_ + ".mlp.fc1")
                    self.p.conv(h, w2, dst, shift=b2, res=cur, name=bn_ + ".mlp.fc2")
                cur = dst
            for buf in [t] + ([] if h is None else [h]) + pp_:
                self.p.release(buf)
            self.p.release(a)
            a = out
            if si >= 1:
                feats.append(a)
                if on_feature is not None:
                    on_feature(si, a)
        return feats

    def neck_v0(self, f3, f4, f5):
        nk = self.m.neck
        p3 = self.convblock(f3, nk.lat3, None, "neck.lat3")
        p4 = self.convblock(f4, nk.lat4, None, "neck.lat4")
        p5 = self.convblock(f5, nk.lat5, None, "neck.lat5")
        for t in (f3, f4, f5):
            self.p.release(t)
        for ui, u in enumerate(nk.units):
            nm = f"neck.units.{ui}"

            def node(add, inputs, modes, like: Act, key):
                w = torch.relu(add.w.detach().float().cpu())
                w = w / (w.sum() + add.eps)
                s_ = self.p.new(like.N, like.H, like.W, like.C, self.code)
                self.p.fuse(inputs, [float(v) for v in w], modes, s_, bug=True, name=f"{nm}.add_{key}")
                o = self.dwblock(s_, u.conv[key], f"{nm}.conv.{key}")
                self.p.release(s_)
                return o

            p4_td = node(u.add_p4_td, [p4, p5], [L.RES_ID, L.RES_UP_NEAREST], p4, "p4_td")
            p3_td = node(u.add_p3_td, [p3, p4_td], [L.RES_ID, L.RES_UP_NEAREST], p3, "p3_td")
            p4_out = node(u.add_p4_out, [p4, p4_td, p3_td], [L.RES_ID, L.RES_ID, L.RES_MAXPOOL], p4, "p4_out")
            p5_out = node(u.add_p5_out, [p5, p4_out], [L.RES_ID, L.RES_MAXPOOL], p5, "p5_out")
            for t in (p3, p4, p5, p4_td):
                self.p.release(t)
            p3, p4, p5 = p3_td, p4_out, p5_out
        return p3, p4, p5

    @staticmethod
    def _norm_w(w, eps):
        w = torch.nn.functional.elu(w.detach().float().cpu())
        return w / (w.sum(dim=0, keepdim=True) + eps)

    def neck(self, c3, c4, c5, on_level=None):
        nk = self.m.neck
        p3 = self.convblock(c3, nk.p3_proj, None, "neck.p3_proj")
        p4 = self.convblock(c4, nk.p4_proj, None, "neck.p4_proj")
        p5 = self.convblock(c5, nk.p5_proj, None, "neck.p5_proj")
        for t in (c3, c4, c5):
            self.p.release(t)
        for ui, u in enumerate(nk.bifpn_units):
            nm = f"neck.bifpn_units.{ui}"
            a, b = self._norm_w(u.w1, u.eps), self._norm_w(u.w2, u.eps)

            def node(inputs, weights, modes, like: Act, conv, cf, tag):
                K = conv.pointwise.out_channels
                shapes = ([L.RES_ID, L.RES_UP_BILINEAR], [L.RES_ID, L.RES_ID, L.RES_DOWN_MEAN])
                if (self.code in (L.BF16, L.F16) and like.C in (128, 256) and K == like.C and list(modes) in shapes and not conv.bn.training
                        and plan_option(self.m, "NODE_FUSED") == "1"):
                    w, shift = fold_dwblock(conv)
                    d = self.p.new(like.N, like.H, like.W, K, self.code)
                    self.p.node(inputs, [float(v) for v in weights], modes, self.W(w), self.F(shift), d, act=L.ACT_ELU,
                                name=f"{nm}.{tag}.fuse+conv")
                else:
                    s = self.p.new(like.N, like.H, like.W, like.C, self.code)
                    self.p.fuse(inputs, [float(v) for v in weights], modes, s, name=f"{nm}.{tag}.fuse")
                    c1 = cf.cv1.conv
                    if self.pw_chain_on(conv.bn, cf.cv1.bn) and c1.kernel_size == (1, 1) and K == like.C:
                        def cv1(dst):
                            sc, sh = _bn_fold(cf.cv1.bn, c1.bias)
                            if self.pw_pair(s, fold_dwblock(conv) + (L.ACT_ELU,), (_krsc(c1.weight).float() * sc[:, None], sh, L.ACT_SILU), dst,
                                            f"{nm}.{tag}_conv+cf.cv1"):
                                return
                            d = self.dw_pointwise(s, conv, f"{nm}.{tag}_conv")
                            self.convblock(d, cf.cv1, dst, f"{nm}.{tag}_cf.cv1")
                            self.p.release(d)
                        o = self.c2f(s, cf, f"{nm}.{tag}_cf", cv1=cv1)
                        self.p.release(s)
                        return o
                    d = self.dw_pointwise(s, conv, f"{nm}.{tag}_conv")
                    self.p.release(s)
                o = self.c2f(d, cf, f"{nm}.{tag}_cf")
                self.p.release(d)
                return o

            last = on_level is not None and ui == len(nk.bifpn_units) - 1
            p4_td = node([p4, p5], [a[0, 0], a[1, 0]], [L.RES_ID, L.RES_UP_BILINEAR], p4, u.p4_td_conv, u.p4_td_cf, "p4_td")
            p3_td = node([p3, p4_td], [a[0, 1], a[1, 1]], [L.RES_ID, L.RES_UP_BILINEAR], p3, u.p3_td_conv, u.p3_td_cf, "p3_td")
            if last:
                on_level(0, p3_td)
            p4_out = node([p4, p4_td, p3_td], [b[0, 0], b[1, 0], b[2, 0]], [L.RES_ID, L.RES_ID, L.RES_DOWN_MEAN], p4,
                          u.p4_out_conv, u.p4_out_cf, "p4_out")
            if last:
                on_level(1, p4_out)
            p5_out = node([p5, p5, p4_out], [b[0, 1], b[1, 1], b[2, 1]], [L.RES_ID, L.RES_ID, L.RES_DOWN_MEAN], p5,
                          u.p5_out_conv, u.p5_out_cf, "p5_out")
            if last:
                on_level(2, p5_out)
            for t in (p3, p4, p5, p4_td):
                self.p.release(t)
            p3, p4, p5 = p3_td, p4_out, p5_out
        return p3, p4, p5

    def f32_out(self, N, H, W, Cc) -> Act:
        return Act.of(torch.empty((N, H, W, Cc), dtype=torch.float32, device=self.device))

    def head_map(self, f: Act, head: Detect) -> Act:
        ld = (head.no + 3) // 4 * 4
        buf = torch.empty((f.N, f.H, f.W, ld), dtype=torch.float32, device=self.device)
        return Act(buf, 0, f.N, f.H, f.W, head.no, ld, f.H * f.W * ld)

    def cls_chain(self, i, f: Act, head: Detect, tag, dst: Act):
        s = head.cv3[i]
        d1 = self.dwblock(f, s[0][0], f"{tag}.cv3.{i}.0.0")
        t1 = self.convblock(d1, s[0][1], None, f"{tag}.cv3.{i}.0.1")
        self.p.release(d1)
        d2 = self.dwblock(t1, s[1][0], f"{tag}.cv3.{i}.1.0")
        self.p.release(t1)
        c1, c2 = s[1][1].conv, s[2]
        if (self.pw_chain_on(s[1][1].bn) and not self.merged and c1.kernel_size == (1, 1) and c2.kernel_size == (1, 1) and c2.stride == (1, 1)
                and c2.padding == (0, 0)):
            sc, sh = _bn_fold(s[1][1].bn, c1.bias)
            if self.pw_pair(d2, (_krsc(c1.weight).float() * sc[:, None], sh, L.ACT_SILU), (_krsc(c2.weight), c2.bias, L.ACT_NONE), dst,
                            f"{tag}.cv3.{i}.1.1+2"):
                self.p.release(d2)
                return
        t2 = self.convblock(d2, s[1][1], None, f"{tag}.cv3.{i}.1.1")
        self.p.release(d2)
        self.conv_plain(t2, s[2], dst, f"{tag}.cv3.{i}.2")
        self.p.release(t2)

    def conv_chain(self, f: Act, s, name, dst: Act):
        t1 = self.convblock(f, s[0], None, name + ".0")
        t2 = self.convblock(t1, s[1], None, name + ".1")
        self.p.release(t1)
        self.conv_plain(t2, s[2], dst, name + ".2")
        self.p.release(t2)

    def det_level(self, i, f: Act, head: Detect, tag, full: Act, gate=None):
        first = len(self.p.launches)
        self.cls_chain(i, f, head, tag, full.slice(4 * head.reg_max, head.nc))
        box = len(self.p.launches)
        self.conv_chain(f, head.cv2[i], f"{tag}.cv2.{i}", full.slice(0, 4 * head.reg_max))
        if gate:
            self.p.amend(first, reads=gate)
            self.p.amend(box, reads=gate)

    def heads_mergeable(self, i, heads, f: Act) -> bool:
        seg = heads[-1][0]
        if not isinstance(seg, Segment) or f.C % 128 or not f.dense:
            return False
        mods = [m for h, _ in heads for br in (h.cv2[i], h.cv3[i]) for m in br.modules()] + list(seg.cv4[i].modules())
        if any(m.training for m in mods if isinstance(m, nn.BatchNorm2d)):
            return False
        c2 = {h.cv2[i][0].conv.out_channels for h, _ in heads} | {seg.cv4[i][0].conv.out_channels}
        c3 = {h.cv3[i][0][1].conv.out_channels for h, _ in heads}
        same = len(c2) == 1 and len(c3) == 1 and len({(h.nc, h.reg_max, h.no) for h, _ in heads}) == 1
        return same and c3 == {f.C} and all(h.cv3[i][1][0].conv.groups == f.C for h, _ in heads)

    def _batch(self, members, name, **kw):
        names = name.split(" + ")
        if len(members) > 1:
            first = len(self.p.launches)
            arr = self.p.conv_batch(members, name=name, **kw)
            choice = (C.c_int32 * 4)()
            if self.p.lib.mtbt_conv_batch_kernel_choice(C.cast(arr, C.c_void_p), len(members), choice) == 0:
                return
            del self.p.launches[first:]
        for (x, w, y, shift), nm in zip(members, names):
            self.p.conv(x, w, y, shift=shift, name=nm, **{k: v for k, v in kw.items()})

    def heads_level_merged(self, i, f: Act, heads, maps):
        seg = heads[-1][0]
        nh, c2, c3 = len(heads), seg.cv4[i][0].conv.out_channels, f.C
        N, H, W = f.N, f.H, f.W

        def box_chains():
            firsts = [h.cv2[i][0] for h, _ in heads] + [seg.cv4[i][0]]
            tags = [f"{t}.cv2.{i}" for _, t in heads] + [f"segment.cv4.{i}"]
            w1, sh1 = pack_convblocks(firsts)
            t1 = self.p.new(N, H, W, w1.shape[0], self.code)
            self.p.conv(f, self.W(w1), t1, R=3, S=3, pad=1, shift=self.F(sh1), act=L.ACT_SILU, name=" + ".join(f"{t}.0" for t in tags),
                        policy=32 if w1.shape[0] % 128 else 0)
            t2 = self.p.new(N, H, W, w1.shape[0], self.code)
            seconds = [h.cv2[i][1] for h, _ in heads] + [seg.cv4[i][1]]
            members = []
            for j, m in enumerate(seconds):
                wj, sj = pack_convblocks([m])
                members.append((t1.slice(j * c2, c2), self.W(wj), t2.slice(j * c2, c2), self.F(sj)))
            self._batch(members, " + ".join(f"{t}.1" for t in tags), R=3, S=3, pad=1, act=L.ACT_SILU)
            self.p.release(t1)
            outs = [h.cv2[i][2] for h, _ in heads]
            self._batch([(t2.slice(j * c2, c2), self.W(_krsc(cv.weight)), maps[j].slice(0, 4 * h.reg_max), self.F(cv.bias))
                         for j, ((h, _), cv) in enumerate(zip(heads, outs))], " + ".join(f"{t}.cv2.{i}.2" for _, t in heads))
            self.conv_plain(t2.slice(nh * c2, c2), seg.cv4[i][2], self.mc_level(i, f), f"segment.cv4.{i}.2")
            self.p.release(t2)

        if nh == 1:
            h, t = heads[0]
            self.cls_chain(i, f, h, t, maps[0].slice(4 * h.reg_max, h.nc))
            return box_chains()
        ctags = [f"{t}.cv3.{i}" for _, t in heads]
        wd, scd, shd = pack_dwblocks([h.cv3[i][0][0] for h, _ in heads])
        d1 = self.p.new(N, H, W, nh * c3, self.code)
        self.p.dwconv(f, self.W(wd), d1, 3, scale=self.F(scd), shift=self.F(shd), act=L.ACT_SILU, name=" + ".join(f"{t}.0.0" for t in ctags))
        u1 = self.p.new(N, H, W, nh * c3, self.code)

        def pointwise(src, dst, k):
            members = []
            for j, (h, _) in enumerate(heads):
                wj, sj = pack_convblocks([h.cv3[i][k][1]])
                members.append((src.slice(j * c3, c3), self.W(wj), dst.slice(j * c3, c3), self.F(sj)))
            self._batch(members, " + ".join(f"{t}.{k}.1" for t in ctags), act=L.ACT_SILU)
        pointwise(d1, u1, 0)
        self.p.release(d1)
        wd, scd, shd = pack_dwblocks([h.cv3[i][1][0] for h, _ in heads])
        d2 = self.p.new(N, H, W, nh * c3, self.code)
        self.p.dwconv(u1, self.W(wd), d2, 3, scale=self.F(scd), shift=self.F(shd), act=L.ACT_SILU, name=" + ".join(f"{t}.1.0" for t in ctags))
        self.p.release(u1)
        u2 = self.p.new(N, H, W, nh * c3, self.code)
        pointwise(d2, u2, 1)
        self.p.release(d2)
        self._batch([(u2.slice(j * c3, c3), self.W(_krsc(h.cv3[i][2].weight)), maps[j].slice(4 * h.reg_max, h.nc), self.F(h.cv3[i][2].bias))
                     for j, (h, _) in enumerate(heads)], " + ".join(f"{t}.2" for t in ctags))
        self.p.release(u2)
        box_chains()

    def mc_buffer(self, shapes, head: Segment):
        N = shapes[0][0]
        A = sum(h * w for _, h, w in shapes)
        offs, off = [], 0
        for _, h, w in shapes:
            offs.append(off)
            off += h * w
        return torch.empty((N, A, head.nm), dtype=torch.float32, device=self.device), offs, A

    def mc_level(self, i, f: Act) -> Act:
        nm = self.m.segment.nm
        return Act(self.mc, self.offs[i] * nm, f.N, f.H, f.W, nm, nm, self.A * nm)

    def proto(self, f: Act, head: Segment) -> Act:
        pr = head.proto
        t1 = self.convblock(f, pr.cv1, None, "segment.proto.cv1")
        if not pr.cv2.bn.training and f.H % 16 == 0 and f.W % 16 == 0 and pr.cv2.conv.out_channels % 128 == 0:
            sc, sh = _bn_fold(pr.cv2.bn)
            wc, shift9 = compose_upconv(pr.upsample.weight, pr.upsample.bias, pr.cv2.conv.weight, sc, sh)
            t2 = self.p.new(f.N, 2 * f.H, 2 * f.W, pr.cv2.conv.out_channels, self.code)
            self.p.upconv(t1, self.W(wc), self.F(shift9), t2, act=L.ACT_SILU, name="segment.proto.upsample+cv2")
            self.p.release(t1)
        else:
            up = self.p.new(f.N, 2 * f.H, 2 * f.W, pr.upsample.out_channels, self.code)
            wt = pr.upsample.weight.detach()
            self.p.conv(t1, self.W(wt.permute(2, 3, 1, 0).reshape(4 * wt.shape[1], wt.shape[0])), up,
                        shift=self.F(pr.upsample.bias.detach().repeat(4)), out_mode=L.OUT_CONVT2X2, name="segment.proto.upsample")
            self.p.release(t1)
            t2 = self.convblock(up, pr.cv2, None, "segment.proto.cv2")
            self.p.release(up)
        protos = self.f32_out(f.N, 2 * f.H, 2 * f.W, head.nm)
        self.convblock(t2, pr.cv3, protos, "segment.proto.cv3")
        self.p.release(t2)
        return protos

    def cls_head(self, n5: Act):
        logits = torch.empty((n5.N, self.m.cls_fc.out_features), dtype=torch.float32, device=self.device)
        self.p.gap_fc(n5, self.F(self.m.cls_fc.weight), self.F(self.m.cls_fc.bias), logits, name="cls_pool+cls_fc")
        return logits

    def level_heads(self, i, f: Act):
        seg = self.m.segment
        with self.p.branch(side=self.early, reuse=False):
            if i == 0:
                self.protos = self.proto(f, seg)
            maps = [self.head_map(f, h) for h, _ in self.heads]
            if self.merged and self.heads_mergeable(i, self.heads, f):
                self.heads_level_merged(i, f, self.heads, maps)
            else:
                for (h, tag), full in zip(self.heads[:-1], maps):
                    self.det_level(i, f, h, tag, full)
                self.conv_chain(f, seg.cv4[i], f"segment.cv4.{i}", self.mc_level(i, f))
                self.det_level(i, f, seg, "segment", maps[-1], maps[:-1] if self.gate else None)
        if self.det_maps is not None:
            self.det_maps[i] = maps[0]
        self.seg_maps[i] = maps[-1]

    def lower(self, sig=None) -> "_Compiled":
        m, p = self.m, self.p
# ... 381 lines not shown
```

Before: 2756 images/s.

## Fuse 3x3 conv with trailing 1x1 projection in detect-head conv chains

Adds a conv-tail kernel variant (both igemm and direct row-reuse 3x3 paths) that keeps the 64-channel SiLU output of the middle conv in LDS and applies the final 1x1 conv with bias via MFMA, writing fp32 head outputs directly. This removes the intermediate activation write/read and one launch per head branch. The path is gated behind a new TAIL_CHAIN plan option that defaults off, though it is added to the autotune knob list. Risk is extra register pressure from preloaded second-stage weights and restriction to K=64 tiles.

Measured after the change: 2723 images/s. 0.988x the previous value.

```diff
diff --git a/include/mtbt_hip.h b/include/mtbt_hip.h
--- a/include/mtbt_hip.h
+++ b/include/mtbt_hip.h
@@ -136,6 +136,19 @@
 int mtbt_pw_chain_supported(const mtbt_pw_chain_args* a);
 int mtbt_sizeof_pw_chain_args(void);
 
+typedef struct mtbt_conv_tail_args {
+  mtbt_conv_args conv;
+  const void* w2;
+  const float* bias2;
+  float* y;
+  int64_t y_batch_stride;
+  int32_t y_pixel_stride;
+  int32_t K2;
+} mtbt_conv_tail_args;
+int mtbt_conv2d_tail_nhwc(const mtbt_conv_tail_args* a, void* stream);
+int mtbt_conv_tail_supported(const mtbt_conv_tail_args* a);
+int mtbt_sizeof_tail_chain_args(int which);
+
 int64_t mtbt_bn_train_workspace_bytes(int64_t pixels, int C);
 int mtbt_bn_train_nhwc(const void* x, void* y, const float* gamma, const float* beta, float* running_mean,
                        float* running_var, float momentum, float eps, int act, int64_t pixels, int C, int dtype,
diff --git a/multitask_bonetumor_yolo_amd/_lib.py b/multitask_bonetumor_yolo_amd/_lib.py
--- a/multitask_bonetumor_yolo_amd/_lib.py
+++ b/multitask_bonetumor_yolo_amd/_lib.py
@@ -48,6 +48,11 @@
     _fields_ = [("x", C.c_void_p), ("w1", C.c_void_p), ("scale1", C.c_void_p), ("shift1", C.c_void_p), ("w2", C.c_void_p), ("scale2", C.c_void_p),
                 ("shift2", C.c_void_p), ("y", C.c_void_p), ("pixels", C.c_int64), ("y_pixel_stride", C.c_int32), ("C", C.c_int32), ("M", C.c_int32),
                 ("K", C.c_int32), ("dtype", C.c_int32), ("out_dtype", C.c_int32), ("act1", C.c_int32), ("act2", C.c_int32)]
+
+
+class ConvTailArgs(C.Structure):
+    _fields_ = [("conv", ConvArgs), ("w2", C.c_void_p), ("bias2", C.c_void_p), ("y", C.c_void_p), ("y_batch_stride", C.c_int64),
+                ("y_pixel_stride", C.c_int32), ("K2", C.c_int32)]
 
 
 class UpconvArgs(C.Structure):
@@ -258,6 +263,9 @@
     "mtbt_pw_chain_nhwc": (C.c_int, [C.POINTER(PwChainArgs), C.c_void_p]),
     "mtbt_pw_chain_supported": (C.c_int, [C.POINTER(PwChainArgs)]),
     "mtbt_sizeof_pw_chain_args": (C.c_int, []),
+    "mtbt_conv2d_tail_nhwc": (C.c_int, [C.POINTER(ConvTailArgs), C.c_void_p]),
+    "mtbt_conv_tail_supported": (C.c_int, [C.POINTER(ConvTailArgs)]),
+    "mtbt_sizeof_tail_chain_args": (C.c_int, [C.c_int]),
     "mtbt_bn_train_workspace_bytes": (C.c_int64, [C.c_int64, C.c_int]),
     "mtbt_bn_train_nhwc": (C.c_int, [C.c_void_p] * 6 + [C.c_float, C.c_float, C.c_int, C.c_int64, C.c_int, C.c_int, C.c_void_p,
                                       C.c_int64, C.c_void_p]),
@@ -394,6 +402,7 @@
 COMPONENTS_STRUCTS = (ComponentsArgs, SelectComponentsArgs)
 POLYGON_STRUCTS = (FillPolygonsArgs,)
 CLAHE_STRUCTS = (ClaheImage,)
+TAIL_CHAIN_STRUCTS = (ConvTailArgs,)
 _lib = None
 
 
@@ -417,7 +426,7 @@
         for sizeof, structs in ((lib.mtbt_sizeof_frame_args, FRAME_STRUCTS), (lib.mtbt_sizeof_mask_eval_args, MASK_EVAL_STRUCTS),
                                 (lib.mtbt_sizeof_tile_args, TILE_STRUCTS), (lib.mtbt_sizeof_surface_args, SURFACE_STRUCTS),
                                 (lib.mtbt_sizeof_components_args, COMPONENTS_STRUCTS), (lib.mtbt_sizeof_fill_polygons_args, POLYGON_STRUCTS),
-                                (lib.mtbt_sizeof_clahe_args, CLAHE_STRUCTS)):
+                                (lib.mtbt_sizeof_clahe_args, CLAHE_STRUCTS), (lib.mtbt_sizeof_tail_chain_args, TAIL_CHAIN_STRUCTS)):
             for which, st in enumerate(structs):
                 if sizeof(which) != C.sizeof(st):
                     raise RuntimeError(f"libmtbt_hip.so was built with sizeof({st.__name__}) = {sizeof(which)}, this binding lays it "
diff --git a/multitask_bonetumor_yolo_amd/build.py b/multitask_bonetumor_yolo_amd/build.py
--- a/multitask_bonetumor_yolo_amd/build.py
+++ b/multitask_bonetumor_yolo_amd/build.py
@@ -7,7 +7,7 @@
 CSRC = os.path.join(HERE, "csrc")
 INCLUDE = os.path.join(os.path.dirname(HERE), "include")
 LIB = os.path.join(CSRC, "libmtbt_hip.so")
-SOURCES = ["conv_igemm.hip", "conv_igemm_bf16.hip", "conv_igemm_bf16_n.hip", "conv_direct_bf16.hip", "conv_igemm_f32.hip", "conv_igemm_f32_n.hip", "conv_direct_f32.hip", "conv_igemm_f16.hip", "conv_igemm_f16_n.hip", "conv_direct_f16.hip", "conv_batch_bf16.hip", "conv_batch_f16.hip", "conv_batch_f32.hip", "dwconv.hip", "dwconv_bf16.hip", "dwconv_f16.hip", "dwconv_f32.hip", "pointwise.hip", "postprocess.hip", "mask_mfma.hip", "mask_frame.hip", "bn_train.hip", "mlp_fused.hip", "upconv_fused.hip", "node_gemm.hip", "pw_stream.hip", "pw_chain.hip", "loss.hip", "mask_loss.hip", "det_loss_tal.hip", "preprocess.hip", "metrics.hip", "optim.hip", "wgrad.hip", "pointwise_bwd.hip", "train_ops.hip", "resample_bwd.hip", "box_eval.hip", "mask_eval.hip", "box_fuse.hip", "mask_vote.hip", "tile_merge.hip", "mask_tiles.hip", "surface_dist.hip", "components.hip", "polygon_fill.hip", "clahe.hip"]
+SOURCES = ["conv_igemm.hip", "conv_igemm_bf16.hip", "conv_igemm_bf16_n.hip", "conv_direct_bf16.hip", "conv_igemm_f32.hip", "conv_igemm_f32_n.hip", "conv_direct_f32.hip", "conv_igemm_f16.hip", "conv_igemm_f16_n.hip", "conv_direct_f16.hip", "conv_batch_bf16.hip", "conv_batch_f16.hip", "conv_batch_f32.hip", "dwconv.hip", "dwconv_bf16.hip", "dwconv_f16.hip", "dwconv_f32.hip", "pointwise.hip", "postprocess.hip", "mask_mfma.hip", "mask_frame.hip", "bn_train.hip", "mlp_fused.hip", "upconv_fused.hip", "node_gemm.hip", "pw_stream.hip", "pw_chain.hip", "conv_tail.hip", "loss.hip", "mask_loss.hip", "det_loss_tal.hip", "preprocess.hip", "metrics.hip", "optim.hip", "wgrad.hip", "pointwise_bwd.hip", "train_ops.hip", "resample_bwd.hip", "box_eval.hip", "mask_eval.hip", "box_fuse.hip", "mask_vote.hip", "tile_merge.hip", "mask_tiles.hip", "surface_dist.hip", "components.hip", "polygon_fill.hip", "clahe.hip"]
 HIPCC = os.environ.get("HIPCC", "/opt/rocm/bin/hipcc")
 FLAGS = ["--offload-arch=gfx950", "-O3", "-std=c++17", "-fPIC", "-I" + INCLUDE, "-I" + CSRC,
          "-fno-gpu-rdc", "-Wno-unused-value"]
diff --git a/multitask_bonetumor_yolo_amd/csrc/conv3x3_direct.inc b/multitask_bonetumor_yolo_amd/csrc/conv3x3_direct.inc
--- a/multitask_bonetumor_yolo_amd/csrc/conv3x3_direct.inc
+++ b/multitask_bonetumor_yolo_amd/csrc/conv3x3_direct.inc
@@ -149,14 +149,31 @@
 template <typename T, int TC>
 __global__ __launch_bounds__(256, 2) void conv3x3_rr_kernel(const ConvP p) {
   const unsigned bid = blockIdx.x;
+  constexpr int TAIL_FC2 = 0;
+  constexpr TailP tp{};
 #include "conv3x3_rr_body.inc"
 }
+
+#ifdef MTBT_CONV_TAIL_UNIT
+template <typename T, int TC, int FC2>
+__global__ __launch_bounds__(256, 2) void conv3x3_rr_tail_kernel(const ConvTailP q) {
+  static_assert(sizeof(T) == 2 && TC == 64 && FC2 >= 1 && FC2 <= 4, "one 64-channel tile: the image holds every channel of the 256 tile pixels");
+  static_assert(256 * 128 <= ((324 * 4 + 255) / 256) * 256 * 16 + 2 * 3 * TC * 64, "the image fits the halo and weight stages");
+  const ConvP p = q.p;
+  const TailP tp = q.t;
+  const unsigned bid = blockIdx.x;
+  constexpr int TAIL_FC2 = FC2;
+#include "conv3x3_rr_body.inc"
+}
+#endif
 
 #ifdef MTBT_CONV_BATCH_UNIT
 template <typename T, int TC>
 __global__ __launch_bounds__(256, 2) void conv3x3_rr_batch_kernel(const ConvBatchP b) {
   const ConvP p = conv_member(b, (int)blockIdx.y);
   const unsigned bid = blockIdx.x;
+  constexpr int TAIL_FC2 = 0;
+  constexpr TailP tp{};
 #include "conv3x3_rr_body.inc"
 }
 #endif
diff --git a/multitask_bonetumor_yolo_amd/csrc/conv3x3_rr_body.inc b/multitask_bonetumor_yolo_amd/csrc/conv3x3_rr_body.inc
--- a/multitask_bonetumor_yolo_amd/csrc/conv3x3_rr_body.inc
+++ b/multitask_bonetumor_yolo_amd/csrc/conv3x3_rr_body.inc
@@ -121,7 +121,23 @@
       }
     }
   }
+  constexpr int NF2 = TAIL_FC2 > 0 ? TAIL_FC2 : 1;
+  uint4 a2[2][NF2];
+  if constexpr (TAIL_FC2 > 0) tail_load_w2<T, NF2>(tp, lr, lq, a2);
   __syncthreads();
+
+  if constexpr (TAIL_FC2 > 0) {
+#pragma unroll
+    for (int j = 0; j < FP; ++j) tail_put8<T, TC>(smem, (8 * wr + j) * 16 + lr, wc * WCH + lq * 8, aff, acc[0][j], acc[1][j]);
+    lds_barrier();
+#pragma unroll
+    for (int jj = 0; jj < 4; ++jj) {
+      f32x4 o[NF2];
+      tail_gemm16<T, NF2>(smem, (4 * wave + jj) * 16 + lr, lq, a2, o);
+      tail_store<NF2>(tp, tp.y + (long)n * tp.ybs + ((long)(ty0 + 4 * wave + jj) * p.W + tx0 + lr) * tp.ldy, lq, o);
+    }
+    return;
+  }
 
   const EpiSeq seq{(long)(ty0 + 8 * wr) * p.W + tx0, p.W, 0x7fffffffffffffffL, (long)n * p.ybs, (long)n * p.rbs};
   conv_epilogue<T, TC, FC, FP, false, MTBT_RR_RESPF, (sizeof(T) == 2), true>(p, acc, smem + wave * (2 * 16 * (WCH * 4 + 16)), aff, cbase, wc * WCH, lane,
diff --git a/multitask_bonetumor_yolo_amd/csrc/conv_epilogue.h b/multitask_bonetumor_yolo_amd/csrc/conv_epilogue.h
--- a/multitask_bonetumor_yolo_amd/csrc/conv_epilogue.h
+++ b/multitask_bonetumor_yolo_amd/csrc/conv_epilogue.h
@@ -321,6 +321,63 @@
       st8<HT>(yp + q.ybias + px * p.ldy + ch, v);
     }
   }
+}
+
+__device__ __forceinline__ int tail_img_off(int q, int slot) { return q * 128 + ((slot ^ ((q >> 1) & 7)) << 4); }
+
+template <typename T, int FC2>
+__device__ __forceinline__ void tail_gemm16(const char* img, int q, int lq, const uint4 (&a2)[2][FC2], f32x4 (&o)[FC2]) {
+#pragma unroll
+  for (int i = 0; i < FC2; ++i) o[i] = f32x4{0.f, 0.f, 0.f, 0.f};
+#pragma unroll
+  for (int g = 0; g < 2; ++g) {
+    const uint4 b = *reinterpret_cast<const uint4*>(img + tail_img_off(q, g * 4 + lq));
+#pragma unroll
+    for (int i = 0; i < FC2; ++i) o[i] = mfma_16x16x32<T>(a2[g][i], b, o[i]);
+  }
+}
+
+template <int FC2>
+__device__ __forceinline__ void tail_store(const TailP& tp, float* yrow, int lq, const f32x4 (&o)[FC2]) {
+#pragma unroll
+  for (int i = 0; i < FC2; ++i) {
+    const int ch = i * 16 + lq * 4;
+    if (ch >= tp.K2) continue;
+    float sh[4];
+#pragma unroll
+    for (int e = 0; e < 4; ++e) sh[e] = (tp.bias2 && ch + e < tp.K2) ? tp.bias2[ch + e] : 0.f;
+    const f32x4 v = f32x4{o[i][0] + sh[0], o[i][1] + sh[1], o[i][2] + sh[2], o[i][3] + sh[3]};
+    if (tp.vec_ok && ch + 4 <= tp.K2) *reinterpret_cast<f32x4*>(yrow + ch) = v;
+    else {
+#pragma unroll
+      for (int e = 0; e < 4; ++e)
+        if (ch + e < tp.K2) yrow[ch + e] = v[e];
+    }
+  }
+}
+
+template <typename T, int FC2>
+__device__ __forceinline__ void tail_load_w2(const TailP& tp, int lr, int lq, uint4 (&a2)[2][FC2]) {
+  const T* w2 = reinterpret_cast<const T*>(tp.w2);
+#pragma unroll
+  for (int g = 0; g < 2; ++g)
+#pragma unroll
+    for (int f = 0; f < FC2; ++f) {
+      const int row = f * 16 + lr;
+      a2[g][f] = row < tp.K2 ? *reinterpret_cast<const uint4*>(w2 + (long)row * 64 + g * 32 + lq * 8) : uint4{0u, 0u, 0u, 0u};
+    }
+}
+
+template <typename T, int TC>
+__device__ __forceinline__ void tail_put8(char* img, int q, int cl, const float* aff, const f32x4& lo, const f32x4& hi) {
+  const float4 s0 = *reinterpret_cast<const float4*>(aff + cl), s1 = *reinterpret_cast<const float4*>(aff + cl + 4);
+  const float4 h0 = *reinterpret_cast<const float4*>(aff + TC + cl), h1 = *reinterpret_cast<const float4*>(aff + TC + cl + 4);
+  float v[8];
+  v[0] = act_apply(fmaf(lo[0], s0.x, h0.x), MTBT_ACT_SILU); v[1] = act_apply(fmaf(lo[1], s0.y, h0.y), MTBT_ACT_SILU);
+  v[2] = act_apply(fmaf(lo[2], s0.z, h0.z), MTBT_ACT_SILU); v[3] = act_apply(fmaf(lo[3], s0.w, h0.w), MTBT_ACT_SILU);
+  v[4] = act_apply(fmaf(hi[0], s1.x, h1.x), MTBT_ACT_SILU); v[5] = act_apply(fmaf(hi[1], s1.y, h1.y), MTBT_ACT_SILU);
+  v[6] = act_apply(fmaf(hi[2], s1.z, h1.z), MTBT_ACT_SILU); v[7] = act_apply(fmaf(hi[3], s1.w, h1.w), MTBT_ACT_SILU);
+  st8<T>(reinterpret_cast<T*>(img + tail_img_off(q, cl >> 3)), v);
 }
 
 
diff --git a/multitask_bonetumor_yolo_amd/csrc/conv_igemm.hip b/multitask_bonetumor_yolo_amd/csrc/conv_igemm.hip
--- a/multitask_bonetumor_yolo_amd/csrc/conv_igemm.hip
+++ b/multitask_bonetumor_yolo_amd/csrc/conv_igemm.hip
@@ -267,3 +267,44 @@
   if (!choice) return MTBT_EINVAL;
   return conv_batch_impl(calls, n, nullptr, choice);
 }
+
+int mtbt_conv_tail_dispatch(const ConvTailP& q, int dtype, bool direct, hipStream_t s);
+
+static int tail_plan(const mtbt_conv_tail_args* a, ConvTailP* q, bool* direct) {
+  if (!a || !a->w2 || !a->y) return MTBT_EINVAL;
+  mtbt_conv_args c = a->conv;
+  if (c.dtype != MTBT_BF16 && c.dtype != MTBT_F16) return MTBT_EINVAL;
+  if (c.K != 64 || c.act != MTBT_ACT_SILU || c.out_mode != MTBT_OUT_NHWC) return MTBT_EINVAL;
+  if (c.res || c.y2 || c.colsum || c.colsum_ws || c.debug) return MTBT_EINVAL;
+  if (a->K2 < 1 || a->K2 > 64 || a->y_pixel_stride < a->K2) return MTBT_EINVAL;
+  c.y = const_cast<void*>(c.x);
+  c.out_dtype = c.dtype;
+  c.y_pixel_stride = c.K;
+  c.y_batch_stride = (int64_t)c.Ho * c.Wo * c.K;
+  ConvChoice ch;
+  if (const int rc = conv_plan(&c, 0, &q->p, &ch)) return rc;
+  *direct = ch.kind == CONV_DIRECT3X3;
+  if (!(ch.kind == CONV_IGEMM && ch.TC == 64 && ch.TP == 64 && ch.wide) && !(*direct && ch.TC == 64 && ch.row_reuse)) return MTBT_EINVAL;
+  if (!aligned16(a->w2) || (reinterpret_cast<uintptr_t>(a->y) & 3)) return MTBT_EALIGN;
+  q->p.y = nullptr;
+  TailP& t = q->t;
+  t.w2 = a->w2; t.bias2 = a->bias2; t.y = a->y; t.ybs = a->y_batch_stride; t.ldy = a->y_pixel_stride; t.K2 = a->K2;
+  t.vec_ok = (a->y_pixel_stride % 4 == 0 && a->y_batch_stride % 4 == 0 && aligned16(a->y)) ? 1 : 0;
+  return MTBT_OK;
+}
+
+extern "C" int mtbt_sizeof_tail_chain_args(int which) { return which == 0 ? (int)sizeof(mtbt_conv_tail_args) : -1; }
+
+extern "C" int mtbt_conv_tail_supported(const mtbt_conv_tail_args* a) {
+  ConvTailP q;
+  bool direct;
+  if (tail_plan(a, &q, &direct) != MTBT_OK) return 1;
+  return 0;
+}
+
+extern "C" int mtbt_conv2d_tail_nhwc(const mtbt_conv_tail_args* a, void* stream) {
+  ConvTailP q;
+  bool direct;
+  if (const int rc = tail_plan(a, &q, &direct)) return rc;
+  return mtbt_conv_tail_dispatch(q, a->conv.dtype, direct, reinterpret_cast<hipStream_t>(stream));
+}
diff --git a/multitask_bonetumor_yolo_amd/csrc/conv_igemm.inc b/multitask_bonetumor_yolo_amd/csrc/conv_igemm.inc
--- a/multitask_bonetumor_yolo_amd/csrc/conv_igemm.inc
+++ b/multitask_bonetumor_yolo_amd/csrc/conv_igemm.inc
@@ -16,14 +16,31 @@
 template <typename T, int TC, int TP, int WAVES_C, int WAVES_P, int BKB, int NBUF>
 __global__ __launch_bounds__(256, 2) void conv_igemm_kernel(const ConvP p) {
   const unsigned bid = blockIdx.x;
+  constexpr int TAIL_FC2 = 0;
+  constexpr TailP tp{};
 #include "conv_igemm_body.inc"
 }
+
+#ifdef MTBT_CONV_TAIL_UNIT
+template <typename T, int TC, int TP, int WAVES_C, int WAVES_P, int BKB, int NBUF, int FC2>
+__global__ __launch_bounds__(256, 2) void conv_igemm_tail_kernel(const ConvTailP q) {
+  static_assert(sizeof(T) == 2 && TC == 64 && TP == 64 && WAVES_C == 1 && WAVES_P == 4 && BKB == 128 && FC2 >= 1 && FC2 <= 4,
+                "a wave owns all 64 channels of 16 pixels; the image is one 128-byte K-step's B tile");
+  const ConvP p = q.p;
+  const TailP tp = q.t;
+  const unsigned bid = blockIdx.x;
+  constexpr int TAIL_FC2 = FC2;
+#include "conv_igemm_body.inc"
+}
+#endif
 
 #ifdef MTBT_CONV_BATCH_UNIT
 template <typename T, int TC, int TP, int WAVES_C, int WAVES_P, int BKB, int NBUF>
 __global__ __launch_bounds__(256, 2) void conv_igemm_batch_kernel(const ConvBatchP b) {
   const ConvP p = conv_member(b, (int)blockIdx.y);
   const unsigned bid = blockIdx.x;
+  constexpr int TAIL_FC2 = 0;
+  constexpr TailP tp{};
 #include "conv_igemm_body.inc"
 }
 #endif
diff --git a/multitask_bonetumor_yolo_amd/csrc/conv_igemm_body.inc b/multitask_bonetumor_yolo_amd/csrc/conv_igemm_body.inc
--- a/multitask_bonetumor_yolo_amd/csrc/conv_igemm_body.inc
+++ b/multitask_bonetumor_yolo_amd/csrc/conv_igemm_body.inc
@@ -156,8 +156,25 @@
       }
     }
   }
+  constexpr int NF2 = TAIL_FC2 > 0 ? TAIL_FC2 : 1;
+  uint4 a2[2][NF2];
+  if constexpr (TAIL_FC2 > 0) tail_load_w2<T, NF2>(tp, lr, lq, a2);
   __syncthreads();
   if (MTBT_ABL(p, 16)) return;
+
+  if constexpr (TAIL_FC2 > 0) {
+    const int q = wp * WP + lr;
+#pragma unroll
+    for (int m = 0; m < FC / 2; ++m) tail_put8<T, TC>(smem, q, m * 32 + lq * 8, aff, acc[2 * m][0], acc[2 * m + 1][0]);
+    lds_barrier();
+    f32x4 o[NF2];
+    tail_gemm16<T, NF2>(smem, q, lq, a2, o);
+    const int pix = pbase + q;
+    if (pix >= p.M) return;
+    const int n = pix / HoWo;
+    tail_store<NF2>(tp, tp.y + (long)n * tp.ybs + (long)(pix - n * HoWo) * tp.ldy, lq, o);
+    return;
+  }
 
   const int Cq = p.K >> 2;
   const EpiSeq seq{(long)pbase + wp * WP, 16, (long)p.M, 0, 0};
diff --git a/multitask_bonetumor_yolo_amd/csrc/conv_params.h b/multitask_bonetumor_yolo_amd/csrc/conv_params.h
--- a/multitask_bonetumor_yolo_amd/csrc/conv_params.h
+++ b/multitask_bonetumor_yolo_amd/csrc/conv_params.h
@@ -46,9 +46,23 @@
   ConvMember m[MTBT_CONV_BATCH_MAX];
 };
 
+struct TailP {
+  const void* w2;
+  const float* bias2;
+  float* y;
+  long ybs;
+  int ldy, K2, vec_ok;
+};
+
+struct ConvTailP {
+  ConvP p;
+  TailP t;
+};
+
 #if defined(__HIPCC__)
 inline ConvP& conv_of(ConvP& p) { return p; }
 inline ConvP& conv_of(ConvBatchP& b) { return b.p; }
+inline ConvP& conv_of(ConvTailP& q) { return q.p; }
 template <typename Kernel, typename Params>
 int conv_launch_tiles(Kernel kernel, Params& q, int TC, long ptiles, int n, int lds, hipStream_t stream) {
   ConvP& p = conv_of(q);
diff --git a/multitask_bonetumor_yolo_amd/csrc/conv_tail.hip b/multitask_bonetumor_yolo_amd/csrc/conv_tail.hip
--- /dev/null
+++ b/multitask_bonetumor_yolo_amd/csrc/conv_tail.hip
@@ -0,0 +1,27 @@
+#define MTBT_CONV_TAIL_UNIT
+#include "conv_igemm.inc"
+#include "conv3x3_direct.inc"
+
+namespace {
+
+template <typename T, int FC2>
+int launch_tail(const ConvTailP& q, hipStream_t s) {
+  return launch_tile<64, 64, 1, 128, 2>(conv_igemm_tail_kernel<T, 64, 64, 1, 4, 128, 2, FC2>, q, 1, s);
+}
+
+template <typename T, int FC2>
+int launch_tail_rr(const ConvTailP& q, hipStream_t s) {
+  return launch_direct3x3_rr<64>(conv3x3_rr_tail_kernel<T, 64, FC2>, q, 1, s);
+}
+
+template <typename T>
+int launch_tail_t(const ConvTailP& q, bool direct, hipStream_t s) {
+  if (direct) return q.t.K2 <= 32 ? launch_tail_rr<T, 2>(q, s) : launch_tail_rr<T, 4>(q, s);
+  return q.t.K2 <= 32 ? launch_tail<T, 2>(q, s) : launch_tail<T, 4>(q, s);
+}
+
+}
+
+int mtbt_conv_tail_dispatch(const ConvTailP& q, int dtype, bool direct, hipStream_t s) {
+  return dtype == MTBT_F16 ? launch_tail_t<f16_t>(q, direct, s) : launch_tail_t<bf16_t>(q, direct, s);
+}
diff --git a/multitask_bonetumor_yolo_amd/engine.py b/multitask_bonetumor_yolo_amd/engine.py
--- a/multitask_bonetumor_yolo_amd/engine.py
+++ b/multitask_bonetumor_yolo_amd/engine.py
@@ -562,6 +562,27 @@
         self._io([x, w1, shift1, w2, shift2], [y])
         return a
 
+    def conv_tail_args(self, x: Act, w1: torch.Tensor, shift1, w2: torch.Tensor, bias2, y: Act, *, R=3, S=3, pad=1, scale1=None, any_speed=False):
+        if x.code not in (L.BF16, L.F16) or y.code != L.F32 or (x.N, x.H, x.W) != (y.N, y.H, y.W) or y.C != w2.shape[0] or w2.shape[1] != w1.shape[0]:
+            return None
+        t = Act(x.buf, 0, x.N, x.H, x.W, w1.shape[0], w1.shape[0], x.H * x.W * w1.shape[0])
+        ca, flops, byts = self._conv_args(x, w1, t, R, S, 1, pad, scale1, shift1, L.ACT_SILU, None, L.OUT_NHWC, 0, 0)
+        a = L.ConvTailArgs()
+        a.conv = ca
+        a.conv.y = None
+        a.w2, a.y = w2.data_ptr(), y.ptr
+        a.bias2 = bias2.data_ptr() if bias2 is not None else None
+        a.y_batch_stride, a.y_pixel_stride, a.K2 = y.batch_stride, y.ld, w2.shape[0]
+        return a if self.lib.mtbt_conv_tail_supported(C.byref(a)) in ((0, 2) if any_speed else (0,)) else None
+
+    def conv_tail(self, a, x: Act, w1, shift1, w2, bias2, y: Act, name="conv_tail", scale1=None):
+        n = x.N * x.H * x.W
+        M, K2 = w1.shape[0], w2.shape[0]
+        self.launches.append(Launch(self.lib.mtbt_conv2d_tail_nhwc, (C.byref(a),), name, (a, x.buf, w1, scale1, shift1, w2, bias2, y.buf),
+                                    2.0 * n * (M * w1.shape[1] + K2 * M), (n * x.C + M * w1.shape[1] + K2 * M) * ESIZE[x.code] + n * K2 * 4))
+        self._io([x, w1, scale1, shift1, w2, bias2], [y])
+        return a
+
     def upconv(self, x: Act, w: torch.Tensor, shift9: torch.Tensor, y: Act, act=L.ACT_SILU, name="upconv"):
         K = w.shape[0] // 4
         assert w.shape[1] == 4 * x.C and tuple(shift9.shape) == (9, K) and y.C == K and y.H == 2 * x.H and y.W == 2 * x.W and x.code == y.code
diff --git a/multitask_bonetumor_yolo_amd/graphed.py b/multitask_bonetumor_yolo_amd/graphed.py
--- a/multitask_bonetumor_yolo_amd/graphed.py
+++ b/multitask_bonetumor_yolo_amd/graphed.py
@@ -3,7 +3,7 @@
 from . import postprocess as pp
 
 
-AUTOTUNE_KNOBS = (("PW_CHAIN", ("1",)), ("NODE_FUSED", ("1",)), ("SEG_GATE", ("1", "2")), ("LANE_WIDE_US", ("200",)), ("LANES", ("3",)), ("ADAPTOR_EARLY", ("1",)),
+AUTOTUNE_KNOBS = (("PW_CHAIN", ("1",)), ("TAIL_CHAIN", ("1",)), ("NODE_FUSED", ("1",)), ("SEG_GATE", ("1", "2")), ("LANE_WIDE_US", ("200",)), ("LANES", ("3",)), ("ADAPTOR_EARLY", ("1",)),
                   ("HEADS_EARLY", ("1",)))
 
 
diff --git a/multitask_bonetumor_yolo_amd/model.py b/multitask_bonetumor_yolo_amd/model.py
--- a/multitask_bonetumor_yolo_amd/model.py
+++ b/multitask_bonetumor_yolo_amd/model.py
@@ -245,7 +245,7 @@
     return torch.cat(ws, 1).contiguous(), torch.cat(scs, 0), torch.cat(shs, 0)
 
 
-PLAN_OPTION_DEFAULTS = {"NODE_FUSED": "0", "ADAPTOR_EARLY": "0", "HEADS_EARLY": "0", "SEG_GATE": "0", "HEADS_MERGED": "0", "PW_CHAIN": "0", "LANES": None, "LANE_WIDE_US": None}
+PLAN_OPTION_DEFAULTS = {"NODE_FUSED": "0", "ADAPTOR_EARLY": "0", "HEADS_EARLY": "0", "SEG_GATE": "0", "HEADS_MERGED": "0", "PW_CHAIN": "0", "TAIL_CHAIN": "0", "LANES": None, "LANE_WIDE_US": None}
 
 
 def plan_option(model, name: str):
@@ -562,8 +562,29 @@
         self.conv_plain(t2, s[2], dst, f"{tag}.cv3.{i}.2")
         self.p.release(t2)
 
+    def conv_tail(self, x: Act, block, out: nn.Conv2d, dst: Act, name) -> bool:
+        opt = plan_option(self.m, "TAIL_CHAIN")
+        conv = block.conv
+        if (opt not in ("1", "2") or self.merged or self.code not in (L.BF16, L.F16) or block.bn.training or out.kernel_size != (1, 1)
+                or out.stride != (1, 1) or out.padding != (0, 0) or conv.stride != (1, 1) or conv.kernel_size[0] != conv.kernel_size[1]):
+            return False
+        n0 = len(self.p.consts)
+        k = conv.kernel_size[0]
+        scale, shift = _bn_fold(block.bn, conv.bias)
+        w1, s1 = self.W(_krsc(conv.weight).float() * scale[:, None]), self.F(shift)
+        w2, b2 = self.W(_krsc(out.weight)), (self.F(out.bias) if out.bias is not None else None)
+        a = self.p.conv_tail_args(x, w1, s1, w2, b2, dst, R=k, S=k, pad=k // 2, any_speed=opt == "2")
+        if a is None:
+            del self.p.consts[n0:]
+            return False
+        self.p.conv_tail(a, x, w1, s1, w2, b2, dst, name=name)
+        return True
+
     def conv_chain(self, f: Act, s, name, dst: Act):
         t1 = self.convblock(f, s[0], None, name + ".0")
+        if self.conv_tail(t1, s[1], s[2], dst, name + ".1+2"):
+            self.p.release(t1)
+            return
         t2 = self.convblock(t1, s[1], None, name + ".1")
         self.p.release(t1)
         self.conv_plain(t2, s[2], dst, name + ".2")
```
